# seung-lab/igneous

Measured on AMD Instinct MI355X. Metric: Mvoxels/s meshed (512^3 uint64 seg chunk), higher is better.
Workload: dtype u64; 1 GPU; 512^3 uint64 Voronoi chunk, ~50k labels, seed=303 (BASELINE configs[2]); labels=50000, simplification=0, input_residency=device (MG_FLAG_SKIP_H2D, MG_FLAG_DEVICE_ONLY), n_labels_meshed=49992, total_tris=155686827

## Files before the change

### igneous_amd/csrc/mc_table.h

```cpp
#ifndef MC_TABLE_H
#define MC_TABLE_H

#ifndef MC_TABLE_QUAL
#define MC_TABLE_QUAL static const
#endif

#define MC_MAX_TRIS 5

MC_TABLE_QUAL unsigned char MC_TRI_COUNT[256] = {
  0, 1, 1, 2, 1, 2, 2, 3, 1, 2, 2, 3, 2, 3, 3, 2,
  1, 2, 2, 3, 2, 3, 3, 4, 2, 3, 3, 4, 3, 4, 4, 3,
  1, 2, 2, 3, 2, 3, 3, 4, 2, 3, 3, 4, 3, 4, 4, 3,
  2, 3, 3, 2, 3, 4, 4, 3, 3, 4, 4, 3, 4, 5, 5, 2,
  1, 2, 2, 3, 2, 3, 3, 4, 2, 3, 3, 4, 3, 4, 4, 3,
  2, 3, 3, 4, 3, 2, 4, 3, 3, 4, 4, 5, 4, 3, 5, 2,
  2, 3, 3, 4, 3, 4, 4, 5, 3, 4, 4, 5, 4, 5, 5, 4,
  3, 4, 4, 3, 4, 3, 5, 2, 4, 5, 5, 4, 5, 4, 2, 1,
  1, 2, 2, 3, 2, 3, 3, 4, 2, 3, 3, 4, 3, 4, 4, 3,
  2, 3, 3, 4, 3, 4, 4, 5, 3, 4, 4, 5, 4, 5, 5, 4,
  2, 3, 3, 4, 3, 4, 4, 5, 3, 4, 2, 3, 4, 5, 3, 2,
  3, 4, 4, 3, 4, 5, 5, 4, 4, 5, 3, 2, 5, 2, 4, 1,
  2, 3, 3, 4, 3, 4, 4, 5, 3, 4, 4, 5, 2, 3, 3, 2,
  3, 4, 4, 5, 4, 3, 5, 4, 4, 5, 5, 2, 3, 2, 4, 1,
  3, 4, 4, 5, 4, 5, 5, 2, 4, 5, 3, 4, 3, 4, 2, 1,
// ... 496 lines not shown
  {0x5d30, 0x0af0, 0x6050, 0x6b10, 0x4750},
  {0x6891, 0x5d22, 0x0000, 0x0000, 0x0000},
  {0x5302, 0x5682, 0x5ea2, 0x0000, 0x0000},
  {0x5ea0, 0x0ae0, 0x0000, 0x0000, 0x0000},
  {0x5d30, 0x0af0, 0x6050, 0x5310, 0x0000},
  {0x5d22, 0x0000, 0x0000, 0x0000, 0x0000},
  {0x6ad2, 0x6f52, 0x6772, 0x0000, 0x0000},
  {0x2080, 0x6ad2, 0x6f52, 0x6772, 0x0000},
  {0x5a50, 0x6ad0, 0x6f50, 0x1770, 0x0000},
  {0x6ad2, 0x6f52, 0x1772, 0x10b2, 0x2092},
  {0x6761, 0x4b21, 0x5a41, 0x52c1, 0x0000},
  {0x6c20, 0x6760, 0x4b20, 0x5a40, 0x22c0},
  {0x5a50, 0x52d0, 0x0690, 0x6c30, 0x1770},
  {0x1761, 0x22d2, 0x0000, 0x0000, 0x0000},
  {0x66b1, 0x4b31, 0x5a51, 0x6ad1, 0x0000},
  {0x2080, 0x66b1, 0x4b31, 0x5a51, 0x6ad1},
  {0x5a50, 0x6ad0, 0x4750, 0x0000, 0x0000},
  {0x2091, 0x4911, 0x5a51, 0x6ad1, 0x0000},
  {0x52d2, 0x5692, 0x66b2, 0x0000, 0x0000},
  {0x66a0, 0x4b20, 0x5a40, 0x22c0, 0x0000},
  {0x5a50, 0x52d0, 0x0000, 0x0000, 0x0000},
  {0x22d2, 0x0000, 0x0000, 0x0000, 0x0000},
  {0x6f58, 0x6778, 0x0000, 0x0000, 0x0000},
  {0x6880, 0x6f40, 0x6760, 0x0000, 0x0000},
  {0x6b10, 0x6f50, 0x1770, 0x0000, 0x0000},
  {0x6f44, 0x1764, 0x0000, 0x0000, 0x0000},
  {0x6761, 0x6321, 0x5301, 0x0000, 0x0000},
  {0x6c20, 0x6760, 0x0000, 0x0000, 0x0000},
  {0x5310, 0x0690, 0x6c30, 0x1770, 0x0000},
  {0x1761, 0x0000, 0x0000, 0x0000, 0x0000},
  {0x66b1, 0x6331, 0x6b11, 0x0000, 0x0000},
  {0x6880, 0x4740, 0x5620, 0x66a0, 0x0000},
  {0x6b10, 0x4750, 0x0000, 0x0000, 0x0000},
  {0x6891, 0x0000, 0x0000, 0x0000, 0x0000},
  {0x66b4, 0x6334, 0x0000, 0x0000, 0x0000},
  {0x66a0, 0x0000, 0x0000, 0x0000, 0x0000},
  {0x5310, 0x0000, 0x0000, 0x0000, 0x0000},
  {0x0000, 0x0000, 0x0000, 0x0000, 0x0000},
};

MC_TABLE_QUAL unsigned char MC_TRI_FIRST[256][5] = {
  {0, 0, 0, 0, 0},
  {7, 0, 0, 0, 0},
  {7, 0, 0, 0, 0},
  {7, 4, 0, 0, 0},
  {7, 0, 0, 0, 0},
  {7, 4, 0, 0, 0},
  {7, 7, 0, 0, 0},
  {7, 4, 4, 0, 0},
  {7, 0, 0, 0, 0},
  {7, 7, 0, 0, 0},
  {7, 4, 0, 0, 0},
  {7, 4, 4, 0, 0},
  {7, 4, 0, 0, 0},
  {7, 4, 4, 0, 0},
  {7, 4, 4, 0, 0},
  {7, 4, 0, 0, 0},
  {7, 0, 0, 0, 0},
  {7, 4, 0, 0, 0},
  {7, 7, 0, 0, 0},
  {7, 4, 4, 0, 0},
  {7, 7, 0, 0, 0},
  {7, 4, 4, 0, 0},
  {7, 7, 7, 0, 0},
  {7, 4, 4, 4, 0},
  {7, 7, 0, 0, 0},
  {7, 4, 7, 0, 0},
  {7, 4, 7, 0, 0},
  {7, 4, 4, 4, 0},
  {7, 7, 4, 0, 0},
  {7, 4, 4, 4, 0},
  {7, 4, 4, 7, 0},
  {7, 4, 4, 0, 0},
  {7, 0, 0, 0, 0},
  {7, 7, 0, 0, 0},
  {7, 4, 0, 0, 0},
  {7, 4, 4, 0, 0},
  {7, 7, 0, 0, 0},
  {7, 4, 7, 0, 0},
  {7, 4, 7, 0, 0},
  {7, 4, 4, 4, 0},
  {7, 7, 0, 0, 0},
  {7, 7, 7, 0, 0},
  {7, 4, 4, 0, 0},
  {7, 4, 4, 4, 0},
  {7, 7, 4, 0, 0},
  {7, 4, 4, 7, 0},
  {7, 4, 4, 4, 0},
  {7, 4, 4, 0, 0},
  {7, 4, 0, 0, 0},
  {7, 4, 4, 0, 0},
  {7, 4, 4, 0, 0},
  {7, 4, 0, 0, 0},
  {7, 7, 4, 0, 0},
  {7, 4, 4, 4, 0},
  {7, 4, 4, 7, 0},
  {7, 4, 4, 0, 0},
  {7, 7, 4, 0, 0},
  {7, 4, 4, 7, 0},
  {7, 4, 4, 4, 0},
  {7, 4, 4, 0, 0},
  {7, 4, 7, 4, 0},
  {7, 4, 4, 4, 4},
  {7, 4, 4, 4, 4},
  {7, 4, 0, 0, 0},
  {7, 0, 0, 0, 0},
  {7, 7, 0, 0, 0},
  {7, 7, 0, 0, 0},
  {7, 7, 4, 0, 0},
  {7, 4, 0, 0, 0},
  {7, 4, 4, 0, 0},
  {7, 7, 4, 0, 0},
  {7, 4, 4, 4, 0},
  {7, 7, 0, 0, 0},
  {7, 7, 7, 0, 0},
  {7, 4, 7, 0, 0},
  {7, 4, 4, 7, 0},
  {7, 4, 4, 0, 0},
  {7, 4, 4, 4, 0},
  {7, 4, 4, 4, 0},
  {7, 4, 4, 0, 0},
  {7, 4, 0, 0, 0},
  {7, 4, 4, 0, 0},
  {7, 7, 4, 0, 0},
  {7, 4, 4, 4, 0},
  {7, 4, 4, 0, 0},
  {7, 4, 0, 0, 0},
  {7, 7, 4, 4, 0},
  {7, 4, 4, 0, 0},
  {7, 7, 4, 0, 0},
  {7, 4, 4, 7, 0},
  {7, 4, 7, 4, 0},
  {7, 4, 4, 4, 4},
  {7, 4, 4, 4, 0},
  {7, 4, 4, 0, 0},
  {7, 4, 4, 4, 4},
  {7, 4, 0, 0, 0},
  {7, 7, 0, 0, 0},
  {7, 7, 7, 0, 0},
  {7, 4, 7, 0, 0},
  {7, 4, 4, 7, 0},
  {7, 4, 7, 0, 0},
  {7, 4, 4, 7, 0},
  {7, 4, 7, 4, 0},
  {7, 4, 4, 4, 4},
  {7, 7, 7, 0, 0},
  {7, 7, 7, 7, 0},
  {7, 4, 4, 7, 0},
  {7, 4, 4, 4, 7},
  {7, 7, 4, 4, 0},
  {7, 4, 4, 4, 7},
  {7, 4, 4, 4, 4},
  {7, 4, 4, 4, 0},
  {7, 4, 4, 0, 0},
  {7, 4, 4, 4, 0},
  {7, 4, 4, 4, 0},
  {7, 4, 4, 0, 0},
  {7, 4, 4, 4, 0},
  {7, 4, 4, 0, 0},
  {7, 4, 4, 4, 4},
  {7, 4, 0, 0, 0},
  {7, 7, 4, 4, 0},
  {7, 4, 4, 4, 7},
  {7, 4, 4, 4, 4},
  {7, 4, 4, 4, 0},
  {7, 4, 4, 4, 4},
  {7, 4, 4, 4, 0},
  {7, 7, 0, 0, 0},
  {7, 0, 0, 0, 0},
  {7, 0, 0, 0, 0},
  {7, 7, 0, 0, 0},
  {7, 7, 0, 0, 0},
  {7, 7, 4, 0, 0},
  {7, 7, 0, 0, 0},
  {7, 4, 7, 0, 0},
  {7, 7, 7, 0, 0},
  {7, 4, 4, 7, 0},
  {7, 4, 0, 0, 0},
  {7, 7, 4, 0, 0},
  {7, 4, 4, 0, 0},
  {7, 4, 4, 4, 0},
  {7, 4, 4, 0, 0},
  {7, 4, 4, 4, 0},
  {7, 4, 4, 4, 0},
  {7, 4, 4, 0, 0},
  {7, 7, 0, 0, 0},
  {7, 4, 7, 0, 0},
  {7, 7, 7, 0, 0},
  {7, 4, 4, 7, 0},
  {7, 7, 7, 0, 0},
  {7, 4, 4, 7, 0},
  {7, 7, 7, 7, 0},
  {7, 4, 4, 4, 7},
  {7, 4, 7, 0, 0},
  {7, 4, 7, 4, 0},
  {7, 4, 4, 7, 0},
  {7, 4, 4, 4, 4},
  {7, 7, 4, 4, 0},
  {7, 4, 4, 4, 4},
  {7, 4, 4, 4, 7},
  {7, 4, 4, 4, 0},
  {7, 4, 0, 0, 0},
  {7, 7, 4, 0, 0},
  {7, 4, 4, 0, 0},
  {7, 4, 4, 4, 0},
  {7, 7, 4, 0, 0},
  {7, 4, 7, 4, 0},
  {7, 4, 4, 7, 0},
  {7, 4, 4, 4, 4},
  {7, 4, 4, 0, 0},
  {7, 7, 4, 4, 0},
  {7, 4, 0, 0, 0},
  {7, 4, 4, 0, 0},
  {7, 4, 4, 4, 0},
  {7, 4, 4, 4, 4},
  {7, 4, 4, 0, 0},
  {7, 4, 0, 0, 0},
  {7, 4, 4, 0, 0},
  {7, 4, 4, 4, 0},
  {7, 4, 4, 4, 0},
  {7, 4, 4, 0, 0},
  {7, 7, 4, 4, 0},
  {7, 4, 4, 4, 4},
  {7, 4, 4, 4, 7},
  {7, 4, 4, 4, 0},
  {7, 4, 4, 4, 0},
  {7, 4, 4, 4, 4},
  {7, 4, 4, 0, 0},
  {7, 4, 0, 0, 0},
  {7, 4, 4, 4, 4},
  {7, 7, 0, 0, 0},
  {7, 4, 4, 4, 0},
  {7, 0, 0, 0, 0},
  {7, 4, 0, 0, 0},
  {7, 7, 4, 0, 0},
  {7, 7, 4, 0, 0},
  {7, 4, 7, 4, 0},
  {7, 4, 4, 0, 0},
  {7, 4, 4, 4, 0},
  {7, 7, 4, 4, 0},
  {7, 4, 4, 4, 4},
  {7, 4, 4, 0, 0},
  {7, 7, 4, 4, 0},
  {7, 4, 4, 4, 0},
  {7, 4, 4, 4, 4},
  {7, 4, 0, 0, 0},
  {7, 4, 4, 0, 0},
  {7, 4, 4, 0, 0},
  {7, 4, 0, 0, 0},
  {7, 4, 4, 0, 0},
  {7, 4, 4, 4, 0},
  {7, 7, 4, 4, 0},
  {7, 4, 4, 4, 4},
  {7, 4, 4, 4, 0},
  {7, 4, 4, 0, 0},
  {7, 7, 4, 4, 4},
  {7, 4, 4, 4, 0},
  {7, 4, 4, 4, 0},
  {7, 4, 4, 4, 4},
  {7, 4, 4, 4, 4},
  {7, 7, 0, 0, 0},
  {7, 4, 4, 0, 0},
  {7, 4, 0, 0, 0},
  {7, 4, 4, 4, 0},
  {7, 0, 0, 0, 0},
  {7, 4, 4, 0, 0},
  {7, 7, 4, 4, 0},
  {7, 4, 4, 4, 0},
  {7, 4, 4, 4, 4},
  {7, 4, 4, 4, 0},
  {7, 4, 4, 4, 4},
  {7, 4, 4, 4, 4},
  {7, 7, 0, 0, 0},
  {7, 4, 4, 4, 0},
  {7, 7, 4, 4, 4},
  {7, 4, 4, 0, 0},
  {7, 4, 4, 4, 0},
  {7, 4, 4, 0, 0},
  {7, 4, 4, 4, 0},
  {7, 4, 0, 0, 0},
  {7, 0, 0, 0, 0},
  {7, 4, 0, 0, 0},
  {7, 4, 4, 0, 0},
  {7, 4, 4, 0, 0},
  {7, 4, 0, 0, 0},
  {7, 4, 4, 0, 0},
  {7, 4, 0, 0, 0},
  {7, 4, 4, 4, 0},
  {7, 0, 0, 0, 0},
  {7, 4, 4, 0, 0},
  {7, 4, 4, 4, 0},
  {7, 4, 0, 0, 0},
  {7, 0, 0, 0, 0},
  {7, 4, 0, 0, 0},
  {7, 0, 0, 0, 0},
  {7, 0, 0, 0, 0},
  {0, 0, 0, 0, 0},
};

MC_TABLE_QUAL unsigned char MC_EDGE_NEED[12] = {
  6, 4, 2, 0, 5, 4, 1, 0, 3, 2, 1, 0,
};

MC_TABLE_QUAL unsigned char MC_EDGE_CORNERS[12][2] = {
  {0, 1},
  {2, 3},
  {4, 5},
  {6, 7},
  {0, 2},
  {1, 3},
  {4, 6},
  {5, 7},
  {0, 4},
  {1, 5},
  {2, 6},
  {3, 7},
};

MC_TABLE_QUAL unsigned long long MC_EDGE_KEYOFF[12] = {
  0x1ULL,
  0x2001ULL,
  0x2000001ULL,
  0x2002001ULL,
  0x1000ULL,
  0x1002ULL,
  0x2001000ULL,
  0x2001002ULL,
  0x1000000ULL,
  0x1000002ULL,
  0x1002000ULL,
  0x1002002ULL,
};

#endif
```

### igneous_amd/csrc/meshgine.hip

```cpp

#include "mg_ctx.h"

#include <algorithm>
#include <atomic>
#include <vector>

#define MC_TABLE_QUAL __device__ static const
#include "mc_table.h"


#define WAVE 64

static inline uint64_t next_pow2_u64(uint64_t x) {
  if (x < 2) return 2;
  return 1ull << (64 - __builtin_clzll(x - 1));
}

__device__ __forceinline__ uint64_t mix64(uint64_t x) {
  x += 0x9E3779B97F4A7C15ull;
  x = (x ^ (x >> 30)) * 0xBF58476D1CE4E5B9ull;
  x = (x ^ (x >> 27)) * 0x94D049BB133111EBull;
  return x ^ (x >> 31);
}

__device__ __forceinline__ uint32_t wave_incl_scan(uint32_t x, int lane) {
  for (int d = 1; d < WAVE; d <<= 1) {
    uint32_t y = __shfl_up(x, d, WAVE);
    if (lane >= d) x += y;
  }
  return x;
}


struct LabelHash {
  uint64_t *keys;
  uint32_t *vals;
  uint32_t *counter;
  uint32_t *overflow;
  uint64_t nslots;
};

__device__ __forceinline__ void label_insert(LabelHash h, uint64_t label) {
  uint64_t slot = mix64(label) & (h.nslots - 1);
  for (uint64_t probe = 0; probe < h.nslots; ++probe) {
    uint64_t cur = h.keys[slot];
    if (cur == label) return;
    if (cur == 0) {
      uint64_t prev = atomicCAS((unsigned long long *)&h.keys[slot], 0ull,
                                (unsigned long long)label);
      if (prev == 0) {
        h.vals[slot] = atomicAdd(h.counter, 1u);
        return;
      }
      if (prev == label) return;
    }
    slot = (slot + 1) & (h.nslots - 1);
  }
  atomicExch(h.overflow, 1u);
}

__device__ __forceinline__ uint32_t label_lookup(LabelHash h, uint64_t label) {
  uint64_t slot = mix64(label) & (h.nslots - 1);
  for (uint64_t probe = 0; probe < h.nslots; ++probe) {
    if (h.keys[slot] == label) return h.vals[slot];
    slot = (slot + 1) & (h.nslots - 1);
  }
  atomicExch(h.overflow, 1u);
  return 0;
}


template <typename T>
__global__ void k_dust_build(const T *__restrict__ labels, uint64_t nvox,
                             LabelHash lh) {
  for (uint64_t i = (uint64_t)blockIdx.x * blockDim.x + threadIdx.x;
       i < nvox; i += (uint64_t)gridDim.x * blockDim.x) {
    T L = labels[i];
    if (L != 0) label_insert(lh, (uint64_t)L);
  }
}

template <typename T>
__global__ void k_dust_count(const T *__restrict__ labels, uint64_t nvox,
                             LabelHash lh, uint32_t *__restrict__ counts) {
  for (uint64_t i = (uint64_t)blockIdx.x * blockDim.x + threadIdx.x;
       i < nvox; i += (uint64_t)gridDim.x * blockDim.x) {
    T L = labels[i];
    if (L != 0) atomicAdd(&counts[label_lookup(lh, (uint64_t)L)], 1u);
  }
}

template <typename T>
__global__ void k_dust_zero(T *__restrict__ labels, uint64_t nvox,
                            LabelHash lh,
                            const uint32_t *__restrict__ counts,
                            uint64_t thr) {
  for (uint64_t i = (uint64_t)blockIdx.x * blockDim.x + threadIdx.x;
       i < nvox; i += (uint64_t)gridDim.x * blockDim.x) {
    T L = labels[i];
    if (L != 0 && (uint64_t)counts[label_lookup(lh, (uint64_t)L)] < thr)
      labels[i] = 0;
  }
}


struct MapTable {
  ulonglong2 *slots;
  uint64_t nslots;
};

#define MAP_ERR_DUPLICATE 1u
#define MAP_ERR_FULL      2u

__global__ void k_map_build(const uint64_t *__restrict__ keys,
                            const uint64_t *__restrict__ vals, uint64_t n,
                            MapTable t, uint32_t *__restrict__ err) {
  uint64_t i = (uint64_t)blockIdx.x * blockDim.x + threadIdx.x;
  if (i >= n) return;
  const uint64_t key = keys[i];
  uint64_t slot = mix64(key) & (t.nslots - 1);
  for (uint64_t probe = 0; probe < t.nslots; ++probe) {
    uint64_t prev = atomicCAS((unsigned long long *)&t.slots[slot].x, 0ull,
                              (unsigned long long)key);
    if (prev == 0) {
      t.slots[slot].y = vals[i];
      return;
    }
    if (prev == key) {
      atomicOr(err, MAP_ERR_DUPLICATE);
      return;
    }
    slot = (slot + 1) & (t.nslots - 1);
  }
  atomicOr(err, MAP_ERR_FULL);
}

template <typename T>
__device__ __forceinline__ T map_one(T L, const MapTable &t, bool miss_zero,
                                     T &cl, T &cr) {
  if (L == 0) return 0;
  if (L == cl) return cr;
  T r = miss_zero ? (T)0 : L;
  uint64_t slot = mix64((uint64_t)L) & (t.nslots - 1);
  for (uint64_t probe = 0; probe < t.nslots; ++probe) {
    ulonglong2 e = t.slots[slot];
    if (e.x == (uint64_t)L) { r = (T)e.y; break; }
    if (e.x == 0) break;
    slot = (slot + 1) & (t.nslots - 1);
  }
  cl = L;
  cr = r;
  return r;
}

template <typename T> struct MapVec;
template <> struct MapVec<uint64_t> { typedef ulonglong2 type; };
template <> struct MapVec<uint32_t> { typedef uint4 type; };

template <typename T>
__device__ __forceinline__ void map_volume(T *__restrict__ labels,
                                           uint64_t nvox, const MapTable &t,
                                           uint32_t miss_zero) {
  typedef typename MapVec<T>::type V;
  constexpr int NV = 16 / sizeof(T);
  const uint64_t nvec = nvox / NV;
  const uint64_t tid = (uint64_t)blockIdx.x * blockDim.x + threadIdx.x;
  const uint64_t nthr = (uint64_t)gridDim.x * blockDim.x;
  const bool mz = miss_zero != 0;
  T cl = 0, cr = 0;
  V *vp = reinterpret_cast<V *>(labels);
  for (uint64_t i = tid; i < nvec; i += nthr) {
    union { V v; T e[NV]; } in, o;
    in.v = vp[i];
    bool changed = false;
#pragma unroll
    for (int k = 0; k < NV; ++k) {
      o.e[k] = map_one<T>(in.e[k], t, mz, cl, cr);
      changed |= (o.e[k] != in.e[k]);
    }
    if (changed) vp[i] = o.v;
  }
  const uint64_t i = nvec * NV + tid;
  if (i < nvox) {
    T L = labels[i];
    T r = map_one<T>(L, t, mz, cl, cr);
    if (r != L) labels[i] = r;
  }
}

template <typename T>
__global__ void k_label_map(T *__restrict__ labels, uint64_t nvox,
                            MapTable t, uint32_t miss_zero) {
  map_volume<T>(labels, nvox, t, miss_zero);
}

#define MAP_LDS_MAX_ENTRIES 2048u
#define MAP_LDS_BLOCK 1024

template <typename T>
__global__ __launch_bounds__(MAP_LDS_BLOCK) void k_label_map_lds(
    T *__restrict__ labels, uint64_t nvox, MapTable g, uint32_t miss_zero) {
  extern __shared__ ulonglong2 s_map_tab[];
  for (uint32_t i = threadIdx.x; i < (uint32_t)g.nslots; i += blockDim.x)
    s_map_tab[i] = g.slots[i];
  __syncthreads();
  MapTable t;
  t.slots = s_map_tab;
  t.nslots = g.nslots;
  map_volume<T>(labels, nvox, t, miss_zero);
}

__global__ void k_label_values(LabelHash h, uint64_t *values, uint64_t nslots) {
  uint64_t i = (uint64_t)blockIdx.x * blockDim.x + threadIdx.x;
  if (i >= nslots) return;
  uint64_t k = h.keys[i];
  if (k != 0) values[h.vals[i]] = k;
}


template <typename T>
__device__ __forceinline__ void load_corners(const T *__restrict__ labels,
                                             int64_t sx, int64_t sxy,
                                             int64_t cx, int64_t cy, int64_t cz,
                                             T c[8]) {
  const T *p = labels + cx + cy * sx + cz * sxy;
  c[0] = p[0];            c[1] = p[1];
  c[2] = p[sx];           c[3] = p[sx + 1];
  c[4] = p[sxy];          c[5] = p[sxy + 1];
  c[6] = p[sxy + sx];     c[7] = p[sxy + sx + 1];
}

struct CellClass {
  uint64_t rows;
  uint32_t first;
  __device__ __forceinline__ uint32_t row(uint32_t i) const {
    return (uint32_t)(rows >> (i * 8u)) & 255u;
  }
};

template <typename T>
__device__ __forceinline__ CellClass classify_cell(const T c[8]) {
  uint32_t r[8];
  #pragma unroll
  for (int i = 0; i < 8; ++i) r[i] = 1u << i;
  uint32_t seen = 0;
  #pragma unroll
  for (int j = 1; j < 8; ++j) {
    #pragma unroll
    for (int i = 0; i < j; ++i) {
      const bool eq = c[i] == c[j];
      r[i] |= eq ? (1u << j) : 0u;
      r[j] |= eq ? (1u << i) : 0u;
      seen |= eq ? (1u << j) : 0u;
    }
  }
  uint32_t nz = 0;
  #pragma unroll
  for (int i = 0; i < 8; ++i) nz |= (c[i] != 0) ? (1u << i) : 0u;
  const uint32_t lo = r[0] | (r[1] << 8) | (r[2] << 16) | (r[3] << 24);
  const uint32_t hi = r[4] | (r[5] << 8) | (r[6] << 16) | (r[7] << 24);
  CellClass k;
  k.rows = ((uint64_t)hi << 32) | lo;
  k.first = r[0] == 255u ? 0u : (nz & ~seen);
  return k;
}

template <typename T>
__device__ __forceinline__ T pick_corner(const T c[8], uint32_t i) {
  const bool b0 = i & 1u, b1 = i & 2u, b2 = i & 4u;
  const T a0 = b0 ? c[1] : c[0], a1 = b0 ? c[3] : c[2];
  const T a2 = b0 ? c[5] : c[4], a3 = b0 ? c[7] : c[6];
  const T d0 = b1 ? a1 : a0, d1 = b1 ? a3 : a2;
  return b2 ? d1 : d0;
}

struct GridDims {
  int64_t sx, sy, sz;
  int64_t ncx, ncy, ncz;
  int64_t nsegx;
  int64_t nseg;
};

struct SegSched {
  int64_t beg, end, step;
};

__device__ __forceinline__ SegSched xcd_seg_sched(int64_t nseg,
                                                  int waves_per_blk,
                                                  int wave_in_blk) {
  const int64_t xcd = blockIdx.x & 7;
  const int64_t j = blockIdx.x >> 3;
  const int64_t nbx = (gridDim.x + 7) >> 3;
  const int64_t slab = (nseg + 7) >> 3;
  SegSched ss;
  ss.beg = xcd * slab + j * waves_per_blk + wave_in_blk;
  ss.end = std::min<int64_t>((xcd + 1) * slab, nseg);
  ss.step = nbx * waves_per_blk;
  return ss;
}

template <typename T>
__global__ void k_count(const T *__restrict__ labels, GridDims g,
                        uint64_t *__restrict__ segcnt, LabelHash lh) {
  __shared__ uint8_t s_cnt[256];
  for (int k = threadIdx.x; k < 256; k += blockDim.x)
    s_cnt[k] = MC_TRI_COUNT[k];
  __syncthreads();
  const int lane = threadIdx.x & (WAVE - 1);
  const int wave_in_blk = threadIdx.x / WAVE;
  const int waves_per_blk = blockDim.x / WAVE;
  const int64_t sxy = g.sx * g.sy;
  const SegSched ss = xcd_seg_sched(g.nseg, waves_per_blk, wave_in_blk);
  for (int64_t seg = ss.beg; seg < ss.end; seg += ss.step) {
    const int64_t row = seg / g.nsegx;
    const int64_t segx = seg - row * g.nsegx;
    const int64_t cy = row % g.ncy;
    const int64_t cz = row / g.ncy;
    const int64_t cx = segx * WAVE + lane;
    uint32_t cnt = 0;
    if (cx < g.ncx) {
      T c[8];
      load_corners(labels, g.sx, sxy, cx, cy, cz, c);
      const CellClass k = classify_cell(c);
      cnt = (uint32_t)__popc(k.first);
      for (uint32_t f = k.first; f; f &= f - 1) {
        const uint32_t i = (uint32_t)__builtin_ctz(f);
        cnt += (uint32_t)s_cnt[k.row(i)] << 16;
        label_insert(lh, (uint64_t)pick_corner(c, i));
      }
    }
    uint32_t incl = wave_incl_scan(cnt, lane);
    if (lane == WAVE - 1)
      segcnt[seg] = ((uint64_t)(incl >> 16) << 32) | (incl & 0xffffu);
  }
}


__device__ __forceinline__ void stage_decode_tables(
    uint16_t *s_pack, uint32_t *s_comb, int64_t sx, int64_t sxy) {
  for (int k = threadIdx.x; k < 256; k += blockDim.x) {
    #pragma unroll
    for (int t = 0; t < MC_MAX_TRIS; ++t)
      s_pack[k * MC_MAX_TRIS + t] = MC_TRI_PACK[k][t];
  }
  if (threadIdx.x < 12) {
    int e = threadIdx.x;
    uint32_t eoff = (uint32_t)(MC_EDGE_DOFF[e][0] >> 1) +
                    (uint32_t)(MC_EDGE_DOFF[e][1] >> 1) * (uint32_t)sx +
                    (uint32_t)(MC_EDGE_DOFF[e][2] >> 1) * (uint32_t)sxy;
    uint32_t axis = (MC_EDGE_DOFF[e][0] & 1)
                        ? 0u
                        : ((MC_EDGE_DOFF[e][1] & 1) ? 1u : 2u);
    s_comb[e] = eoff * 3u + axis;
  }
}

template <typename T>
__global__ __launch_bounds__(256, 8) void k_emit(
    const T *__restrict__ labels, GridDims g,
    const uint64_t *__restrict__ segoff, LabelHash lh,
    uint32_t *__restrict__ item_label, uint2 *__restrict__ item_recs) {
  const int lane = threadIdx.x & (WAVE - 1);
  const int wave_in_blk = threadIdx.x / WAVE;
  const int waves_per_blk = blockDim.x / WAVE;
  const int64_t sxy = g.sx * g.sy;
  const SegSched ss = xcd_seg_sched(g.nseg, waves_per_blk, wave_in_blk);
  for (int64_t seg = ss.beg; seg < ss.end; seg += ss.step) {
    const int64_t row = seg / g.nsegx;
    const int64_t segx = seg - row * g.nsegx;
    const int64_t cy = row % g.ncy;
    const int64_t cz = row / g.ncy;
    const int64_t cx = segx * WAVE + lane;
    T c[8];
    CellClass k;
    k.rows = 0;
    k.first = 0;
    if (cx < g.ncx) {
      load_corners(labels, g.sx, sxy, cx, cy, cz, c);
      k = classify_cell(c);
    }
    const uint32_t cnt = (uint32_t)__popc(k.first);
    uint32_t incl = wave_incl_scan(cnt, lane);
    uint32_t pos = (uint32_t)segoff[seg] + incl - cnt;
    const uint32_t cell_lin = (uint32_t)((cz * g.sy + cy) * g.sx + cx);
    const uint32_t zero = (uint32_t)(cx == 0) | ((uint32_t)(cy == 0) << 1) |
                          ((uint32_t)(cz == 0) << 2);
    for (uint32_t f = k.first; f; f &= f - 1) {
      const uint32_t i = (uint32_t)__builtin_ctz(f);
      const uint32_t lid = label_lookup(lh, (uint64_t)pick_corner(c, i));
      item_label[pos] = lid;
      item_recs[pos] = make_uint2(cell_lin, k.row(i) | (zero << 11));
      ++pos;
    }
  }
}

struct ItemTris {
  __device__ uint32_t operator()(uint2 rec) const {
    return MC_TRI_COUNT[rec.y & 255u];
  }
};
struct ItemTrisVia {
  const uint2 *recs;
  __device__ uint32_t operator()(uint32_t o) const {
    return MC_TRI_COUNT[recs[o].y & 255u];
  }
};

#define WELD_FIRST_BLK 256
__global__ void k_label_ranges(const uint32_t *__restrict__ item_lab,
                               uint32_t *__restrict__ itoff,
                               uint32_t *__restrict__ tri_off,
                               uint32_t *__restrict__ blk_item,
                               uint64_t nitems, uint64_t ntris,
                               uint32_t nlabels) {
  uint64_t i = (uint64_t)blockIdx.x * blockDim.x + threadIdx.x;
  if (i >= nitems) return;
  uint32_t a = 0;
  if (i == 0) {
    itoff[0] = 0;
    tri_off[item_lab[0]] = 0;
    tri_off[nlabels] = (uint32_t)ntris;
  } else {
    a = itoff[i];
    if (item_lab[i] != item_lab[i - 1]) tri_off[item_lab[i]] = a;
  }
  const uint32_t b = itoff[i + 1];
  const uint32_t m = (a + WELD_FIRST_BLK - 1) / WELD_FIRST_BLK;
  if (m * WELD_FIRST_BLK < b) blk_item[m] = (uint32_t)i;
}



__global__ __launch_bounds__(WELD_FIRST_BLK) void k_weld_first(
    const uint2 *__restrict__ item_recs,
    const uint32_t *__restrict__ order,
    const uint32_t *__restrict__ item_lab,
    const uint32_t *__restrict__ itoff,
    const uint32_t *__restrict__ blk_item,
    uint32_t *__restrict__ lab_sorted,
    uint32_t *__restrict__ slots_sorted,
    uint32_t *__restrict__ wminp,
    unsigned long long *__restrict__ bits,
    int64_t sx, int64_t sxy,
    uint64_t nitems, uint64_t ntris, uint64_t nwords) {
  __shared__ uint16_t s_pack[256 * MC_MAX_TRIS];
  __shared__ uint8_t s_first[256 * MC_MAX_TRIS];
  __shared__ uint32_t s_comb[12];
  __shared__ uint32_t s_need[12];
  __shared__ uint32_t s_off[WELD_FIRST_BLK + 1];
  __shared__ uint2 s_rec[WELD_FIRST_BLK];
  __shared__ uint32_t s_lab[WELD_FIRST_BLK];
  __shared__ uint8_t s_item[WELD_FIRST_BLK];
  stage_decode_tables(s_pack, s_comb, sx, sxy);
  for (int k = threadIdx.x; k < 256 * MC_MAX_TRIS; k += blockDim.x)
    s_first[k] = MC_TRI_FIRST[k / MC_MAX_TRIS][k % MC_MAX_TRIS];
  if (threadIdx.x < 12) s_need[threadIdx.x] = MC_EDGE_NEED[threadIdx.x];
  const uint64_t t = (uint64_t)blockIdx.x * WELD_FIRST_BLK + threadIdx.x;
  const uint32_t t0 = blockIdx.x * WELD_FIRST_BLK;
  const uint64_t first = blk_item[blockIdx.x];
  const uint64_t it = first + threadIdx.x;
  s_off[threadIdx.x] = itoff[std::min<uint64_t>(it, nitems)];
  if (threadIdx.x == 0)
    s_off[WELD_FIRST_BLK] =
        itoff[std::min<uint64_t>(first + WELD_FIRST_BLK, nitems)];
  __syncthreads();
  {
    const uint32_t lo = std::max(s_off[threadIdx.x], t0);
    const uint32_t hi = std::min<uint32_t>(s_off[threadIdx.x + 1],
                                           t0 + WELD_FIRST_BLK);
    if (lo < hi) {
      s_rec[threadIdx.x] = order ? item_recs[order[it]] : item_recs[it];
      s_lab[threadIdx.x] = item_lab[it];
      for (uint32_t q = lo; q < hi; ++q)
        s_item[q - t0] = (uint8_t)threadIdx.x;
    }
  }
  __syncthreads();
  const uint32_t lane = threadIdx.x & (WAVE - 1);
  bool f[3] = {false, false, false};
  if (t < ntris) {
    const uint32_t j = s_item[threadIdx.x];
    uint2 rec = s_rec[j];
    rec.y |= ((uint32_t)t - s_off[j]) << 8;
    lab_sorted[t] = s_lab[j];
    const uint32_t ti = (rec.y & 255u) * MC_MAX_TRIS + ((rec.y >> 8) & 7u);
    const uint32_t pk = s_pack[ti];
    const uint32_t fb = s_first[ti];
    const uint32_t interior = ~(rec.y >> 11) & 7u;
    const uint32_t cl3 = rec.x * 3u;
    #pragma unroll
    for (int v = 0; v < 3; ++v) {
      const uint32_t nib = (pk >> (5 * v)) & 31u;
      const uint32_t e = nib & 15u;
      const uint32_t slot = ((cl3 + s_comb[e]) << 1) | (nib >> 4);
      slots_sorted[3 * t + v] = slot;
      f[v] = ((fb >> v) & 1u) && (s_need[e] & interior) == 0;
      if (f[v]) wminp[slot] = (uint32_t)(3 * t + v);
    }
  }
  const unsigned long long bal[3] = {__ballot(f[0]), __ballot(f[1]),
                                     __ballot(f[2])};
  const uint64_t w0 = (t / WAVE) * 3;
  #pragma unroll
  for (uint32_t j = 0; j < 3; ++j) {
    const uint32_t c = 64 * j + lane;
    const uint32_t q = c / 3, r = c - 3 * q;
    const unsigned long long src = r == 0 ? bal[0] : (r == 1 ? bal[1] : bal[2]);
    const unsigned long long word = __ballot((src >> q) & 1ull);
    if (lane == j && w0 + j < nwords) bits[w0 + j] = word;
  }
}

struct PopcWord {
  __device__ uint32_t operator()(unsigned long long w) const {
    return (uint32_t)__popcll(w);
  }
};

__device__ __forceinline__ uint32_t vtx_id_of(
    const uint32_t *__restrict__ wscan,
    const unsigned long long *__restrict__ bits, uint64_t i) {
  uint64_t w = i >> 6;
  unsigned long long mask = (1ull << (i & 63)) - 1;
  return wscan[w] + (uint32_t)__popcll(bits[w] & mask);
}

__global__ void k_total_verts(const uint32_t *__restrict__ wscan,
                              const unsigned long long *__restrict__ bits,
                              uint64_t nwords, uint32_t *out) {
  *out = wscan[nwords - 1] + (uint32_t)__popcll(bits[nwords - 1]);
}

__global__ void k_vbase(const uint32_t *__restrict__ tri_off,
                        const uint32_t *__restrict__ wscan,
                        const unsigned long long *__restrict__ bits,
                        uint32_t *__restrict__ vbase,
                        uint32_t nlabels, uint64_t total_verts) {
  uint32_t l = blockIdx.x * blockDim.x + threadIdx.x;
  if (l > nlabels) return;
  if (l == nlabels) vbase[l] = (uint32_t)total_verts;
  else vbase[l] = vtx_id_of(wscan, bits, 3ull * tri_off[l]);
}

__global__ void k_weld_verts_faces(const uint32_t *__restrict__ slots,
                                   const uint32_t *__restrict__ wminp,
                                   const uint32_t *__restrict__ lab_sorted,
                                   const uint32_t *__restrict__ wscan,
                                   const unsigned long long *__restrict__ bits,
                                   const uint32_t *__restrict__ vbase,
                                   float *__restrict__ verts,
                                   uint32_t *__restrict__ faces,
                                   uint32_t usx, uint32_t usxy,
                                   float rx, float ry, float rz, float shift,
                                   uint64_t ntris) {
  uint64_t t = (uint64_t)blockIdx.x * blockDim.x + threadIdx.x;
  if (t >= ntris) return;
  const uint32_t e[3] = {slots[3 * t], slots[3 * t + 1], slots[3 * t + 2]};
  const uint32_t base = vbase[lab_sorted[t]];
  const uint64_t w0 = (3 * t) >> 6;
  const uint32_t b0 = (uint32_t)((3 * t) & 63);
  const bool straddle = b0 > 61;
  const unsigned long long word0 = bits[w0];
  const uint32_t scan0 = wscan[w0];
  const unsigned long long word1 = straddle ? bits[w0 + 1] : 0ull;
  const uint32_t scan1 = straddle ? wscan[w0 + 1] : 0u;
  #pragma unroll
  for (int v = 0; v < 3; ++v) {
    uint32_t b = b0 + v;
    const bool second = b > 63;
    const unsigned long long word = second ? word1 : word0;
    b &= 63;
    uint32_t vid;
    if ((word >> b) & 1ull) {
      vid = (second ? scan1 : scan0) +
            (uint32_t)__popcll(word & ((1ull << b) - 1));
      uint32_t eslot = e[v] >> 1;
      uint32_t axis = eslot % 3u;
      uint32_t lin = eslot / 3u;
      uint32_t vz = lin / usxy;
      uint32_t rem = lin - vz * usxy;
      uint32_t vy = rem / usx;
      uint32_t vx = rem - vy * usx;
      float dx = (float)(2 * vx + (axis == 0));
      float dy = (float)(2 * vy + (axis == 1));
      float dz = (float)(2 * vz + (axis == 2));
      verts[3ull * vid + 0] = (0.5f * dx + shift) * rx;
      verts[3ull * vid + 1] = (0.5f * dy + shift) * ry;
      verts[3ull * vid + 2] = (0.5f * dz + shift) * rz;
    } else {
      vid = vtx_id_of(wscan, bits, wminp[e[v]]);
    }
    faces[3 * t + v] = vid - base;
  }
}

__global__ void k_iota(uint32_t *p, uint64_t n) {
  uint64_t i = (uint64_t)blockIdx.x * blockDim.x + threadIdx.x;
  if (i < n) p[i] = (uint32_t)i;
}

__global__ void k_last_sum(const uint32_t *scan, const uint32_t *input,
                           uint64_t n, uint32_t *out) {
  *out = scan[n - 1] + input[n - 1];
}

__global__ void k_any_active(const uint8_t *active, uint32_t nlabels,
                             uint32_t *any) {
  uint32_t l = blockIdx.x * blockDim.x + threadIdx.x;
  if (l < nlabels && active[l]) atomicExch(any, 1u);
}

#include "simplify.hip"


static LabelHash label_hash_view(mg_ctx *c) {
  LabelHash lh;
  lh.keys = c->lh_keys.get();
  lh.vals = c->lh_vals.get();
  lh.counter = &c->scalars->lh_counter;
  lh.overflow = &c->scalars->lh_overflow;
  lh.nslots = c->lh_slots;
  return lh;
}

static int label_hash_reset(mg_ctx *c, int rc) {
  if (ensure(c, c->lh_keys, c->lh_slots)) return rc;
  if (ensure(c, c->lh_vals, c->lh_slots)) return rc;
  HIP_TRY(c, hipMemsetAsync(c->lh_keys.get(), 0, c->lh_slots * 8, c->stream),
          rc);
  HIP_TRY(c, hipMemsetAsync(c->scalars.get(), 0, sizeof(CtxScalars),
                            c->stream), rc);
  return 0;
}

static int label_hash_grow(mg_ctx *c, const char *where, int rc) {
  if (c->lh_slots >= (1ull << 27)) {
    SET_ERR(c, "label hash overflow%s at %llu slots", where,
            (unsigned long long)c->lh_slots);
    return rc;
  }
  c->lh_slots <<= 2;
  return 0;
}

static int hash_volume_labels(mg_ctx *c, int dtype, uint64_t nvox,
                              const char *where, int rc, uint32_t *p_n) {
  hipStream_t s = c->stream;
  for (;;) {
    if (int e = label_hash_reset(c, rc)) return e;
    const LabelHash lh = label_hash_view(c);
    by_dtype(dtype, [&](auto t) {
      using T = decltype(t);
      hipLaunchKernelGGL(k_dust_build<T>, dim3(4096), dim3(256), 0, s,
                         c->labels.as<const T>(), nvox, lh);
    });
    uint32_t misc[2] = {0, 0};
    HIP_TRY(c, hipMemcpyAsync(misc, &c->scalars->lh_counter, 8,
                              hipMemcpyDeviceToHost, s), rc);
    HIP_TRY(c, hipStreamSynchronize(s), rc);
    if (!misc[1]) {
      *p_n = misc[0];
      return 0;
    }
    if (int e = label_hash_grow(c, where, rc)) return e;
  }
}

#include "fill_holes.hip"

extern "C" {

const char *mg_version(void) { return "meshgine 0.1.0 (gfx950)"; }

int mg_device_count(void) {
  int n = 0;
  if (hipGetDeviceCount(&n) != hipSuccess) return 0;
  return n;
}

mg_ctx *mg_init(int device_id) {
  int n = 0;
  if (hipGetDeviceCount(&n) != hipSuccess || device_id >= n || n == 0) {
    return nullptr;
  }
  if (hipSetDevice(device_id) != hipSuccess) return nullptr;
  mg_ctx *c = new mg_ctx();
  c->device = device_id;
  bool ok =
      hipStreamCreateWithFlags(&c->stream, hipStreamNonBlocking) ==
          hipSuccess &&
      hipStreamCreateWithFlags(&c->stream2, hipStreamNonBlocking) ==
          hipSuccess;
  for (auto &e : c->ev) ok = ok && hipEventCreate(&e) == hipSuccess;
  ok = ok && ensure(c, c->scalars, 1) == 0 &&
       hipMemsetAsync(c->scalars.get(), 0, sizeof(CtxScalars), c->stream) ==
           hipSuccess;
  if (!ok) {
    delete c;
    return nullptr;
  }
  return c;
}

void mg_destroy(mg_ctx *c) { delete c; }

const char *mg_last_error(mg_ctx *c) {
  return c ? c->err.c_str() : g_err.c_str();
}

int mg_get_stats(mg_ctx *c, mg_stats *out) {
  if (!c || !out) return 1;
  *out = c->stats;
  return 0;
}

void mg_meshset_free(mg_meshset *ms) {
  free(ms);
}

}

static int new_meshset(mg_ctx *c, uint32_t n, mg_meshset **out) {
  *out = alloc_meshset(n, 0);
  if (!*out) {
    SET_ERR(c, "mesh_chunk: out of host memory");
    return 24;
  }
  return 0;
}

static double ev_ms(mg_ctx *c, int a, int b) {
  float ms = 0.f;
  if (hipEventElapsedTime(&ms, c->ev[a], c->ev[b]) != hipSuccess) return 0.0;
  return (double)ms;
}


#define MG_MAP_MAX_ENTRIES (1ull << 24)

struct ChunkCall {
  int sx, sy, sz, dtype;
  size_t esize;
  uint64_t nvox;
  GridDims g;
  float rx, ry, rz;
  int voxel_centered;
  uint32_t nlabels;
  uint64_t NI;
  uint64_t T;
  uint64_t V;
  const uint32_t *item_lab;
  const uint2 *rec_src;
  const uint32_t *order_sorted;
  uint32_t *slots;
  uint32_t *lab_sorted;
};

static void set_hole_stash(mg_ctx *c, const ChunkCall &k) {
  c->holes_valid = true;
  c->holes_sx = k.sx; c->holes_sy = k.sy; c->holes_sz = k.sz;
  c->holes_dtype = k.dtype;
}

static int upload_labels(mg_ctx *c, const ChunkCall &k,
                         const void *labels_host, uint32_t flags) {
  const size_t bytes = k.nvox * k.esize;
  if ((flags & (MG_FLAG_SKIP_H2D | MG_FLAG_COUNTED)) && c->labels.cap >= bytes)
    return 0;
  if (ensure_bytes(c, c->labels, bytes)) return 11;
  HIP_TRY(c, hipMemcpyAsync(c->labels.ptr, labels_host, bytes,
                            hipMemcpyHostToDevice, c->stream), 11);
  return 0;
}

static int run_dust(mg_ctx *c, const ChunkCall &k, uint64_t dust_threshold) {
  hipStream_t s = c->stream;
  uint32_t ndl = 0;
  if (int e = hash_volume_labels(c, k.dtype, k.nvox, " (dust)", 16, &ndl))
    return e;
  if (ndl == 0) return 0;
  const LabelHash lh = label_hash_view(c);
  if (ensure(c, c->order, ndl)) return 16;
  HIP_TRY(c, hipMemsetAsync(c->order.get(), 0, (uint64_t)ndl * 4, s), 16);
  by_dtype(k.dtype, [&](auto t) {
    using T = decltype(t);
    const dim3 nb(4096), blk(256);
    hipLaunchKernelGGL(k_dust_count<T>, nb, blk, 0, s,
                       c->labels.as<const T>(), k.nvox, lh, c->order.get());
    hipLaunchKernelGGL(k_dust_zero<T>, nb, blk, 0, s, c->labels.as<T>(),
                       k.nvox, lh, c->order.get(), dust_threshold);
  });
  HIP_TRY(c, hipGetLastError(), 16);
  return 0;
}

static int run_label_map(mg_ctx *c, const ChunkCall &k,
                         const mg_label_map *map) {
  hipStream_t s = c->stream;
  const uint64_t n = map->n, nvox = k.nvox;
  MapTable mt;
  mt.nslots = next_pow2_u64(std::max<uint64_t>(2 * n, 64));
  if (ensure(c, c->map_tab, mt.nslots)) return 41;
  mt.slots = c->map_tab.get();
  uint32_t *d_err = &c->scalars->map_err;
  HIP_TRY(c, hipEventRecord(c->ev[EV_MAP_START], s), 41);
  HIP_TRY(c, hipMemsetAsync(mt.slots, 0, mt.nslots * 16, s), 41);
  HIP_TRY(c, hipMemsetAsync(d_err, 0, 4, s), 41);
  if (n > 0) {
    if (ensure(c, c->map_keys, n)) return 41;
    if (ensure(c, c->map_vals, n)) return 41;
    HIP_TRY(c, hipMemcpyAsync(c->map_keys.get(), map->keys, n * 8,
                              hipMemcpyHostToDevice, s), 41);
    HIP_TRY(c, hipMemcpyAsync(c->map_vals.get(), map->vals, n * 8,
                              hipMemcpyHostToDevice, s), 41);
    const int bblk = 256;
    hipLaunchKernelGGL(k_map_build, dim3((uint32_t)((n + bblk - 1) / bblk)),
                       dim3(bblk), 0, s, c->map_keys.get(),
                       c->map_vals.get(), n, mt, d_err);
  }
  const uint64_t nvec = nvox / (16 / k.esize);
  const uint32_t miss_zero = map->miss == MG_MAP_MISS_ZERO;
  static const bool use_lds = []() {
    const char *e = getenv("MG_MAP_LDS");
    return !(e && e[0] == '0');
  }();
  const bool lds = use_lds && n <= MAP_LDS_MAX_ENTRIES;
  const int mblk = lds ? MAP_LDS_BLOCK : 256;
  const uint32_t mnb = (uint32_t)std::min<uint64_t>(
      std::max<uint64_t>((nvec + mblk - 1) / mblk, 1), lds ? 512 : 4096);
  by_dtype(k.dtype, [&](auto t) {
    using T = decltype(t);
    if (lds)
      hipLaunchKernelGGL(k_label_map_lds<T>, dim3(mnb), dim3(mblk),
                         mt.nslots * 16, s, c->labels.as<T>(), nvox, mt,
                         miss_zero);
    else
      hipLaunchKernelGGL(k_label_map<T>, dim3(mnb), dim3(mblk), 0, s,
                         c->labels.as<T>(), nvox, mt, miss_zero);
  });
  HIP_TRY(c, hipGetLastError(), 41);
  HIP_TRY(c, hipEventRecord(c->ev[EV_MAP_END], s), 41);
  uint32_t map_err = 0;
  HIP_TRY(c, hipMemcpyAsync(&map_err, d_err, 4, hipMemcpyDeviceToHost, s),
          41);
  HIP_TRY(c, hipStreamSynchronize(s), 41);
  if (map_err & MAP_ERR_DUPLICATE) {
    SET_ERR(c, "label map: duplicate key among %llu entries",
            (unsigned long long)n);
    return 42;
  }
  if (map_err) {
    SET_ERR(c, "label map: table build failed (flag %u)", map_err);
    return 42;
  }
  c->stats.ms_labelmap = ev_ms(c, EV_MAP_START, EV_MAP_END);
  return 0;
}

static inline uint32_t seg_blocks(const GridDims &g, int blk) {
  const int waves_per_blk = blk / WAVE;
  int64_t nb = std::min<int64_t>(
      (g.nseg + waves_per_blk - 1) / waves_per_blk, 8192);
  return (uint32_t)((nb + 7) & ~7ll);
}

static int count_pass(mg_ctx *c, ChunkCall &k, bool *p_overflow) {
  hipStream_t s = c->stream;
  const LabelHash lh = label_hash_view(c);
  uint64_t *d_segcnt = c->segcnt.get();
  uint64_t *d_segoff = c->segoff.get();
  const int64_t nseg = k.g.nseg;
  HIP_TRY(c, hipEventRecord(c->ev[EV_H2D_END], s), 30);
  by_dtype(k.dtype, [&](auto t) {
    using T = decltype(t);
    hipLaunchKernelGGL(k_count<T>, dim3(seg_blocks(k.g, 256)), dim3(256), 0,
                       s, c->labels.as<const T>(), k.g, d_segcnt, lh);
  });
  HIP_TRY(c, hipGetLastError(), 30);
  HIP_TRY(c, hipEventRecord(c->ev[EV_COUNT_END], s), 30);

  uint32_t misc[2] = {0, 0};
  HIP_TRY(c, hipMemcpyAsync(misc, &c->scalars->lh_counter, 8,
                            hipMemcpyDeviceToHost, s), 30);
  if (int e = scan_u64(c, d_segcnt, d_segoff, (size_t)nseg, s,
                       "seg scan size query failed", "seg scan failed", 30))
    return e;
  uint64_t last_off = 0, last_cnt = 0;
  HIP_TRY(c, hipMemcpyAsync(&last_off, d_segoff + (nseg - 1), 8,
                            hipMemcpyDeviceToHost, s), 30);
  HIP_TRY(c, hipMemcpyAsync(&last_cnt, d_segcnt + (nseg - 1), 8,
                            hipMemcpyDeviceToHost, s), 30);
  HIP_TRY(c, hipEventRecord(c->ev[EV_SCAN_END], s), 30);
  HIP_TRY(c, hipStreamSynchronize(s), 30);
  *p_overflow = misc[1] != 0;
  k.nlabels = misc[0];
  const uint64_t total = last_off + last_cnt;
  k.NI = total & 0xffffffffull;
  k.T = total >> 32;
  return 0;
}

static int run_count_emit(mg_ctx *c, ChunkCall &k) {
  hipStream_t s = c->stream;
  if (ensure(c, c->segcnt, k.g.nseg)) return 12;
  if (ensure(c, c->segoff, k.g.nseg)) return 12;
  for (;;) {
    if (int e = label_hash_reset(c, 12)) return e;
    bool overflow = false;
    if (int e = count_pass(c, k, &overflow)) return e;
    if (!overflow) break;
    if (int e = label_hash_grow(c, "", 13)) return e;
  }
  c->stats.total_tris = k.T;
  c->stats.n_labels = k.nlabels;
  if (k.T == 0 || k.nlabels == 0) return 0;
  if (k.T > (1ull << 31) / 3 * 2) {
    SET_ERR(c, "chunk produces %llu triangles (> corner-index limit); "
            "split the task shape", (unsigned long long)k.T);
    return 15;
  }
  if (k.nlabels >= (1u << 27)) {
    SET_ERR(c, "%u labels exceed the 2^27 per-chunk label limit", k.nlabels);
    return 15;
  }
  const LabelHash lh = label_hash_view(c);
  if (ensure(c, c->label_values, k.nlabels)) return 17;
  hipLaunchKernelGGL(k_label_values,
                     dim3((uint32_t)((c->lh_slots + 255) / 256)), dim3(256),
                     0, s, lh, c->label_values.get(), c->lh_slots);
  if (ensure(c, c->tri_label, k.NI)) return 18;
  if (ensure(c, c->tri_keys, k.NI)) return 18;
  by_dtype(k.dtype, [&](auto t) {
    using T = decltype(t);
    hipLaunchKernelGGL(k_emit<T>, dim3(seg_blocks(k.g, 256)), dim3(256), 0, s,
                       c->labels.as<const T>(), k.g, c->segoff.get(), lh,
                       c->tri_label.get(), c->tri_keys.get());
  });
  HIP_TRY(c, hipGetLastError(), 18);
  HIP_TRY(c, hipEventRecord(c->ev[EV_EMIT_END], s), 18);
  return 0;
}

struct TriSortView {
  uint64_t *recs, *recs_alt;
  uint32_t *slots;
};

static TriSortView tri_sort_view(mg_ctx *c, uint64_t NI) {
  return {reinterpret_cast<uint64_t *>(c->tri_keys.get()),
          reinterpret_cast<uint64_t *>(c->keys_sorted.get()),
          c->keys_sorted.get() + 2 * NI};
}

static int run_partition(mg_ctx *c, ChunkCall &k) {
  hipStream_t s = c->stream;
  const uint64_t T = k.T, NI = k.NI;
  const char *sre = getenv("MG_SORT_RECS");
  const bool sort_recs = !(sre && sre[0] == '0');
  if (ensure(c, c->keys_sorted, 2 * NI + 3 * T)) return 19;
  if (ensure(c, c->tri_label_alt, NI)) return 19;
  const TriSortView tv = tri_sort_view(c, NI);
  k.slots = tv.slots;
  const dim3 nb((uint32_t)((NI + 255) / 256)), blk(256);
  unsigned end_bit = 1;
  while ((1u << end_bit) < k.nlabels) ++end_bit;
  rocprim::double_buffer<uint32_t> d_keys(c->tri_label.get(),
                                          c->tri_label_alt.get());
  if (sort_recs) {
    rocprim::double_buffer<uint64_t> d_vals(tv.recs, tv.recs_alt);
    if (int e = sort_pairs(c, d_keys, d_vals, NI, 0u, end_bit, s,
                           "radix_sort size query failed",
                           "radix_sort failed", 19))
      return e;
    k.rec_src = reinterpret_cast<const uint2 *>(d_vals.current());
    k.order_sorted = nullptr;
  } else {
    if (ensure(c, c->order, NI)) return 19;
    if (ensure(c, c->order_alt, NI)) return 19;
    hipLaunchKernelGGL(k_iota, nb, blk, 0, s, c->order.get(), NI);
    rocprim::double_buffer<uint32_t> d_vals(c->order.get(),
                                            c->order_alt.get());
    if (int e = sort_pairs(c, d_keys, d_vals, NI, 0u, end_bit, s,
                           "radix_sort size query failed",
                           "radix_sort failed", 19))
      return e;
    k.rec_src = c->tri_keys.get();
    k.order_sorted = d_vals.current();
  }
  k.item_lab = d_keys.current();
  if (ensure(c, c->itoff, NI + 1)) return 19;
  uint32_t *itoff = c->itoff.get();
  if (int e = k.order_sorted
          ? scan_incl_u32(c, rocprim::make_transform_iterator(
                                 k.order_sorted, ItemTrisVia{k.rec_src}),
                          itoff + 1, NI, s, "item scan size query failed",
                          "item scan failed", 19)
          : scan_incl_u32(c, rocprim::make_transform_iterator(
                                 k.rec_src, ItemTris{}),
                          itoff + 1, NI, s, "item scan size query failed",
                          "item scan failed", 19))
    return e;
  if (ensure(c, c->tri_off, (uint64_t)k.nlabels + 1)) return 19;
  if (ensure(c, c->blk_item, (T + WELD_FIRST_BLK - 1) / WELD_FIRST_BLK))
    return 19;
  hipLaunchKernelGGL(k_label_ranges, nb, blk, 0, s, k.item_lab, itoff,
                     c->tri_off.get(), c->blk_item.get(), NI, T, k.nlabels);
  HIP_TRY(c, hipGetLastError(), 19);
  HIP_TRY(c, hipEventRecord(c->ev[EV_PARTITION_END], s), 19);
  return 0;
}

struct WeldScanView {
  unsigned long long *bits;
  uint32_t *wscan;
};

static WeldScanView weld_scan_view(mg_ctx *c, uint64_t nwords) {
  return {reinterpret_cast<unsigned long long *>(c->vtx_scan.get()),
          c->vtx_scan.get() + 2 * nwords};
}

static int run_weld(mg_ctx *c, ChunkCall &k) {
  hipStream_t s = c->stream;
  const uint64_t T = k.T, NC = 3 * T;
  const uint64_t wslots = 6 * k.nvox;
  if (wslots >= (1ull << 32)) {
    SET_ERR(c, "chunk too large for the 32-bit weld table (%d x %d x %d); "
            "split the task shape (the reference's own mesher bound is "
            "1023x1023x511, igneous_cli/cli.py:1049-1052)", k.sx, k.sy, k.sz);
    return 20;
  }
  if (ensure(c, c->wh_keys, wslots)) return 20;
  if (ensure(c, c->vtx_scan, NC)) return 20;
  if (ensure(c, c->lab_sorted, T)) return 20;
  k.lab_sorted = c->lab_sorted.get();
  uint32_t *wminp = c->wh_keys.get();
  const dim3 nbt((uint32_t)((T + 255) / 256)), blk(256);
  const uint64_t nwords = (NC + 63) / 64;
  auto [bits, wscan] = weld_scan_view(c, nwords);
  hipLaunchKernelGGL(k_weld_first,
                     dim3((uint32_t)((T + WELD_FIRST_BLK - 1) / WELD_FIRST_BLK)),
                     dim3(WELD_FIRST_BLK), 0, s, k.rec_src, k.order_sorted,
                     k.item_lab, c->itoff.get(), c->blk_item.get(),
                     k.lab_sorted, k.slots, wminp, bits, k.g.sx,
                     k.g.sx * k.g.sy, k.NI, T, nwords);
  if (int e = scan_u32(c, rocprim::make_transform_iterator(bits, PopcWord{}),
                       wscan, nwords, s, "weld scan size query failed",
                       "weld scan failed", 20))
    return e;
  uint32_t *d_tv = &c->scalars->weld_verts;
  hipLaunchKernelGGL(k_total_verts, dim3(1), dim3(1), 0, s, wscan, bits,
                     nwords, d_tv);
  uint32_t tv = 0;
  HIP_TRY(c, hipMemcpyAsync(&tv, d_tv, 4, hipMemcpyDeviceToHost, s), 21);
  HIP_TRY(c, hipStreamSynchronize(s), 21);
  k.V = tv;
  c->stats.total_verts = tv;

  if (ensure(c, c->verts, 3 * k.V)) return 22;
  if (ensure(c, c->faces, NC)) return 22;
  if (ensure(c, c->vbase, (uint64_t)k.nlabels + 1)) return 22;
  hipLaunchKernelGGL(k_vbase, dim3((k.nlabels + 1 + 255) / 256), dim3(256),
                     0, s, c->tri_off.get(), wscan, bits, c->vbase.get(),
                     k.nlabels, k.V);
  hipLaunchKernelGGL(k_weld_verts_faces, nbt, blk, 0, s, k.slots, wminp,
                     k.lab_sorted, wscan, bits, c->vbase.get(),
                     c->verts.get(), c->faces.get(), (uint32_t)k.g.sx,
                     (uint32_t)(k.g.sx * k.g.sy), k.rx, k.ry, k.rz,
                     k.voxel_centered ? 0.0f : 0.5f, T);
  HIP_TRY(c, hipGetLastError(), 22);
  HIP_TRY(c, hipEventRecord(c->ev[EV_WELD_END], s), 22);
  return 0;
}

static int extract_meshset(mg_ctx *c, const ChunkCall &k, uint32_t flags,
                           mg_meshset **out) {
  hipStream_t s = c->stream;
  if (flags & MG_FLAG_DEVICE_ONLY) {
    HIP_TRY(c, hipStreamSynchronize(s), 23);
    return new_meshset(c, 0, out);
  }
  const uint32_t nlabels = k.nlabels;
  const uint64_t V = k.V, NC = 3 * k.T;
  if (ensure(c, c->h_verts, 3 * V + 3)) return 24;
  if (ensure(c, c->h_faces, NC + 1)) return 24;
  float *h_verts = c->h_verts.get();
  uint32_t *h_faces = c->h_faces.get();
  std::vector<uint32_t> h_tri_off(nlabels + 1), h_vbase(nlabels + 1);
  std::vector<uint64_t> h_label_values(nlabels);
  if (V > 0)
    HIP_TRY(c, hipMemcpyAsync(h_verts, c->verts.get(), V * 12,
                              hipMemcpyDeviceToHost, s), 24);
  if (NC > 0)
    HIP_TRY(c, hipMemcpyAsync(h_faces, c->faces.get(), NC * 4,
                              hipMemcpyDeviceToHost, s), 24);
  HIP_TRY(c, hipMemcpyAsync(h_tri_off.data(), c->tri_off.get(),
                            (nlabels + 1) * 4, hipMemcpyDeviceToHost, s), 24);
  HIP_TRY(c, hipMemcpyAsync(h_vbase.data(), c->vbase.get(), (nlabels + 1) * 4,
                            hipMemcpyDeviceToHost, s), 24);
  HIP_TRY(c, hipMemcpyAsync(h_label_values.data(), c->label_values.get(),
                            nlabels * 8, hipMemcpyDeviceToHost, s), 24);
  HIP_TRY(c, hipStreamSynchronize(s), 24);

  mg_meshset *ms = nullptr;
  if (int e = new_meshset(c, nlabels, &ms)) return e;
  ms->verts_base = h_verts;
  ms->faces_base = h_faces;
  ms->total_verts = V;
  ms->total_tris = k.T;
  std::vector<uint32_t> idx(nlabels);
  for (uint32_t i = 0; i < nlabels; ++i) idx[i] = i;
  std::sort(idx.begin(), idx.end(), [&](uint32_t a, uint32_t b) {
    return h_label_values[a] < h_label_values[b];
  });
  for (uint32_t m = 0; m < nlabels; ++m) {
    uint32_t l = idx[m];
    set_mesh(ms, m, h_label_values[l], h_vbase[l], h_vbase[l + 1] - h_vbase[l],
             h_tri_off[l], h_tri_off[l + 1] - h_tri_off[l]);
  }
  *out = ms;
  return 0;
}

#include "encode.hip"

struct ChunkRequest {
  const void *labels;
  int sx, sy, sz, dtype;
  float rx, ry, rz;
  uint32_t reduction_factor;
  float max_error;
  int voxel_centered;
  uint64_t dust_threshold;
  uint32_t flags;
  const mg_label_map *map;
  uint32_t fill_level;
  const mg_encode_params *ep;
  mg_meshset **out;
  mg_blobset **bout;
  EncParams enc;
};

static int empty_result(mg_ctx *c, const ChunkRequest &r) {
  return r.bout ? new_blobset(c, 0, r.bout) : new_meshset(c, 0, r.out);
}

static void write_stage_times(mg_ctx *c, const ChunkRequest &r, bool meshed) {
  mg_stats &st = c->stats;
  st.ms_h2d = ev_ms(c, EV_START, EV_H2D_END);
  if (r.fill_level) st.ms_fill = ev_ms(c, EV_FILL_START, EV_FILL_END);
  if (!meshed) return;
  st.ms_count = ev_ms(c, EV_H2D_END, EV_COUNT_END);
  st.ms_scan = ev_ms(c, EV_COUNT_END, EV_SCAN_END);
  st.ms_emit = ev_ms(c, EV_SCAN_END, EV_EMIT_END);
  st.ms_partition = ev_ms(c, EV_EMIT_END, EV_PARTITION_END);
  st.ms_weld = ev_ms(c, EV_PARTITION_END, EV_WELD_END);
  st.ms_simplify = ev_ms(c, EV_WELD_END, EV_SIMPLIFY_END);
  st.ms_d2h = ev_ms(c, r.bout ? EV_ENCODE_END : EV_SIMPLIFY_END, EV_END);
  if (r.bout) st.ms_encode = ev_ms(c, EV_SIMPLIFY_END, EV_ENCODE_END);
  st.ms_total = ev_ms(c, EV_START, EV_END);
}

static int mesh_chunk_impl(mg_ctx *c, const ChunkRequest &r) {
  ChunkCall k = {};
  k.sx = r.sx; k.sy = r.sy; k.sz = r.sz; k.dtype = r.dtype;
  k.esize = (r.dtype == MG_U64) ? 8 : 4;
  k.nvox = (uint64_t)r.sx * r.sy * r.sz;
  k.rx = r.rx; k.ry = r.ry; k.rz = r.rz;
  k.voxel_centered = r.voxel_centered;
  GridDims &g = k.g;
  g.sx = r.sx; g.sy = r.sy; g.sz = r.sz;
  g.ncx = r.sx > 1 ? r.sx - 1 : 0;
  g.ncy = r.sy > 1 ? r.sy - 1 : 0;
  g.ncz = r.sz > 1 ? r.sz - 1 : 0;
  g.nsegx = (g.ncx + WAVE - 1) / WAVE;
  g.nseg = g.nsegx * g.ncy * g.ncz;

  memset(&c->stats, 0, sizeof(c->stats));
  c->stats.bytes_read_algorithmic = k.nvox * k.esize;
  hipStream_t s = c->stream;

  if (g.nseg == 0) {
    if (int e = empty_result(c, r)) return e;
    if (r.fill_level) set_hole_stash(c, k);
    return 0;
  }

  HIP_TRY(c, hipEventRecord(c->ev[EV_START], s), 10);
  if (int e = upload_labels(c, k, r.labels, r.flags)) return e;
  HIP_TRY(c, hipEventRecord(c->ev[EV_H2D_END], s), 11);
  if (r.dust_threshold > 0)
    if (int e = run_dust(c, k, r.dust_threshold)) return e;
  if (r.map)
    if (int e = run_label_map(c, k, r.map)) return e;
  if (r.fill_level) {
    HIP_TRY(c, hipEventRecord(c->ev[EV_FILL_START], s), 56);
    if (int e = run_fill_holes(c, r.dtype, r.sx, r.sy, r.sz, r.fill_level,
                               nullptr))
      return e;
    HIP_TRY(c, hipEventRecord(c->ev[EV_FILL_END], s), 56);
    set_hole_stash(c, k);
  }

  if (int e = run_count_emit(c, k)) return e;
  if (k.T == 0 || k.nlabels == 0) {
    if (int e = empty_result(c, r)) return e;
    HIP_TRY(c, hipStreamSynchronize(s), 14);
    write_stage_times(c, r, false);
    return 0;
  }
  if (int e = run_partition(c, k)) return e;
  if (int e = run_weld(c, k)) return e;
  if (r.reduction_factor > 1 && k.T > 0)
    if (int e = run_simplify(c, k.nlabels, k.lab_sorted, r.reduction_factor,
                             r.max_error, &k.T, &k.V))
      return e;
  HIP_TRY(c, hipEventRecord(c->ev[EV_SIMPLIFY_END], s), 22);
  if (int e = r.bout ? run_encode(c, k, r.flags, r.enc, r.bout)
                     : extract_meshset(c, k, r.flags, r.out))
    return e;
  HIP_TRY(c, hipEventRecord(c->ev[EV_END], s), 25);
  HIP_TRY(c, hipStreamSynchronize(s), 25);
  write_stage_times(c, r, true);
  return 0;
}


static int check_volume_args(mg_ctx *c, int sx, int sy, int sz, int dtype) {
  if (sx < 1 || sy < 1 || sz < 1 || sx > 2047 || sy > 2047 || sz > 2047) {
    SET_ERR(c, "dims out of range (1..2047): %d %d %d", sx, sy, sz);
    return 2;
  }
  if (dtype != MG_U32 && dtype != MG_U64) {
    SET_ERR(c, "bad dtype %d", dtype);
    return 3;
  }
  return 0;
}

static int check_label_map(mg_ctx *c, const mg_label_map *map, int dtype,
                           uint32_t flags) {
  if (map->miss != MG_MAP_MISS_KEEP && map->miss != MG_MAP_MISS_ZERO) {
    SET_ERR(c, "label map: bad miss policy %u", map->miss);
    return 5;
  }
  if (flags & MG_FLAG_SKIP_H2D) {
    SET_ERR(c, "label map cannot be combined with MG_FLAG_SKIP_H2D "
            "(the resident volume is already mapped)");
    return 5;
  }
  if (map->n > MG_MAP_MAX_ENTRIES) {
    SET_ERR(c, "label map: %llu entries exceed the %llu-entry cap",
            (unsigned long long)map->n,
            (unsigned long long)MG_MAP_MAX_ENTRIES);
    return 5;
  }
  if (map->n > 0 && (!map->keys || !map->vals)) {
    SET_ERR(c, "label map: null keys/vals with n=%llu",
            (unsigned long long)map->n);
    return 5;
  }
  for (uint64_t i = 0; i < map->n; ++i) {
    if (map->keys[i] == 0) {
      SET_ERR(c, "label map: key 0 at entry %llu (label 0 is never "
              "looked up)", (unsigned long long)i);
      return 5;
    }
    if (dtype == MG_U32 && map->vals[i] > 0xFFFFFFFFull) {
      SET_ERR(c, "label map: value %llu at entry %llu does not fit "
              "MG_U32", (unsigned long long)map->vals[i],
              (unsigned long long)i);
      return 5;
    }
  }
  return 0;
}

#include "chunk_mesh.hip"
#include "merge_verts.hip"
#include "octree_level.hip"
#include "count_voxels.hip"

static int check_counted(mg_ctx *c, const ChunkRequest &r, bool counted) {
  if (r.flags & MG_FLAG_SKIP_H2D) {
    SET_ERR(c, "MG_FLAG_COUNTED cannot be combined with MG_FLAG_SKIP_H2D");
    return 9;
  }
  if (!counted) {
    SET_ERR(c, "MG_FLAG_COUNTED: no counted volume on this ctx (it is left "
            "by mg_count_voxels for the call right after it)");
    return 9;
  }
  if (r.sx != c->counted_sx || r.sy != c->counted_sy ||
      r.sz != c->counted_sz || r.dtype != c->counted_dtype) {
    SET_ERR(c, "MG_FLAG_COUNTED: the counted volume is %d x %d x %d dtype %d, "
            "the call asks for %d x %d x %d dtype %d", c->counted_sx,
            c->counted_sy, c->counted_sz, c->counted_dtype, r.sx, r.sy, r.sz,
            r.dtype);
    return 9;
  }
  return 0;
}

static int mesh_chunk_checked(mg_ctx *c, ChunkRequest r) {
  if (!c) { SET_ERR(c, "null ctx"); return 1; }
  std::lock_guard<std::mutex> g(c->lock);
  c->err.clear();
  if (r.fill_level > 2) {
    SET_ERR(c, "fill_level %u: only levels 0-2 are implemented (level 3 "
            "needs a multilabel dilation, 4+ a merge threshold)",
            r.fill_level);
    return 6;
  }
  if (r.fill_level && (r.flags & MG_FLAG_SKIP_H2D)) {
    SET_ERR(c, "fill_holes cannot be combined with MG_FLAG_SKIP_H2D (the "
            "resident volume is already filled)");
    return 6;
  }
  if (!r.labels || (!r.out && !r.bout)) {
    SET_ERR(c, "null argument");
    return 1;
  }
  if (r.bout)
    if (int e = check_encode_params(c, r.ep, &r.enc)) return e;
  const bool counted = c->counted_valid;
  c->holes_valid = false;
  c->counted_valid = false;
  if (int e = check_volume_args(c, r.sx, r.sy, r.sz, r.dtype)) return e;
  if (r.map)
    if (int e = check_label_map(c, r.map, r.dtype, r.flags)) return e;
  if (r.flags & MG_FLAG_COUNTED)
    if (int e = check_counted(c, r, counted)) return e;
  HIP_TRY(c, hipSetDevice(c->device), 4);
  return mesh_chunk_impl(c, r);
}

extern "C" {

int mg_mesh_chunk_filled(mg_ctx *c, const void *labels, int sx, int sy,
                         int sz, int dtype, float rx, float ry, float rz,
                         uint32_t reduction_factor, float max_error,
                         int voxel_centered, uint64_t dust_threshold,
                         uint32_t flags, const mg_label_map *map,
                         uint32_t fill_level, mg_meshset **out) {
  return mesh_chunk_checked(
      c, {labels, sx, sy, sz, dtype, rx, ry, rz, reduction_factor, max_error,
          voxel_centered, dust_threshold, flags, map, fill_level, nullptr,
          out, nullptr});
}

int mg_mesh_chunk_encoded(mg_ctx *c, const void *labels, int sx, int sy,
                          int sz, int dtype, float rx, float ry, float rz,
                          uint32_t reduction_factor, float max_error,
                          int voxel_centered, uint64_t dust_threshold,
                          uint32_t flags, const mg_label_map *map,
                          const mg_encode_params *params, mg_blobset **out) {
  return mesh_chunk_checked(
      c, {labels, sx, sy, sz, dtype, rx, ry, rz, reduction_factor, max_error,
          voxel_centered, dust_threshold, flags, map, 0u, params, nullptr,
          out});
}

void mg_blobset_free(mg_blobset *bs) { free(bs); }

int mg_mesh_chunk_mapped(mg_ctx *c, const void *labels, int sx, int sy,
                         int sz, int dtype, float rx, float ry, float rz,
                         uint32_t reduction_factor, float max_error,
                         int voxel_centered, uint64_t dust_threshold,
                         uint32_t flags, const mg_label_map *map,
                         mg_meshset **out) {
  return mesh_chunk_checked(
      c, {labels, sx, sy, sz, dtype, rx, ry, rz, reduction_factor, max_error,
          voxel_centered, dust_threshold, flags, map, 0u, nullptr, out,
          nullptr});
}

int mg_mesh_chunk(mg_ctx *c, const void *labels, int sx, int sy, int sz,
                  int dtype, float rx, float ry, float rz,
                  uint32_t reduction_factor, float max_error,
                  int voxel_centered, uint64_t dust_threshold,
                  uint32_t flags, mg_meshset **out) {
  return mesh_chunk_checked(
      c, {labels, sx, sy, sz, dtype, rx, ry, rz, reduction_factor, max_error,
          voxel_centered, dust_threshold, flags, nullptr, 0u, nullptr, out,
          nullptr});
}

int mg_mesh_holes(mg_ctx *c, float rx, float ry, float rz,
                  uint32_t reduction_factor, float max_error,
                  int voxel_centered, uint32_t flags, mg_meshset **out) {
  if (!c) { SET_ERR(c, "null ctx"); return 1; }
  std::lock_guard<std::mutex> g(c->lock);
  c->err.clear();
  if (!out) { SET_ERR(c, "null argument"); return 1; }
  if (!c->holes_valid) {
    SET_ERR(c, "mg_mesh_holes: no hole volume on this ctx (it is left by "
            "mg_mesh_chunk_filled with fill_level > 0 and consumed by one "
            "mg_mesh_holes call)");
    return 7;
  }
  c->holes_valid = false;
  c->counted_valid = false;
  HIP_TRY(c, hipSetDevice(c->device), 4);
  std::swap(c->labels, c->holes);
  return mesh_chunk_impl(
      c, {nullptr, c->holes_sx, c->holes_sy, c->holes_sz, c->holes_dtype, rx,
          ry, rz, reduction_factor, max_error, voxel_centered, 0,
          (flags & MG_FLAG_DEVICE_ONLY) | MG_FLAG_SKIP_H2D, nullptr, 0u,
          nullptr, out, nullptr});
}

int mg_fill_holes(mg_ctx *c, const void *labels, int sx, int sy, int sz,
                  int dtype, uint32_t level, void *filled_out,
                  void *holes_out, uint32_t *rounds_out) {
  if (!c) { SET_ERR(c, "null ctx"); return 1; }
  std::lock_guard<std::mutex> g(c->lock);
  c->err.clear();
  if (!labels || !filled_out || !holes_out) {
    SET_ERR(c, "null argument");
    return 1;
  }
  if (int e = check_volume_args(c, sx, sy, sz, dtype)) return e;
  if (level < 1 || level > 2) {
    SET_ERR(c, "fill level %u: only levels 1-2 are implemented (level 3 "
            "needs a multilabel dilation, 4+ a merge threshold)", level);
    return 6;
  }
  HIP_TRY(c, hipSetDevice(c->device), 4);
  const size_t bytes = (size_t)sx * sy * sz * (dtype == MG_U64 ? 8 : 4);
  c->holes_valid = false;
  c->counted_valid = false;
  if (ensure_bytes(c, c->labels, bytes)) return 11;
  HIP_TRY(c, hipMemcpyAsync(c->labels.ptr, labels, bytes,
                            hipMemcpyHostToDevice, c->stream), 11);
  uint32_t rounds = 0;
  int rc = run_fill_holes(c, dtype, sx, sy, sz, level, &rounds);
  if (rc) return rc;
  HIP_TRY(c, hipMemcpyAsync(filled_out, c->labels.ptr, bytes,
                            hipMemcpyDeviceToHost, c->stream), 55);
  HIP_TRY(c, hipMemcpyAsync(holes_out, c->holes.ptr, bytes,
                            hipMemcpyDeviceToHost, c->stream), 55);
  HIP_TRY(c, hipStreamSynchronize(c->stream), 55);
  if (rounds_out) *rounds_out = rounds;
  return 0;
}

int mg_simplify_mesh(mg_ctx *c,
                     const float *verts, uint32_t nverts,
                     const uint32_t *faces, uint32_t ntris,
                     uint32_t reduction_factor, float max_error,
                     const float **out_verts, uint32_t *out_nverts,
                     const uint32_t **out_faces, uint32_t *out_ntris) {
  if (!c) { SET_ERR(c, "null ctx"); return 1; }
  std::lock_guard<std::mutex> g(c->lock);
  c->err.clear();
  if (!verts || !faces || !out_verts || !out_faces) {
    SET_ERR(c, "null argument");
    return 1;
  }
  c->counted_valid = false;
  if (ntris > (1u << 31) / 3) {
    SET_ERR(c, "mesh too large (%u tris)", ntris);
    return 2;
  }
  HIP_TRY(c, hipSetDevice(c->device), 4);
  hipStream_t s = c->stream;
  uint64_t T = ntris, V = nverts;

  if (reduction_factor > 1 && T > 0 && V > 0) {
    if (ensure(c, c->verts, 3 * V + 3)) return 10;
    if (ensure(c, c->faces, 3 * T + 1)) return 10;
    if (ensure(c, c->tri_off, 2)) return 10;
    if (ensure(c, c->vbase, 2)) return 10;
    if (ensure(c, c->tri_label, T + 1)) return 10;
    if (ensure(c, c->vtx_scan, std::max<uint64_t>(V + 1, 3 * T))) return 10;
    HIP_TRY(c, hipMemcpyAsync(c->verts.get(), verts, V * 12,
                              hipMemcpyHostToDevice, s), 11);
    HIP_TRY(c, hipMemcpyAsync(c->faces.get(), faces, 3 * T * 4,
                              hipMemcpyHostToDevice, s), 11);
    uint32_t off_h[2] = {0, (uint32_t)T};
    uint32_t vb_h[2] = {0, (uint32_t)V};
    HIP_TRY(c, hipMemcpyAsync(c->tri_off.get(), off_h, 8,
                              hipMemcpyHostToDevice, s), 11);
    HIP_TRY(c, hipMemcpyAsync(c->vbase.get(), vb_h, 8,
                              hipMemcpyHostToDevice, s), 11);
    HIP_TRY(c, hipMemsetAsync(c->tri_label.get(), 0, T * 4, s), 11);
    int rc = run_simplify(c, 1, c->tri_label.get(), reduction_factor,
                          max_error, &T, &V);
    if (rc) return rc;
    if (ensure(c, c->h_verts, 3 * V + 3)) return 12;
    if (ensure(c, c->h_faces, 3 * T + 1)) return 12;
    if (V > 0)
      HIP_TRY(c, hipMemcpyAsync(c->h_verts.get(), c->verts.get(), V * 12,
                                hipMemcpyDeviceToHost, s), 12);
    if (T > 0)
      HIP_TRY(c, hipMemcpyAsync(c->h_faces.get(), c->faces.get(), 3 * T * 4,
                                hipMemcpyDeviceToHost, s), 12);
    HIP_TRY(c, hipStreamSynchronize(s), 12);
  } else {
    if (ensure(c, c->h_verts, 3 * V + 3)) return 12;
    if (ensure(c, c->h_faces, 3 * T + 1)) return 12;
    memcpy(c->h_verts.get(), verts, V * 12);
    memcpy(c->h_faces.get(), faces, 3 * T * 4);
  }
  *out_verts = c->h_verts.get();
  *out_nverts = (uint32_t)V;
  *out_faces = c->h_faces.get();
  *out_ntris = (uint32_t)T;
  return 0;
}

int mg_chunk_mesh(mg_ctx *c,
                  const float *verts, uint32_t nverts,
                  const uint32_t *faces, uint32_t ntris,
                  const double scale[3], const double offset[3],
                  mg_meshset **out, const uint32_t **out_order) {
  if (!c) { SET_ERR(c, "null ctx"); return 1; }
  std::lock_guard<std::mutex> g(c->lock);
  c->err.clear();
  if (!out || !out_order || !scale || !offset ||
      (ntris > 0 && (!verts || !faces))) {
    SET_ERR(c, "null argument");
    return 1;
  }
  *out = nullptr;
// ... 114 lines not shown
```

### igneous_amd/csrc/mg_ctx.h

```cpp
#pragma once

#include <cmath>
#include <cstddef>
#include <cstdint>
#include <cstdio>
#include <cstdlib>
#include <cstring>
#include <mutex>
#include <string>
#include <utility>

#include <hip/hip_runtime.h>
#include <rocprim/rocprim.hpp>

#include "../../include/meshgine.h"

template <hipError_t (*FREE)(void *)>
struct OwnedBuf {
  void *ptr = nullptr;
  size_t cap = 0;
  OwnedBuf() = default;
  OwnedBuf(const OwnedBuf &) = delete;
  OwnedBuf &operator=(const OwnedBuf &) = delete;
  OwnedBuf(OwnedBuf &&o) noexcept
      : ptr(std::exchange(o.ptr, nullptr)), cap(std::exchange(o.cap, 0)) {}
  OwnedBuf &operator=(OwnedBuf &&o) noexcept {
    if (this != &o) {
      release();
      ptr = std::exchange(o.ptr, nullptr);
      cap = std::exchange(o.cap, 0);
    }
    return *this;
  }
  ~OwnedBuf() { release(); }
  void release() {
    if (ptr) (void)FREE(ptr);
    ptr = nullptr;
    cap = 0;
  }
};
using DevBuf = OwnedBuf<hipFree>;
using HostBuf = OwnedBuf<hipHostFree>;

template <typename T, typename Owner>
struct TypedArr : Owner {
  T *get() const { return static_cast<T *>(this->ptr); }
  T *operator->() const { return get(); }
};
template <typename T> using DevArr = TypedArr<T, DevBuf>;
template <typename T> using HostArr = TypedArr<T, HostBuf>;

struct LabelVolume : DevBuf {
  template <typename T> T *as() const { return static_cast<T *>(ptr); }
};

struct CtxScalars {
  uint32_t lh_counter;
  uint32_t lh_overflow;
  uint32_t map_err;
  uint32_t weld_verts;
  uint32_t simp_kept;
  uint32_t simp_new_verts;
  uint32_t simp_final_tris;
  uint32_t cv_cursor;
  unsigned long long simp_prof[6];
};
static_assert(offsetof(CtxScalars, lh_overflow) ==
                  offsetof(CtxScalars, lh_counter) + 4, "");

struct SimpPlane;
struct CmMisc;
struct MvMisc;

struct DeviceBuffers {
  DevArr<CtxScalars> scalars;
  LabelVolume labels, holes;
  DevBuf scan_tmp, sort_tmp;
  DevArr<uint64_t> lh_keys, label_values,
      segcnt, segoff;
  DevArr<uint32_t> lh_vals,
      tri_label, tri_label_alt, order, order_alt, tri_off,
      itoff,
      blk_item,
      lab_sorted,
      keys_sorted,
      vtx_scan,
      wh_keys, faces, vbase;
  DevArr<uint2> tri_keys;
  DevArr<float> verts;
  DevArr<SimpPlane> simp_fq;
  DevArr<uint8_t> simp_valid;
  DevArr<float> simp_Q, simp_verts_alt;
  DevArr<unsigned long long> simp_pick;
  DevArr<uint32_t> simp_pk, simp_pk_alt, simp_pv, simp_pv_alt,
      simp_remap, simp_flab, simp_flab_alt, simp_faces_alt, simp_vbase_alt,
      simp_meta,
      simp_ref, simp_keep, simp_keep_scan, simp_park, simp_first,
      simp_troff_final, simp_deg, simp_adj, simp_rh, simp_accept;
  DevArr<ulonglong2> map_tab;
  DevArr<uint64_t> map_keys, map_vals;
  DevArr<uint32_t> fill_vol, fill_parent, fill_cmin, fill_cmax, fill_misc;
  DevArr<CmMisc> cm_misc;
  DevArr<float> cm_verts, cm_pos, cm_out_v;
  DevArr<uint32_t> cm_faces, cm_ncells, cm_pair_off,
      cm_fkey, cm_fkey_alt, cm_fval, cm_fval_alt,
      cm_npts, cm_npts_s, cm_fhead, cm_coff, cm_ford,
      cm_cfrag, cm_ccell,
      cm_cells,
      cm_wkey, cm_wkey_alt, cm_wval, cm_wval_alt, cm_whead, cm_wrun,
      cm_head_pos, cm_rep, cm_keep, cm_used, cm_vid, cm_fslot, cm_out_f;
  DevArr<MvMisc> mv_misc;
  DevArr<float> mv_verts, mv_out_v;
  DevArr<long long> mv_cell;
  DevArr<uint32_t> mv_faces, mv_key, mv_key_alt, mv_val, mv_val_alt,
      mv_parent, mv_keep, mv_used, mv_vid, mv_fslot, mv_out_f,
      mv_tab;
  DevArr<uint64_t> enc_size, enc_off, enc_ilen;
  DevArr<uint32_t> enc_box;
  DevArr<float> enc_bbox;
  DevArr<uint8_t> enc_blob;
  DevArr<uint32_t> ol_order, ol_pref;
  DevArr<int32_t> ol_node;
  DevArr<uint64_t> ol_zsize, ol_zoff;
};

enum {
  EV_START = 0,
  EV_H2D_END,
  EV_COUNT_END,
  EV_SCAN_END,
  EV_EMIT_END,
  EV_PARTITION_END,
  EV_WELD_END,
  EV_END,
  EV_SIMPLIFY_END,
  EV_SIMP_FORK,
  EV_SIMP_JOIN,
  EV_MAP_START,
  EV_MAP_END,
  EV_FILL_START,
  EV_FILL_END,
  EV_ENCODE_END,
  EV_COUNT_
};

struct mg_ctx : DeviceBuffers {
  int device = 0;
  hipStream_t stream = nullptr;
  hipStream_t stream2 = nullptr;
  std::mutex lock;
  std::string err;
  mg_stats stats = {};
  bool holes_valid = false;
  int holes_sx = 0, holes_sy = 0, holes_sz = 0, holes_dtype = 0;
  bool counted_valid = false;
  int counted_sx = 0, counted_sy = 0, counted_sz = 0, counted_dtype = 0;
  uint64_t lh_slots = 1ull << 20;
  HostArr<float> h_verts;
  HostArr<uint32_t> h_faces;
  HostArr<uint8_t> h_blob;
  hipEvent_t ev[EV_COUNT_] = {};

  ~mg_ctx() {
    (void)hipSetDevice(device);
    static_cast<DeviceBuffers &>(*this) = DeviceBuffers();
    h_verts.release();
    h_faces.release();
    h_blob.release();
    for (auto &e : ev) if (e) (void)hipEventDestroy(e);
    if (stream2) (void)hipStreamDestroy(stream2);
    if (stream) (void)hipStreamDestroy(stream);
  }
};

static thread_local std::string g_err;

#define SET_ERR(ctx, ...)                                     \
  do {                                                        \
    char _buf[512];                                           \
    snprintf(_buf, sizeof(_buf), __VA_ARGS__);                \
    if (ctx) (ctx)->err = _buf; else g_err = _buf;            \
  } while (0)

#define HIP_TRY(ctx, call, retcode)                           \
  do {                                                        \
    hipError_t _e = (call);                                   \
    if (_e != hipSuccess) {                                   \
      SET_ERR(ctx, "%s failed: %s (%s:%d)", #call,            \
              hipGetErrorString(_e), __FILE__, __LINE__);     \
      return retcode;                                         \
    }                                                         \
  } while (0)

static int ensure_bytes(mg_ctx *c, HostBuf &b, size_t bytes) {
  if (b.cap >= bytes) return 0;
  b.release();
  size_t want = bytes + bytes / 4;
  if (hipHostMalloc(&b.ptr, want) != hipSuccess &&
      hipHostMalloc(&b.ptr, want = bytes) != hipSuccess) {
    SET_ERR(c, "hipHostMalloc(%zu) failed", bytes);
    return 1;
  }
  b.cap = want;
  return 0;
}

static int ensure_bytes(mg_ctx *c, DevBuf &b, size_t bytes) {
  if (b.cap >= bytes) return 0;
  b.release();
  size_t want = bytes + bytes / 4;
  hipError_t e = hipMalloc(&b.ptr, want);
  if (e != hipSuccess) e = hipMalloc(&b.ptr, want = bytes);
  if (e != hipSuccess) {
    SET_ERR(c, "hipMalloc(%zu) failed: %s", bytes, hipGetErrorString(e));
    return 1;
  }
  b.cap = want;
  return 0;
}

template <typename T, typename Owner>
static int ensure(mg_ctx *c, TypedArr<T, Owner> &b, size_t n) {
  return ensure_bytes(c, static_cast<Owner &>(b), n * sizeof(T));
}

template <typename F>
static auto by_dtype(int dtype, F &&f) {
  if (dtype == MG_U64) return f(uint64_t{});
  return f(uint32_t{});
}

template <typename F>
static int rocprim_two_call(mg_ctx *c, DevBuf &tmp, const char *err_size,
                            const char *err_run, int rc, F call) {
  size_t bytes = 0;
  if (call(nullptr, bytes) != hipSuccess) {
    SET_ERR(c, "%s", err_size);
    return rc;
  }
  if (ensure_bytes(c, tmp, bytes)) return rc;
  if (call(tmp.ptr, bytes) != hipSuccess) {
    SET_ERR(c, "%s", err_run);
    return rc;
  }
  return 0;
}

template <typename In>
static int scan_u32(mg_ctx *c, In in, uint32_t *out, size_t n, hipStream_t s,
                    const char *err_size, const char *err_run, int rc) {
  return rocprim_two_call(
      c, c->scan_tmp, err_size, err_run, rc, [&](void *tmp, size_t &bytes) {
        return rocprim::exclusive_scan(tmp, bytes, in, out, 0u, n,
                                       rocprim::plus<uint32_t>(), s);
      });
}

static int scan_u64(mg_ctx *c, const uint64_t *in, uint64_t *out, size_t n,
                    hipStream_t s, const char *err_size, const char *err_run,
                    int rc) {
  return rocprim_two_call(
      c, c->scan_tmp, err_size, err_run, rc, [&](void *tmp, size_t &bytes) {
        return rocprim::exclusive_scan(tmp, bytes, in, out, uint64_t{0}, n,
                                       rocprim::plus<uint64_t>(), s);
      });
}

template <typename In>
static int scan_incl_u32(mg_ctx *c, In in, uint32_t *out, size_t n,
                         hipStream_t s, const char *err_size,
                         const char *err_run, int rc) {
  return rocprim_two_call(
      c, c->scan_tmp, err_size, err_run, rc, [&](void *tmp, size_t &bytes) {
        return rocprim::inclusive_scan(tmp, bytes, in, out, n,
                                       rocprim::plus<uint32_t>(), s);
      });
}

template <typename V>
static int sort_pairs(mg_ctx *c, rocprim::double_buffer<uint32_t> &keys,
                      rocprim::double_buffer<V> &vals, size_t n,
                      unsigned begin_bit, unsigned end_bit, hipStream_t s,
                      const char *err_size, const char *err_run, int rc) {
  return rocprim_two_call(
      c, c->sort_tmp, err_size, err_run, rc, [&](void *tmp, size_t &bytes) {
        return rocprim::radix_sort_pairs(tmp, bytes, keys, vals, n,
                                         begin_bit, end_bit, s);
      });
}

static mg_meshset *alloc_meshset(uint32_t n, uint32_t extra_u32_per_mesh) {
  const size_t meta_off = sizeof(mg_meshset) + sizeof(mg_mesh) * n;
  mg_meshset *ms = (mg_meshset *)calloc(
      1, meta_off + (size_t)n * (24 + 4 * extra_u32_per_mesh) +
             2 * sizeof(void *));
  if (!ms) return nullptr;
  ms->nmeshes = n;
  ms->meshes = (mg_mesh *)((char *)ms + sizeof(mg_meshset));
  ms->labels_arr = (uint64_t *)((char *)ms + meta_off);
  ms->voff_arr = (uint32_t *)(ms->labels_arr + n);
  ms->nv_arr = ms->voff_arr + n;
  ms->foff_arr = ms->nv_arr + n;
  ms->nf_arr = ms->foff_arr + n;
  return ms;
}

static void set_mesh(mg_meshset *ms, uint32_t m, uint64_t label,
                     uint32_t voff, uint32_t nv, uint32_t foff, uint32_t nf) {
  ms->meshes[m] = {label, nv, nf, ms->verts_base + 3ull * voff,
                   ms->faces_base + 3ull * foff};
  ms->labels_arr[m] = label;
  ms->voff_arr[m] = voff;
  ms->nv_arr[m] = nv;
  ms->foff_arr[m] = foff;
  ms->nf_arr[m] = nf;
}
```

### igneous_amd/engine.py

```python
from __future__ import annotations

import ctypes
import os
import threading
from typing import NamedTuple, Optional

import numpy as np

_HERE = os.path.dirname(os.path.abspath(__file__))
SO_PATH = os.path.join(_HERE, "csrc", "libmeshgine.so")

MG_U32, MG_U64 = 0, 1
MG_FLAG_DEVICE_ONLY = 1
MG_FLAG_SKIP_H2D = 2
MG_FLAG_COUNTED = 4
MG_ERR_NOT_COUNTED = 9
MG_MAP_MISS_KEEP, MG_MAP_MISS_ZERO = 0, 1
LABEL_MAP_MAX_ENTRIES = 1 << 24
LABEL_MAP_LDS_MAX = 2048

_EXPORTED_SYMBOLS = [
    "mg_init", "mg_destroy", "mg_mesh_chunk", "mg_mesh_chunk_mapped",
    "mg_mesh_chunk_filled", "mg_mesh_holes", "mg_fill_holes",
    "mg_simplify_mesh", "mg_chunk_mesh", "mg_meshset_free",
    "mg_get_stats", "mg_last_error", "mg_device_count", "mg_version",
    "mg_mesh_chunk_encoded", "mg_blobset_free",
    "mg_count_voxels", "mg_label_counts_free",
    "mg_merge_close_vertices", "mg_retriangulate_mesh",
    "mg_encode_octree_level", "mg_fragset_free",
]
MG_ENC_PRECOMPUTED, MG_ENC_DRACO = 0, 1


class _MgMesh(ctypes.Structure):
    _fields_ = [
        ("label", ctypes.c_uint64),
        ("nverts", ctypes.c_uint32),
        ("ntris", ctypes.c_uint32),
        ("verts", ctypes.POINTER(ctypes.c_float)),
        ("faces", ctypes.POINTER(ctypes.c_uint32)),
    ]


class _MgMeshSet(ctypes.Structure):
    _fields_ = [
        ("nmeshes", ctypes.c_uint32),
        ("meshes", ctypes.POINTER(_MgMesh)),
        ("verts_base", ctypes.POINTER(ctypes.c_float)),
        ("faces_base", ctypes.POINTER(ctypes.c_uint32)),
        ("total_verts", ctypes.c_uint64),
        ("total_tris", ctypes.c_uint64),
        ("labels_arr", ctypes.POINTER(ctypes.c_uint64)),
        ("voff_arr", ctypes.POINTER(ctypes.c_uint32)),
        ("nv_arr", ctypes.POINTER(ctypes.c_uint32)),
        ("foff_arr", ctypes.POINTER(ctypes.c_uint32)),
        ("nf_arr", ctypes.POINTER(ctypes.c_uint32)),
    ]


class _MgLabelMap(ctypes.Structure):
    _fields_ = [
        ("keys", ctypes.c_void_p),
        ("vals", ctypes.c_void_p),
        ("n", ctypes.c_uint64),
        ("miss", ctypes.c_uint32),
    ]


class MgStats(ctypes.Structure):
    _fields_ = [
        ("ms_h2d", ctypes.c_double),
        ("ms_count", ctypes.c_double),
        ("ms_scan", ctypes.c_double),
        ("ms_emit", ctypes.c_double),
        ("ms_partition", ctypes.c_double),
        ("ms_weld", ctypes.c_double),
        ("ms_simplify", ctypes.c_double),
        ("ms_d2h", ctypes.c_double),
        ("ms_total", ctypes.c_double),
        ("total_tris", ctypes.c_uint64),
        ("total_verts", ctypes.c_uint64),
        ("n_labels", ctypes.c_uint64),
        ("bytes_read_algorithmic", ctypes.c_uint64),
        ("ms_labelmap", ctypes.c_double),
    ]

    def as_dict(self) -> dict:
        out = {}
        for klass in reversed(type(self).__mro__):
            for name, _t in klass.__dict__.get("_fields_", ()):
                out[name] = getattr(self, name)
        return out


class MgStatsFill(MgStats):
    _fields_ = [
        ("ms_fill", ctypes.c_double),
    ]


class MgStatsEncode(MgStatsFill):
    _fields_ = [
        ("ms_encode", ctypes.c_double),
    ]


class _MgEncodeParams(ctypes.Structure):
    _fields_ = [
        ("format", ctypes.c_uint32),
        ("shift", ctypes.c_float * 3),
        ("q_origin", ctypes.c_double * 3),
        ("q_range", ctypes.c_double),
        ("q_bits", ctypes.c_uint32),
    ]


class _MgBlobSet(ctypes.Structure):
    _fields_ = [
        ("n", ctypes.c_uint32),
        ("labels", ctypes.POINTER(ctypes.c_uint64)),
        ("offset", ctypes.POINTER(ctypes.c_uint64)),
        ("size", ctypes.POINTER(ctypes.c_uint64)),
        ("nverts", ctypes.POINTER(ctypes.c_uint32)),
        ("ntris", ctypes.POINTER(ctypes.c_uint32)),
        ("bbox", ctypes.POINTER(ctypes.c_float)),
        ("blob", ctypes.POINTER(ctypes.c_uint8)),
        ("blob_bytes", ctypes.c_uint64),
    ]


_ORDER_CELLS_FN = ctypes.CFUNCTYPE(
    ctypes.c_int, ctypes.POINTER(ctypes.c_int32), ctypes.c_uint32,
    ctypes.POINTER(ctypes.c_uint32), ctypes.c_void_p)


class _MgOctreeLevel(ctypes.Structure):
    _fields_ = [
        ("scale", ctypes.c_double * 3),
        ("offset", ctypes.c_double * 3),
        ("retriangulate", ctypes.c_uint32),
        ("upper_scale", ctypes.c_double * 3),
        ("radius", ctypes.c_double),
        ("chunked", ctypes.c_uint32),
        ("q_origin", ctypes.c_double * 3),
        ("q_voffset", ctypes.c_double * 3),
        ("q_cell", ctypes.c_double * 3),
        ("q_bits", ctypes.c_uint32),
        ("order_cells", _ORDER_CELLS_FN),
        ("order_arg", ctypes.c_void_p),
    ]


class _MgFragSet(ctypes.Structure):
    _fields_ = [
        ("n", ctypes.c_uint32),
        ("nodes", ctypes.POINTER(ctypes.c_int32)),
        ("offset", ctypes.POINTER(ctypes.c_uint64)),
        ("size", ctypes.POINTER(ctypes.c_uint64)),
        ("nverts", ctypes.POINTER(ctypes.c_uint32)),
        ("ntris", ctypes.POINTER(ctypes.c_uint32)),
        ("blob", ctypes.POINTER(ctypes.c_uint8)),
        ("blob_bytes", ctypes.c_uint64),
    ]


class EncodedLevel(NamedTuple):
    nodes: tuple
    sizes: list
    blob: bytes


@_ORDER_CELLS_FN
def _order_cells(nodes, n, order, _arg):
    try:
        import functools
        from .tasks.multires import cmp_zorder
        keys = [tuple(nodes[3 * i:3 * i + 3]) for i in range(n)]
        ranked = sorted(range(n), key=functools.cmp_to_key(
            lambda a, b: cmp_zorder(keys[a], keys[b])))
        for r, i in enumerate(ranked):
            order[r] = i
        return 0
    except Exception:
        return 1


class _MgLabelCounts(ctypes.Structure):
    _fields_ = [
        ("n", ctypes.c_uint64),
        ("labels", ctypes.POINTER(ctypes.c_uint64)),
        ("counts", ctypes.POINTER(ctypes.c_uint64)),
    ]


class EncodedChunk:

    def __init__(self, labels, offsets, sizes, nverts, ntris, bboxes, blob):
        self.labels = np.asarray(labels, dtype=np.uint64)
        self.offsets = np.asarray(offsets, dtype=np.uint64)
        self.sizes = np.asarray(sizes, dtype=np.uint64)
        self.nverts = np.asarray(nverts, dtype=np.uint32)
        self.ntris = np.asarray(ntris, dtype=np.uint32)
        self.bboxes = np.asarray(bboxes, dtype=np.float32).reshape(-1, 6)
        self.blob = np.asarray(blob, dtype=np.uint8)
        n = self.labels.shape[0]
        for name in ("offsets", "sizes", "nverts", "ntris", "bboxes"):
            if getattr(self, name).shape[0] != n:
                raise ValueError(f"EncodedChunk: {name} does not have one "
                                 f"entry per label")
        if n and np.any(self.labels[1:] <= self.labels[:-1]):
            raise ValueError("EncodedChunk: labels must be ascending")
        if n and int((self.offsets + self.sizes).max()) > self.blob.shape[0]:
            raise ValueError("EncodedChunk: an entry ends past the blob")

    def __len__(self) -> int:
        return int(self.labels.shape[0])

    def _index(self, label) -> int:
        label = int(label)
        if 0 <= label < (1 << 64):
            i = int(np.searchsorted(self.labels, np.uint64(label)))
            if i < len(self) and int(self.labels[i]) == label:
                return i
        raise KeyError(label)

    def __contains__(self, label) -> bool:
        try:
            self._index(label)
        except KeyError:
            return False
        return True

    def _bytes(self, i: int) -> bytes:
        o = int(self.offsets[i])
        return self.blob[o:o + int(self.sizes[i])].tobytes()

    def __getitem__(self, label) -> bytes:
        return self._bytes(self._index(label))

    def bbox(self, label) -> list:
        return self.bboxes[self._index(label)].tolist()

    def items(self):
        boxes = self.bboxes.tolist()
        for i, label in enumerate(self.labels.tolist()):
            yield label, self._bytes(i), boxes[i]


def _draco_numbers(draco):
    if draco is None:
        raise ValueError("encoding='draco' needs the draco settings "
                         "(quantization_bits / _range / _origin)")
    if draco.get("quantization_origin") is None \
            or draco.get("quantization_range") is None:
        raise ValueError("draco: quantization_origin and quantization_range "
                         "must be given (MeshTask's draco_encoding_settings "
                         "always sets them)")
    origin = np.asarray(draco["quantization_origin"], dtype=np.float64)
    if origin.shape != (3,):
        raise ValueError("draco: quantization_origin must have 3 components")
    rng = float(np.max(draco["quantization_range"]))
    if rng <= 0:
        rng = 1.0
    bits = int(draco.get("quantization_bits", 14))
    return [float(x) for x in origin], rng, bits


_CHUNK_ARGTYPES = [
    ctypes.c_void_p, ctypes.c_void_p,
    ctypes.c_int, ctypes.c_int, ctypes.c_int, ctypes.c_int,
    ctypes.c_float, ctypes.c_float, ctypes.c_float,
    ctypes.c_uint32, ctypes.c_float, ctypes.c_int,
    ctypes.c_uint64, ctypes.c_uint32,
]
_P_MAP = ctypes.POINTER(_MgLabelMap)
_PP_MESHSET = ctypes.POINTER(ctypes.POINTER(_MgMeshSet))
_CHUNK_TAIL_ARGTYPES = {
    "mg_mesh_chunk": [_PP_MESHSET],
    "mg_mesh_chunk_mapped": [_P_MAP, _PP_MESHSET],
    "mg_mesh_chunk_filled": [_P_MAP, ctypes.c_uint32, _PP_MESHSET],
    "mg_mesh_chunk_encoded": [_P_MAP, ctypes.POINTER(_MgEncodeParams),
                              ctypes.POINTER(ctypes.POINTER(_MgBlobSet))],
}

_lib = None
_lib_lock = threading.Lock()


def load_library() -> ctypes.CDLL:
    global _lib
    with _lib_lock:
        if _lib is not None:
            return _lib
        if not os.path.exists(SO_PATH):
            raise RuntimeError(
                f"meshgine HIP engine not built: {SO_PATH} missing. "
                f"Run __graft_entry__.build() (hipcc --offload-arch=gfx950). "
                f"There is no CPU fallback.")
        lib = ctypes.CDLL(SO_PATH)
        for sym in _EXPORTED_SYMBOLS:
            if not hasattr(lib, sym):
                raise RuntimeError(f"{SO_PATH} missing symbol {sym}")
        lib.mg_init.restype = ctypes.c_void_p
        lib.mg_init.argtypes = [ctypes.c_int]
        lib.mg_destroy.argtypes = [ctypes.c_void_p]
        for name, tail in _CHUNK_TAIL_ARGTYPES.items():
            fn = getattr(lib, name)
            fn.restype = ctypes.c_int
            fn.argtypes = _CHUNK_ARGTYPES + tail
        lib.mg_blobset_free.argtypes = [ctypes.POINTER(_MgBlobSet)]
        lib.mg_mesh_holes.restype = ctypes.c_int
        lib.mg_mesh_holes.argtypes = [
            ctypes.c_void_p,
            ctypes.c_float, ctypes.c_float, ctypes.c_float,
            ctypes.c_uint32, ctypes.c_float, ctypes.c_int, ctypes.c_uint32,
            ctypes.POINTER(ctypes.POINTER(_MgMeshSet)),
        ]
        lib.mg_fill_holes.restype = ctypes.c_int
        lib.mg_fill_holes.argtypes = [
            ctypes.c_void_p, ctypes.c_void_p,
            ctypes.c_int, ctypes.c_int, ctypes.c_int, ctypes.c_int,
            ctypes.c_uint32, ctypes.c_void_p, ctypes.c_void_p,
            ctypes.POINTER(ctypes.c_uint32),
        ]
        lib.mg_meshset_free.argtypes = [ctypes.POINTER(_MgMeshSet)]
        lib.mg_count_voxels.restype = ctypes.c_int
        lib.mg_count_voxels.argtypes = [
            ctypes.c_void_p, ctypes.c_void_p,
            ctypes.c_int, ctypes.c_int, ctypes.c_int, ctypes.c_int,
            ctypes.c_uint32,
            ctypes.POINTER(ctypes.POINTER(_MgLabelCounts)),
        ]
        lib.mg_label_counts_free.argtypes = [ctypes.POINTER(_MgLabelCounts)]
        lib.mg_get_stats.restype = ctypes.c_int
        lib.mg_get_stats.argtypes = [ctypes.c_void_p,
                                     ctypes.POINTER(MgStatsEncode)]
        lib.mg_last_error.restype = ctypes.c_char_p
        lib.mg_last_error.argtypes = [ctypes.c_void_p]
        lib.mg_device_count.restype = ctypes.c_int
        lib.mg_version.restype = ctypes.c_char_p
        lib.mg_simplify_mesh.restype = ctypes.c_int
        lib.mg_simplify_mesh.argtypes = [
            ctypes.c_void_p,
            ctypes.c_void_p, ctypes.c_uint32,
            ctypes.c_void_p, ctypes.c_uint32,
            ctypes.c_uint32, ctypes.c_float,
            ctypes.POINTER(ctypes.POINTER(ctypes.c_float)),
            ctypes.POINTER(ctypes.c_uint32),
            ctypes.POINTER(ctypes.POINTER(ctypes.c_uint32)),
            ctypes.POINTER(ctypes.c_uint32),
        ]
        lib.mg_chunk_mesh.restype = ctypes.c_int
        lib.mg_chunk_mesh.argtypes = [
            ctypes.c_void_p,
            ctypes.c_void_p, ctypes.c_uint32,
            ctypes.c_void_p, ctypes.c_uint32,
            ctypes.POINTER(ctypes.c_double), ctypes.POINTER(ctypes.c_double),
            ctypes.POINTER(ctypes.POINTER(_MgMeshSet)),
            ctypes.POINTER(ctypes.POINTER(ctypes.c_uint32)),
        ]
        mesh_out = [
            ctypes.POINTER(ctypes.POINTER(ctypes.c_float)),
            ctypes.POINTER(ctypes.c_uint32),
            ctypes.POINTER(ctypes.POINTER(ctypes.c_uint32)),
            ctypes.POINTER(ctypes.c_uint32),
        ]
        lib.mg_merge_close_vertices.restype = ctypes.c_int
        lib.mg_merge_close_vertices.argtypes = [
            ctypes.c_void_p,
            ctypes.c_void_p, ctypes.c_uint32,
            ctypes.c_void_p, ctypes.c_uint32,
            ctypes.c_double,
        ] + mesh_out
        lib.mg_retriangulate_mesh.restype = ctypes.c_int
        lib.mg_retriangulate_mesh.argtypes = [
            ctypes.c_void_p,
            ctypes.c_void_p, ctypes.c_uint32,
            ctypes.c_void_p, ctypes.c_uint32,
            ctypes.POINTER(ctypes.c_double), ctypes.POINTER(ctypes.c_double),
            ctypes.c_double,
        ] + mesh_out
        lib.mg_encode_octree_level.restype = ctypes.c_int
        lib.mg_encode_octree_level.argtypes = [
            ctypes.c_void_p,
            ctypes.c_void_p, ctypes.c_uint32,
            ctypes.c_void_p, ctypes.c_uint32,
            ctypes.POINTER(_MgOctreeLevel),
            ctypes.POINTER(ctypes.POINTER(_MgFragSet)),
        ]
        lib.mg_fragset_free.argtypes = [ctypes.POINTER(_MgFragSet)]
        _lib = lib
        return lib


def _mg_dtype(arr: np.ndarray) -> int:
    if arr.dtype == np.uint32:
        return MG_U32
    if arr.dtype == np.uint64:
        return MG_U64
    raise ValueError(f"unsupported label dtype {arr.dtype}")


def _np_array(ptr, n: int, width=None, copy: bool = False) -> np.ndarray:
    shape = (n,) if width is None else (n, width)
    if not n:
        return np.zeros(shape, dtype=ptr._type_)
    arr = np.ctypeslib.as_array(ptr, shape=shape)
    return arr.copy() if copy else arr


def _engine(device_id: Optional[int]) -> "Engine":
    if device_id is None:
        device_id = int(os.environ.get("MESHGINE_DEVICE",
                                       os.environ.get("LOCAL_RANK", "0")))
    return Engine.get(device_id)


def _check_dust_global(dust_global, dust_threshold, skip_h2d) -> None:
    if dust_global is None:
        return
    if dust_threshold:
        raise ValueError(
            "dust_global (the global threshold) cannot be combined with "
            "dust_threshold (the chunk-local one)")
    if skip_h2d:
        raise ValueError(
            "dust_global cannot be combined with skip_h2d: it counts and "
            "meshes the volume it is given")
    threshold, lookup = dust_global
    if int(threshold) < 0 or not callable(lookup):
        raise ValueError("dust_global: expected (threshold >= 0, lookup)")


def _fill_level_unsupported(what: str) -> NotImplementedError:
    return NotImplementedError(
        f"{what}: the engine implements levels "
        f"1-2; level 3 needs a multilabel dilation and levels >= 4 "
        f"a merge threshold")


PER_THREAD_CTX = False


class Engine:

    _per_device: dict = {}
    _cls_lock = threading.Lock()

    def __init__(self, device_id: int = 0):
        lib = load_library()
        self.lib = lib
        self.device_id = int(device_id)
        self._lock = threading.Lock()
        self.last_fill_stats = None
        self.ctx = lib.mg_init(self.device_id)
        if not self.ctx:
            raise RuntimeError(
                f"mg_init({device_id}) failed — no usable HIP device. "
                f"The meshgine product path requires an MI355X GPU.")

    @classmethod
    def get(cls, device_id: int = 0) -> "Engine":
        key = (device_id, threading.get_ident()) if PER_THREAD_CTX \
            else device_id
        with cls._cls_lock:
            eng = cls._per_device.get(key)
            if eng is None:
                eng = cls(device_id)
                cls._per_device[key] = eng
            return eng

    def _check(self, rc: int, fn: str) -> None:
        if rc != 0:
            err = self.lib.mg_last_error(self.ctx)
            raise RuntimeError(
                f"{fn} failed rc={rc}: "
                f"{err.decode() if err else 'unknown'}")

    def mesh_chunk(self, labels: np.ndarray, resolution=(1.0, 1.0, 1.0),
                   reduction_factor: int = 0, max_error: float = 40.0,
                   voxel_centered: bool = True,
                   device_only: bool = False,
                   skip_h2d: bool = False,
                   dust_threshold: int = 0,
                   copy: bool = True,
                   label_map=None,
                   fill_holes: int = 0,
                   dust_global=None):
        fill_holes = int(fill_holes)
        if fill_holes < 0 or fill_holes > 2:
            raise _fill_level_unsupported(f"fill_holes={fill_holes}")
        if fill_holes and skip_h2d:
            raise ValueError(
                "fill_holes cannot be combined with skip_h2d: the "
                "resident volume has already been filled")
        if fill_holes:
            copy = True
        _check_dust_global(dust_global, dust_threshold, skip_h2d)
        labels = np.asfortranarray(labels)
        with self._lock:
            if dust_global is not None:
                label_map = self._fold_global_dust(
                    labels, dust_global, label_map)
            args, cmap, _keep = self._chunk_args(
                labels, resolution, reduction_factor, max_error,
                voxel_centered, dust_threshold, device_only, skip_h2d,
                label_map, counted=dust_global is not None)
            if fill_holes:
                fn, tail = "mg_mesh_chunk_filled", (cmap, fill_holes)
            elif cmap is not None:
                fn, tail = "mg_mesh_chunk_mapped", (cmap,)
            else:
                fn, tail = "mg_mesh_chunk", ()
            out = ctypes.POINTER(_MgMeshSet)()
            rc = getattr(self.lib, fn)(*args, *tail, ctypes.byref(out))
            self._check(rc, fn)
            result = self._collect(out, copy)
            if not fill_holes:
                return result
            self.last_fill_stats = self.stats()
            out = ctypes.POINTER(_MgMeshSet)()
            rc = self.lib.mg_mesh_holes(
                self.ctx, *args[6:12],
                MG_FLAG_DEVICE_ONLY if device_only else 0, ctypes.byref(out))
            self._check(rc, "mg_mesh_holes")
            return result, self._collect(out, True)

    def _count_locked(self, labels, skip_h2d: bool = False):
        dtype = _mg_dtype(labels)
        if labels.ndim != 3:
            raise ValueError("count_voxels expects a 3-D volume")
        sx, sy, sz = labels.shape
        out = ctypes.POINTER(_MgLabelCounts)()
        rc = self.lib.mg_count_voxels(
            self.ctx, labels.ctypes.data_as(ctypes.c_void_p),
            sx, sy, sz, dtype, MG_FLAG_SKIP_H2D if skip_h2d else 0,
            ctypes.byref(out))
        self._check(rc, "mg_count_voxels")
        try:
            n = int(out.contents.n)
            return (_np_array(out.contents.labels, n, copy=True),
                    _np_array(out.contents.counts, n, copy=True))
        finally:
            self.lib.mg_label_counts_free(out)

    def count_voxels(self, labels: np.ndarray, skip_h2d: bool = False):
        labels = np.asfortranarray(labels)
        with self._lock:
            return self._count_locked(labels, skip_h2d)

    def _fold_global_dust(self, labels, dust_global, label_map):
        from .remap import fold_dust
        threshold, lookup = dust_global
        values, _ = self._count_locked(labels)
        values = values[values != 0]
        totals = np.asarray(lookup(values), dtype=np.uint64)
        if totals.shape != values.shape:
            raise ValueError("dust_global: lookup must return one count "
                             "per label")
        return fold_dust(label_map, values[totals < np.uint64(threshold)],
                         labels.dtype)

    def _chunk_args(self, labels, resolution, reduction_factor, max_error,
                    voxel_centered, dust_threshold, device_only, skip_h2d,
                    label_map, counted: bool = False):
        labels = np.asfortranarray(labels)
        dtype = _mg_dtype(labels)
        sx, sy, sz = labels.shape
        flags = (MG_FLAG_DEVICE_ONLY if device_only else 0) | \
                (MG_FLAG_SKIP_H2D if skip_h2d else 0) | \
                (MG_FLAG_COUNTED if counted else 0)
        args = (
            self.ctx, labels.ctypes.data_as(ctypes.c_void_p),
            sx, sy, sz, dtype,
            float(resolution[0]), float(resolution[1]), float(resolution[2]),
            int(reduction_factor), float(max_error),
            int(bool(voxel_centered)), int(dust_threshold), flags)
        if label_map is None:
            return args, None, (labels,)
        if skip_h2d:
            raise ValueError(
                "label_map cannot be combined with skip_h2d: the "
                "resident volume has already been mapped")
        keys, vals, miss = label_map
        if miss not in ('keep', 'zero'):
            raise ValueError(f"label_map miss policy {miss!r}: "
                             f"expected 'keep' or 'zero'")
        keys = np.ascontiguousarray(keys, dtype=np.uint64)
        vals = np.ascontiguousarray(vals, dtype=np.uint64)
        if keys.ndim != 1 or keys.shape != vals.shape:
            raise ValueError("label_map keys/vals must be 1-D arrays "
                             "of equal length")
        cmap = _MgLabelMap(
            keys.ctypes.data, vals.ctypes.data, keys.shape[0],
            MG_MAP_MISS_ZERO if miss == 'zero' else MG_MAP_MISS_KEEP)
        return args, ctypes.byref(cmap), (labels, keys, vals, cmap)

    def mesh_chunk_encoded(self, labels: np.ndarray,
                           resolution=(1.0, 1.0, 1.0),
                           reduction_factor: int = 0,
                           max_error: float = 40.0,
                           voxel_centered: bool = True,
                           dust_threshold: int = 0,
                           label_map=None,
                           shift=(0.0, 0.0, 0.0),
                           encoding: str = 'precomputed',
                           draco=None,
                           device_only: bool = False,
                           copy: bool = True,
                           skip_h2d: bool = False,
                           dust_global=None) -> EncodedChunk:
        if encoding not in ('precomputed', 'draco'):
            raise ValueError(f"encoding {encoding!r}: expected "
                             f"'precomputed' or 'draco'")
        params = _MgEncodeParams()
        params.format = (MG_ENC_DRACO if encoding == 'draco'
                         else MG_ENC_PRECOMPUTED)
        shift = np.asarray(shift, dtype=np.float32).reshape(3)
        params.shift[:] = [float(x) for x in shift]
        if encoding == 'draco':
            origin, rng, bits = _draco_numbers(draco)
            params.q_origin[:] = origin
            params.q_range = rng
            if not 0 <= bits < (1 << 32):
                raise ValueError(f"draco: quantization_bits {bits}")
            params.q_bits = bits
        _check_dust_global(dust_global, dust_threshold, skip_h2d)
        labels = np.asfortranarray(labels)
        with self._lock:
            if dust_global is not None:
                label_map = self._fold_global_dust(
                    labels, dust_global, label_map)
            args, cmap, _keep = self._chunk_args(
                labels, resolution, reduction_factor, max_error,
                voxel_centered, dust_threshold, device_only, skip_h2d,
                label_map, counted=dust_global is not None)
            out = ctypes.POINTER(_MgBlobSet)()
            rc = self.lib.mg_mesh_chunk_encoded(
                *args, cmap, ctypes.byref(params), ctypes.byref(out))
            self._check(rc, "mg_mesh_chunk_encoded")
            try:
                bs = out.contents
                n = int(bs.n)
                return EncodedChunk(
                    *(_np_array(p, n, copy=True) for p in (
                        bs.labels, bs.offset, bs.size, bs.nverts, bs.ntris)),
                    _np_array(bs.bbox, n, 6, copy=True),
                    _np_array(bs.blob, int(bs.blob_bytes), copy=copy))
            finally:
                self.lib.mg_blobset_free(out)

    def _collect(self, out, copy: bool) -> dict:
        result = {}
        try:
            ms = out.contents
            n = int(ms.nmeshes)
            if n:
                tv, tt = int(ms.total_verts), int(ms.total_tris)
                if copy:
                    all_v = np.empty((tv, 3), dtype=np.float32)
                    all_f = np.empty((tt, 3), dtype=np.uint32)
                    if tv:
                        ctypes.memmove(all_v.ctypes.data, ms.verts_base,
                                       tv * 12)
                    if tt:
                        ctypes.memmove(all_f.ctypes.data, ms.faces_base,
                                       tt * 12)
                else:
                    all_v = np.ctypeslib.as_array(
                        ms.verts_base, shape=(max(tv, 1), 3))[:tv]
                    all_f = np.ctypeslib.as_array(
                        ms.faces_base, shape=(max(tt, 1), 3))[:tt]
                tables = (_np_array(p, n).tolist() for p in (
                    ms.labels_arr, ms.voff_arr, ms.nv_arr, ms.foff_arr,
                    ms.nf_arr))
                result = {
                    lab: (all_v[vo:vo + kv], all_f[fo:fo + kf])
                    for lab, vo, kv, fo, kf in zip(*tables)
                }
        finally:
            self.lib.mg_meshset_free(out)
        return result

    def fill_holes(self, labels: np.ndarray, level: int = 1):
        level = int(level)
        if level not in (1, 2):
            raise _fill_level_unsupported(f"fill_holes level {level}")
        labels = np.asfortranarray(labels)
        dtype = _mg_dtype(labels)
        if labels.ndim != 3:
            raise ValueError("fill_holes expects a 3-D volume")
        sx, sy, sz = labels.shape
        filled = np.empty(labels.shape, dtype=labels.dtype, order="F")
        holes = np.empty(labels.shape, dtype=labels.dtype, order="F")
        rounds = ctypes.c_uint32()
        with self._lock:
            rc = self.lib.mg_fill_holes(
                self.ctx, labels.ctypes.data_as(ctypes.c_void_p),
                sx, sy, sz, dtype, level,
                filled.ctypes.data_as(ctypes.c_void_p),
                holes.ctypes.data_as(ctypes.c_void_p), ctypes.byref(rounds))
            self._check(rc, "mg_fill_holes")
        return filled, holes, int(rounds.value)

    def simplify_mesh(self, verts: np.ndarray, faces: np.ndarray,
                      reduction_factor: int,
                      max_error: float = 1e30):
        v = np.ascontiguousarray(verts, dtype=np.float32)
        f = np.ascontiguousarray(faces, dtype=np.uint32)
        ov = ctypes.POINTER(ctypes.c_float)()
        of = ctypes.POINTER(ctypes.c_uint32)()
        onv = ctypes.c_uint32()
        ont = ctypes.c_uint32()
        with self._lock:
            rc = self.lib.mg_simplify_mesh(
                self.ctx,
                v.ctypes.data_as(ctypes.c_void_p), v.shape[0],
                f.ctypes.data_as(ctypes.c_void_p), f.shape[0],
                int(reduction_factor), float(max_error),
                ctypes.byref(ov), ctypes.byref(onv),
                ctypes.byref(of), ctypes.byref(ont))
            self._check(rc, "mg_simplify_mesh")
            out_v = _np_array(ov, onv.value, 3, copy=True)
            out_f = _np_array(of, ont.value, 3, copy=True)
        return out_v, out_f

    def chunk_mesh(self, verts: np.ndarray, faces: np.ndarray,
                   scale, offset) -> dict:
        v = np.ascontiguousarray(verts, dtype=np.float32).reshape(-1, 3)
        f = np.ascontiguousarray(faces, dtype=np.uint32).reshape(-1, 3)
        sc = (ctypes.c_double * 3)(*[float(x) for x in scale])
        off = (ctypes.c_double * 3)(*[float(x) for x in offset])
        out = ctypes.POINTER(_MgMeshSet)()
        order = ctypes.POINTER(ctypes.c_uint32)()
        with self._lock:
            rc = self.lib.mg_chunk_mesh(
                self.ctx,
                v.ctypes.data_as(ctypes.c_void_p), v.shape[0],
                f.ctypes.data_as(ctypes.c_void_p), f.shape[0],
                sc, off, ctypes.byref(out), ctypes.byref(order))
            self._check(rc, "mg_chunk_mesh")
            n = int(out.contents.nmeshes)
            idx = _np_array(order, n).tolist()
            by_label = self._collect(out, True)
        labels = list(by_label)
        mask = (1 << 21) - 1
        bias = 1 << 20
        result = {}
        for i in idx:
            lab = labels[i]
            key = (((lab >> 42) & mask) - bias, ((lab >> 21) & mask) - bias,
                   (lab & mask) - bias)
            result[key] = by_label[lab]
        return result

    def _weld_call(self, fn: str, verts, faces, radius, *grid):
        radius = float(radius)
        if not np.isfinite(radius) or radius <= 0:
            raise ValueError(f"radius {radius}: must be finite and > 0")
        v = np.ascontiguousarray(verts, dtype=np.float32).reshape(-1, 3)
        f = np.ascontiguousarray(faces, dtype=np.uint32).reshape(-1, 3)
        grid = [(ctypes.c_double * 3)(*[float(x) for x in g]) for g in grid]
        ov = ctypes.POINTER(ctypes.c_float)()
        of = ctypes.POINTER(ctypes.c_uint32)()
        onv = ctypes.c_uint32()
        ont = ctypes.c_uint32()
        with self._lock:
            rc = getattr(self.lib, fn)(
                self.ctx,
                v.ctypes.data_as(ctypes.c_void_p), v.shape[0],
                f.ctypes.data_as(ctypes.c_void_p), f.shape[0],
                *grid, radius,
                ctypes.byref(ov), ctypes.byref(onv),
                ctypes.byref(of), ctypes.byref(ont))
            self._check(rc, fn)
            if not ov:
                return v.copy(), f.copy()
            return (_np_array(ov, onv.value, 3, copy=True),
                    _np_array(of, ont.value, 3, copy=True))

    def merge_close_vertices(self, verts: np.ndarray, faces: np.ndarray,
                             radius: float = 1e-5):
        return self._weld_call("mg_merge_close_vertices", verts, faces,
                               radius)

    def retriangulate_mesh(self, verts: np.ndarray, faces: np.ndarray,
                           scale, offset, radius: float = 1e-5):
        return self._weld_call("mg_retriangulate_mesh", verts, faces, radius,
                               scale, offset)

    def encode_octree_level(self, verts: np.ndarray, faces: np.ndarray, *,
                            scale, offset, upper_scale=None,
                            radius: float = 1e-5, chunked: bool = True,
                            q_origin, q_voffset, q_cell,
                            q_bits: int) -> EncodedLevel:
        v = np.ascontiguousarray(verts, dtype=np.float32).reshape(-1, 3)
        f = np.ascontiguousarray(faces, dtype=np.uint32).reshape(-1, 3)
        vec = ctypes.c_double * 3
        lv = _MgOctreeLevel()
        lv.scale = vec(*[float(x) for x in scale])
        lv.offset = vec(*[float(x) for x in offset])
        lv.retriangulate = 0 if upper_scale is None else 1
        lv.upper_scale = vec(*[float(x) for x in (
            scale if upper_scale is None else upper_scale)])
        lv.radius = float(radius)
        lv.chunked = 1 if chunked else 0
        lv.q_origin = vec(*[float(x) for x in q_origin])
        lv.q_voffset = vec(*[float(x) for x in q_voffset])
        lv.q_cell = vec(*[float(x) for x in q_cell])
        q_bits = int(q_bits)
        lv.q_bits = q_bits if 0 <= q_bits < 2 ** 32 else 0
        lv.order_cells = _order_cells
        out = ctypes.POINTER(_MgFragSet)()
        with self._lock:
            rc = self.lib.mg_encode_octree_level(
                self.ctx,
                v.ctypes.data_as(ctypes.c_void_p), v.shape[0],
                f.ctypes.data_as(ctypes.c_void_p), f.shape[0],
                ctypes.byref(lv), ctypes.byref(out))
            self._check(rc, "mg_encode_octree_level")
            try:
                fs = out.contents
                n = int(fs.n)
                nodes = _np_array(fs.nodes, 3 * n).reshape(n, 3).tolist()
                sizes = _np_array(fs.size, n).tolist()
                nbytes = int(fs.blob_bytes)
                blob = ctypes.string_at(fs.blob, nbytes) if nbytes else b""
            finally:
                self.lib.mg_fragset_free(out)
        return EncodedLevel(tuple(tuple(p) for p in nodes), sizes, blob)

    def stats(self) -> dict:
        s = MgStatsEncode()
        rc = self.lib.mg_get_stats(self.ctx, ctypes.byref(s))
        if rc != 0:
            raise RuntimeError("mg_get_stats failed")
        return s.as_dict()


def mesh_chunk(labels: np.ndarray, resolution=(1.0, 1.0, 1.0),
               reduction_factor: int = 0, max_error: float = 40.0,
               voxel_centered: bool = True, device_id: Optional[int] = None,
               dust_threshold: int = 0,
               copy: bool = True, label_map=None, fill_holes: int = 0,
               dust_global=None):
    return _engine(device_id).mesh_chunk(
        labels, resolution, reduction_factor, max_error, voxel_centered,
        dust_threshold=dust_threshold, copy=copy, label_map=label_map,
        fill_holes=fill_holes, dust_global=dust_global)


mesh_chunk.handles_dust = True
mesh_chunk.handles_label_map = True
mesh_chunk.handles_fill_holes = True
mesh_chunk.handles_dust_global = True


def mesh_chunk_encoded(labels: np.ndarray, resolution=(1.0, 1.0, 1.0),
                       reduction_factor: int = 0, max_error: float = 40.0,
                       voxel_centered: bool = True,
                       device_id: Optional[int] = None,
                       dust_threshold: int = 0, label_map=None,
                       shift=(0.0, 0.0, 0.0), encoding: str = 'precomputed',
                       draco=None, copy: bool = True,
                       dust_global=None) -> EncodedChunk:
    return _engine(device_id).mesh_chunk_encoded(
        labels, resolution, reduction_factor, max_error, voxel_centered,
        dust_threshold=dust_threshold, label_map=label_map, shift=shift,
        encoding=encoding, draco=draco, copy=copy, dust_global=dust_global)


mesh_chunk.encode_chunk = mesh_chunk_encoded
mesh_chunk_encoded.formats = ('draco',)


def count_voxels(labels: np.ndarray, device_id: Optional[int] = None):
    return _engine(device_id).count_voxels(labels)


mesh_chunk.count_voxels = count_voxels


def fill_holes(labels: np.ndarray, level: int = 1,
               device_id: Optional[int] = None):
    return _engine(device_id).fill_holes(labels, level)


def chunk_mesh(mesh, scale, offset, device_id: Optional[int] = None):
    from .meshes import Mesh
    cells = _engine(device_id).chunk_mesh(
        mesh.vertices, mesh.faces, scale, offset)
    return {key: Mesh(v, f, id=mesh.id) for key, (v, f) in cells.items()}


def merge_close_vertices(mesh, radius: float = 1e-5,
                         device_id: Optional[int] = None):
    from .meshes import Mesh
    v, f = _engine(device_id).merge_close_vertices(
        mesh.vertices, mesh.faces, radius)
    return Mesh(v, f, id=mesh.id)


def retriangulate_mesh(mesh, scale, offset, radius: float = 1e-5,
                       device_id: Optional[int] = None):
    from .meshes import Mesh
    v, f = _engine(device_id).retriangulate_mesh(
        mesh.vertices, mesh.faces, scale, offset, radius)
    return Mesh(v, f, id=mesh.id)


def encode_octree_level(mesh, *, scale, offset, upper_scale=None,
                        radius: float = 1e-5, chunked: bool = True,
                        q_origin, q_voffset, q_cell, q_bits: int,
                        device_id: Optional[int] = None) -> EncodedLevel:
    return _engine(device_id).encode_octree_level(
        mesh.vertices, mesh.faces, scale=scale, offset=offset,
        upper_scale=upper_scale, radius=radius, chunked=chunked,
        q_origin=q_origin, q_voffset=q_voffset, q_cell=q_cell,
        q_bits=q_bits)


def simplify_mesh(mesh, target_count: int, max_error: float = 1e30,
                  device_id: Optional[int] = None):
    from .meshes import Mesh
    nt = int(mesh.faces.shape[0])
    target = max(int(target_count), 1)
    if nt <= target:
        return Mesh(mesh.vertices.copy(), mesh.faces.copy(), id=mesh.id)
    rf = max(nt // target, 2)
    v, f = _engine(device_id).simplify_mesh(
        mesh.vertices, mesh.faces, rf, max_error)
    return Mesh(v, f, id=mesh.id)
```

### include/meshgine.h

```cpp
#ifndef MESHGINE_H
#define MESHGINE_H

#include <stdint.h>

#ifdef __cplusplus
extern "C" {
#endif

typedef struct mg_ctx mg_ctx;

#define MG_U32 0
#define MG_U64 1

#define MG_FLAG_NONE        0u
#define MG_FLAG_DEVICE_ONLY 1u
#define MG_FLAG_SKIP_H2D    2u
#define MG_FLAG_COUNTED     4u

typedef struct {
  uint64_t  label;
  uint32_t  nverts;
  uint32_t  ntris;
  float    *verts;
  uint32_t *faces;
} mg_mesh;

typedef struct {
  uint32_t  nmeshes;
  mg_mesh  *meshes;
  float    *verts_base;
  uint32_t *faces_base;
  uint64_t  total_verts;
  uint64_t  total_tris;
  uint64_t *labels_arr;
  uint32_t *voff_arr;
  uint32_t *nv_arr;
  uint32_t *foff_arr;
  uint32_t *nf_arr;
} mg_meshset;

typedef struct {
  double ms_h2d;
  double ms_count;
  double ms_scan;
  double ms_emit;
  double ms_partition;
  double ms_weld;
  double ms_simplify;
  double ms_d2h;
  double ms_total;
  uint64_t total_tris;
  uint64_t total_verts;
  uint64_t n_labels;
  uint64_t bytes_read_algorithmic;
  double ms_labelmap;
  double ms_fill;
  double ms_encode;
} mg_stats;

#define MG_ENC_PRECOMPUTED 0u
#define MG_ENC_DRACO       1u
typedef struct {
  uint32_t format;
  float    shift[3];
  double   q_origin[3];
  double   q_range;
  uint32_t q_bits;
} mg_encode_params;

typedef struct {
  uint32_t  n;
  uint64_t *labels;
  uint64_t *offset;
  uint64_t *size;
  uint32_t *nverts;
  uint32_t *ntris;
  float    *bbox;
  uint8_t  *blob;
  uint64_t  blob_bytes;
} mg_blobset;

#define MG_MAP_MISS_KEEP 0u
#define MG_MAP_MISS_ZERO 1u
typedef struct {
  const uint64_t *keys;
  const uint64_t *vals;
  uint64_t        n;
  uint32_t        miss;
} mg_label_map;

mg_ctx  *mg_init(int device_id);
void     mg_destroy(mg_ctx *ctx);

int mg_mesh_chunk(mg_ctx *ctx, const void *labels,
                  int sx, int sy, int sz, int dtype,
                  float rx, float ry, float rz,
                  uint32_t reduction_factor, float max_error,
                  int voxel_centered, uint64_t dust_threshold,
                  uint32_t flags,
                  mg_meshset **out);

int mg_mesh_chunk_mapped(mg_ctx *ctx, const void *labels,
                         int sx, int sy, int sz, int dtype,
                         float rx, float ry, float rz,
                         uint32_t reduction_factor, float max_error,
                         int voxel_centered, uint64_t dust_threshold,
                         uint32_t flags,
                         const mg_label_map *map,
                         mg_meshset **out);

int mg_mesh_chunk_filled(mg_ctx *ctx, const void *labels,
                         int sx, int sy, int sz, int dtype,
                         float rx, float ry, float rz,
                         uint32_t reduction_factor, float max_error,
                         int voxel_centered, uint64_t dust_threshold,
                         uint32_t flags,
                         const mg_label_map *map,
                         uint32_t fill_level,
                         mg_meshset **out);

int mg_mesh_chunk_encoded(mg_ctx *ctx, const void *labels,
                          int sx, int sy, int sz, int dtype,
                          float rx, float ry, float rz,
                          uint32_t reduction_factor, float max_error,
                          int voxel_centered, uint64_t dust_threshold,
                          uint32_t flags,
                          const mg_label_map *map,
                          const mg_encode_params *params,
                          mg_blobset **out);

void mg_blobset_free(mg_blobset *bs);

int mg_mesh_holes(mg_ctx *ctx, float rx, float ry, float rz,
                  uint32_t reduction_factor, float max_error,
                  int voxel_centered, uint32_t flags,
                  mg_meshset **out);

int mg_fill_holes(mg_ctx *ctx, const void *labels,
                  int sx, int sy, int sz, int dtype, uint32_t level,
                  void *filled_out, void *holes_out, uint32_t *rounds_out);

void mg_meshset_free(mg_meshset *ms);

typedef struct {
  uint64_t  n;
  uint64_t *labels;
  uint64_t *counts;
} mg_label_counts;

int mg_count_voxels(mg_ctx *ctx, const void *labels,
                    int sx, int sy, int sz, int dtype, uint32_t flags,
                    mg_label_counts **out);

void mg_label_counts_free(mg_label_counts *lc);

int mg_simplify_mesh(mg_ctx *ctx,
                     const float *verts, uint32_t nverts,
                     const uint32_t *faces, uint32_t ntris,
                     uint32_t reduction_factor, float max_error,
                     const float **out_verts, uint32_t *out_nverts,
                     const uint32_t **out_faces, uint32_t *out_ntris);

int mg_chunk_mesh(mg_ctx *ctx,
                  const float *verts, uint32_t nverts,
                  const uint32_t *faces, uint32_t ntris,
                  const double scale[3], const double offset[3],
                  mg_meshset **out, const uint32_t **out_order);

int mg_merge_close_vertices(mg_ctx *ctx,
                            const float *verts, uint32_t nverts,
                            const uint32_t *faces, uint32_t ntris,
                            double radius,
                            const float **out_verts, uint32_t *out_nverts,
                            const uint32_t **out_faces, uint32_t *out_ntris);

int mg_retriangulate_mesh(mg_ctx *ctx,
                          const float *verts, uint32_t nverts,
                          const uint32_t *faces, uint32_t ntris,
                          const double scale[3], const double offset[3],
                          double radius,
                          const float **out_verts, uint32_t *out_nverts,
                          const uint32_t **out_faces, uint32_t *out_ntris);

typedef struct mg_octree_level {
  double   scale[3];
  double   offset[3];
  uint32_t retriangulate;
  double   upper_scale[3];
  double   radius;
  uint32_t chunked;
  double   q_origin[3];
  double   q_voffset[3];
  double   q_cell[3];
  uint32_t q_bits;
  int (*order_cells)(const int32_t *nodes, uint32_t n, uint32_t *order,
                     void *arg);
  void    *order_arg;
} mg_octree_level;

typedef struct mg_fragset {
  uint32_t  n;
  int32_t  *nodes;
  uint64_t *offset;
  uint64_t *size;
  uint32_t *nverts;
  uint32_t *ntris;
  const uint8_t *blob;
  uint64_t  blob_bytes;
} mg_fragset;

int mg_encode_octree_level(mg_ctx *ctx,
                           const float *verts, uint32_t nverts,
                           const uint32_t *faces, uint32_t ntris,
                           const mg_octree_level *lv, mg_fragset **out);

void mg_fragset_free(mg_fragset *fs);

int mg_get_stats(mg_ctx *ctx, mg_stats *out);

const char *mg_last_error(mg_ctx *ctx);

int mg_device_count(void);
const char *mg_version(void);

#ifdef __cplusplus
}
#endif

#endif
```

Before: 12260 Mvox/s.

## Weld vertices per label in LDS with capacity bands, table fallback for large labels

```diff
diff --git a/igneous_amd/csrc/mc_table.h b/igneous_amd/csrc/mc_table.h
--- a/igneous_amd/csrc/mc_table.h
+++ b/igneous_amd/csrc/mc_table.h
@@ -822,6 +822,265 @@
   6, 4, 2, 0, 5, 4, 1, 0, 3, 2, 1, 0,
 };
 
+MC_TABLE_QUAL unsigned short MC_ITEM_FIRST[256][8] = {
+  {0x0000, 0x0000, 0x0000, 0x0000, 0x0000, 0x0000, 0x0000, 0x0000},
+  {0x0007, 0x0001, 0x0002, 0x0000, 0x0004, 0x0000, 0x0000, 0x0000},
+  {0x0007, 0x0007, 0x0004, 0x0004, 0x0002, 0x0002, 0x0000, 0x0000},
+  {0x0027, 0x0024, 0x0021, 0x0020, 0x0006, 0x0004, 0x0000, 0x0000},
+  {0x0007, 0x0001, 0x0007, 0x0001, 0x0002, 0x0000, 0x0002, 0x0000},
+  {0x0027, 0x0003, 0x0006, 0x0002, 0x0024, 0x0000, 0x0004, 0x0000},
+  {0x003f, 0x000f, 0x003c, 0x000c, 0x0012, 0x0002, 0x0010, 0x0000},
+  {0x0127, 0x0121, 0x0103, 0x0101, 0x0026, 0x0020, 0x0002, 0x0000},
+  {0x0007, 0x0007, 0x0007, 0x0007, 0x0004, 0x0004, 0x0004, 0x0004},
+  {0x003f, 0x0039, 0x003a, 0x0038, 0x0024, 0x0020, 0x0020, 0x0020},
+  {0x0027, 0x0027, 0x0024, 0x0024, 0x0006, 0x0006, 0x0004, 0x0004},
+  {0x0127, 0x0121, 0x0103, 0x0101, 0x0124, 0x0120, 0x0100, 0x0100},
+  {0x0027, 0x0006, 0x0027, 0x0006, 0x0024, 0x0004, 0x0024, 0x0004},
+  {0x0127, 0x0007, 0x0026, 0x0006, 0x0124, 0x0004, 0x0024, 0x0004},
+  {0x0127, 0x0007, 0x0124, 0x0004, 0x0026, 0x0006, 0x0024, 0x0004},
+  {0x0027, 0x0006, 0x0024, 0x0004, 0x0027, 0x0006, 0x0024, 0x0004},
+  {0x0007, 0x0001, 0x0004, 0x0000, 0x0007, 0x0001, 0x0004, 0x0000},
+  {0x0027, 0x0021, 0x0006, 0x0000, 0x0024, 0x0020, 0x0004, 0x0000},
+  {0x003f, 0x000f, 0x0024, 0x0004, 0x003a, 0x000a, 0x0020, 0x0000},
+  {0x0127, 0x0007, 0x0124, 0x0004, 0x0103, 0x0003, 0x0100, 0x0000},
+  {0x003f, 0x0009, 0x0027, 0x0001, 0x003a, 0x0008, 0x0022, 0x0000},
+  {0x0127, 0x0103, 0x0026, 0x0002, 0x0124, 0x0100, 0x0024, 0x0000},
+  {0x01ff, 0x004f, 0x013c, 0x000c, 0x01d2, 0x0042, 0x0110, 0x0000},
+  {0x0927, 0x0921, 0x0807, 0x0801, 0x0126, 0x0120, 0x0006, 0x0000},
+  {0x003f, 0x000f, 0x0027, 0x0007, 0x003c, 0x000c, 0x0024, 0x0004},
+  {0x01e7, 0x01e1, 0x01c6, 0x01c0, 0x0124, 0x0120, 0x0104, 0x0100},
+  {0x01e7, 0x0067, 0x0124, 0x0024, 0x01c6, 0x0046, 0x0104, 0x0004},
+  {0x0927, 0x0921, 0x0807, 0x0801, 0x0924, 0x0920, 0x0804, 0x0800},
+  {0x013f, 0x0031, 0x013c, 0x0030, 0x0127, 0x0021, 0x0124, 0x0020},
+  {0x0927, 0x0807, 0x0126, 0x0006, 0x0924, 0x0804, 0x0124, 0x0004},
+  {0x0f27, 0x0207, 0x0924, 0x0004, 0x0e26, 0x0206, 0x0824, 0x0004},
+  {0x0127, 0x0007, 0x0124, 0x0004, 0x0127, 0x0007, 0x0124, 0x0004},
+  {0x0007, 0x0007, 0x0002, 0x0002, 0x0007, 0x0007, 0x0002, 0x0002},
+  {0x003f, 0x0039, 0x0012, 0x0010, 0x003c, 0x0038, 0x0010, 0x0010},
+  {0x0027, 0x0027, 0x0024, 0x0024, 0x0006, 0x0006, 0x0004, 0x0004},
+  {0x0127, 0x0007, 0x0026, 0x0006, 0x0103, 0x0003, 0x0002, 0x0002},
+  {0x003f, 0x0039, 0x0017, 0x0011, 0x003a, 0x0038, 0x0012, 0x0010},
+  {0x01e7, 0x01c3, 0x0086, 0x0082, 0x01e4, 0x01c0, 0x0084, 0x0080},
+  {0x01e7, 0x0067, 0x01e4, 0x0064, 0x0086, 0x0006, 0x0084, 0x0004},
+  {0x0927, 0x0921, 0x0903, 0x0901, 0x0126, 0x0120, 0x0102, 0x0100},
+  {0x003f, 0x003f, 0x0017, 0x0017, 0x003c, 0x003c, 0x0014, 0x0014},
+  {0x01ff, 0x01f9, 0x00ba, 0x00b8, 0x01e4, 0x01e0, 0x00a0, 0x00a0},
+  {0x0127, 0x0127, 0x0124, 0x0124, 0x0026, 0x0026, 0x0024, 0x0024},
+  {0x0927, 0x0921, 0x0903, 0x0901, 0x0924, 0x0920, 0x0900, 0x0900},
+  {0x013f, 0x0037, 0x013a, 0x0032, 0x0127, 0x0027, 0x0122, 0x0022},
+  {0x0f27, 0x0e07, 0x0426, 0x0406, 0x0f24, 0x0e04, 0x0424, 0x0404},
+  {0x0927, 0x0027, 0x0924, 0x0024, 0x0126, 0x0026, 0x0124, 0x0024},
+  {0x0127, 0x0007, 0x0026, 0x0006, 0x0127, 0x0007, 0x0026, 0x0006},
+  {0x0027, 0x0006, 0x0003, 0x0002, 0x0027, 0x0006, 0x0003, 0x0002},
+  {0x0127, 0x0121, 0x0026, 0x0020, 0x0124, 0x0120, 0x0024, 0x0020},
+  {0x0127, 0x0121, 0x0124, 0x0120, 0x0026, 0x0020, 0x0024, 0x0020},
+  {0x0027, 0x0024, 0x0027, 0x0024, 0x0006, 0x0004, 0x0006, 0x0004},
+  {0x013f, 0x0031, 0x001f, 0x0011, 0x013a, 0x0030, 0x001a, 0x0010},
+  {0x0927, 0x0903, 0x0126, 0x0102, 0x0924, 0x0900, 0x0124, 0x0100},
+  {0x0f27, 0x0321, 0x0f24, 0x0320, 0x0426, 0x0020, 0x0424, 0x0020},
+  {0x0127, 0x0121, 0x0127, 0x0121, 0x0026, 0x0020, 0x0026, 0x0020},
+  {0x013f, 0x0037, 0x001f, 0x0017, 0x013c, 0x0034, 0x001c, 0x0014},
+  {0x0f27, 0x0f21, 0x0e26, 0x0e20, 0x0924, 0x0920, 0x0824, 0x0820},
+  {0x0927, 0x0921, 0x0924, 0x0920, 0x0126, 0x0120, 0x0124, 0x0120},
+  {0x0127, 0x0121, 0x0127, 0x0121, 0x0124, 0x0120, 0x0124, 0x0120},
+  {0x09e7, 0x0186, 0x00e7, 0x0086, 0x09e4, 0x0184, 0x00e4, 0x0084},
+  {0x4927, 0x4807, 0x0926, 0x0806, 0x4924, 0x4804, 0x0924, 0x0804},
+  {0x4927, 0x0121, 0x4924, 0x0120, 0x0926, 0x0120, 0x0924, 0x0120},
+  {0x0027, 0x0006, 0x0027, 0x0006, 0x0027, 0x0006, 0x0027, 0x0006},
+  {0x0007, 0x0001, 0x0007, 0x0001, 0x0007, 0x0001, 0x0007, 0x0001},
+  {0x003f, 0x0009, 0x003a, 0x0008, 0x003c, 0x0008, 0x0038, 0x0008},
+  {0x003f, 0x000f, 0x003c, 0x000c, 0x003a, 0x000a, 0x0038, 0x0008},
+  {0x013f, 0x0121, 0x010f, 0x0101, 0x0037, 0x0021, 0x0007, 0x0001},
+  {0x0027, 0x0003, 0x0027, 0x0003, 0x0006, 0x0002, 0x0006, 0x0002},
+  {0x0127, 0x0007, 0x0026, 0x0006, 0x0124, 0x0004, 0x0024, 0x0004},
+  {0x013f, 0x001f, 0x013c, 0x001c, 0x0032, 0x0012, 0x0030, 0x0010},
+  {0x0927, 0x0903, 0x0807, 0x0803, 0x0126, 0x0102, 0x0006, 0x0002},
+  {0x003f, 0x000f, 0x003f, 0x000f, 0x003c, 0x000c, 0x003c, 0x000c},
+  {0x01ff, 0x0079, 0x01fa, 0x0078, 0x01e4, 0x0060, 0x01e0, 0x0060},
+  {0x01e7, 0x0067, 0x01e4, 0x0064, 0x01c6, 0x0046, 0x01c4, 0x0044},
+  {0x0f27, 0x0321, 0x0f03, 0x0301, 0x0f24, 0x0320, 0x0f00, 0x0300},
+  {0x0127, 0x0121, 0x0127, 0x0121, 0x0103, 0x0101, 0x0103, 0x0101},
+  {0x0927, 0x0027, 0x0126, 0x0026, 0x0924, 0x0024, 0x0124, 0x0024},
+  {0x0927, 0x0027, 0x0924, 0x0024, 0x0126, 0x0026, 0x0124, 0x0024},
+  {0x0127, 0x0121, 0x0103, 0x0101, 0x0127, 0x0121, 0x0103, 0x0101},
+  {0x0027, 0x0021, 0x0024, 0x0020, 0x0027, 0x0021, 0x0024, 0x0020},
+  {0x0127, 0x0121, 0x0026, 0x0020, 0x0124, 0x0120, 0x0024, 0x0020},
+  {0x013f, 0x010f, 0x0124, 0x0104, 0x013a, 0x010a, 0x0120, 0x0100},
+  {0x0927, 0x0807, 0x0924, 0x0804, 0x0903, 0x0803, 0x0900, 0x0800},
+  {0x0127, 0x0007, 0x0103, 0x0003, 0x0026, 0x0006, 0x0002, 0x0002},
+  {0x0027, 0x0027, 0x0006, 0x0006, 0x0024, 0x0024, 0x0004, 0x0004},
+  {0x093f, 0x003f, 0x081c, 0x001c, 0x0132, 0x0032, 0x0010, 0x0010},
+  {0x0127, 0x0127, 0x0103, 0x0103, 0x0026, 0x0026, 0x0002, 0x0002},
+  {0x013f, 0x010f, 0x0127, 0x0107, 0x013c, 0x010c, 0x0124, 0x0104},
+  {0x0f27, 0x0f21, 0x0e26, 0x0e20, 0x0924, 0x0920, 0x0824, 0x0820},
+  {0x09e7, 0x0867, 0x0924, 0x0824, 0x09c6, 0x0846, 0x0904, 0x0804},
+  {0x4927, 0x4921, 0x4027, 0x4021, 0x4924, 0x4920, 0x4024, 0x4020},
+  {0x0927, 0x0921, 0x0924, 0x0920, 0x0903, 0x0901, 0x0900, 0x0900},
+  {0x0127, 0x0127, 0x0026, 0x0026, 0x0124, 0x0124, 0x0024, 0x0024},
+  {0x4927, 0x0127, 0x4024, 0x0024, 0x0926, 0x0126, 0x0024, 0x0024},
+  {0x0027, 0x0027, 0x0024, 0x0024, 0x0027, 0x0027, 0x0024, 0x0024},
+  {0x003f, 0x000f, 0x003a, 0x000a, 0x003f, 0x000f, 0x003a, 0x000a},
+  {0x01ff, 0x0079, 0x01d2, 0x0050, 0x01fc, 0x0078, 0x01d0, 0x0050},
+  {0x01e7, 0x0067, 0x01e4, 0x0064, 0x01c6, 0x0046, 0x01c4, 0x0044},
+  {0x0f27, 0x0207, 0x0e26, 0x0206, 0x0f03, 0x0203, 0x0e02, 0x0202},
+  {0x01e7, 0x01c3, 0x00a7, 0x0083, 0x01c6, 0x01c2, 0x0086, 0x0082},
+  {0x0f27, 0x0e07, 0x0426, 0x0406, 0x0f24, 0x0e04, 0x0424, 0x0404},
+  {0x09e7, 0x00e7, 0x09e4, 0x00e4, 0x0186, 0x0086, 0x0184, 0x0084},
+  {0x4927, 0x4903, 0x4807, 0x4803, 0x0926, 0x0902, 0x0806, 0x0802},
+  {0x01ff, 0x007f, 0x01d7, 0x0057, 0x01fc, 0x007c, 0x01d4, 0x0054},
+  {0x0fff, 0x03f9, 0x0eba, 0x02b8, 0x0fe4, 0x03e0, 0x0ea0, 0x02a0},
+  {0x0f27, 0x0327, 0x0f24, 0x0324, 0x0e26, 0x0226, 0x0e24, 0x0224},
+  {0x7927, 0x1921, 0x7903, 0x1901, 0x7924, 0x1920, 0x7900, 0x1900},
+  {0x093f, 0x090f, 0x093a, 0x090a, 0x081f, 0x080f, 0x081a, 0x080a},
+  {0x7927, 0x7027, 0x2126, 0x2026, 0x7924, 0x7024, 0x2124, 0x2024},
+  {0x4927, 0x0127, 0x4924, 0x0124, 0x0926, 0x0126, 0x0924, 0x0124},
+  {0x0927, 0x0027, 0x0126, 0x0026, 0x0927, 0x0027, 0x0126, 0x0026},
+  {0x0127, 0x0007, 0x0103, 0x0003, 0x0127, 0x0007, 0x0103, 0x0003},
+  {0x0927, 0x0921, 0x0126, 0x0120, 0x0924, 0x0920, 0x0124, 0x0120},
+  {0x0927, 0x0921, 0x0924, 0x0920, 0x0126, 0x0120, 0x0124, 0x0120},
+  {0x0127, 0x0007, 0x0127, 0x0007, 0x0103, 0x0003, 0x0103, 0x0003},
+  {0x0927, 0x0027, 0x0807, 0x0007, 0x0126, 0x0026, 0x0006, 0x0006},
+  {0x0127, 0x0127, 0x0026, 0x0026, 0x0124, 0x0124, 0x0024, 0x0024},
+  {0x4927, 0x4921, 0x4924, 0x4920, 0x0902, 0x0900, 0x0900, 0x0900},
+  {0x0027, 0x0027, 0x0027, 0x0027, 0x0006, 0x0006, 0x0006, 0x0006},
+  {0x093f, 0x003f, 0x081f, 0x001f, 0x093c, 0x003c, 0x081c, 0x001c},
+  {0x7927, 0x7921, 0x7126, 0x7120, 0x4924, 0x4920, 0x4124, 0x4120},
+  {0x4927, 0x4921, 0x4924, 0x4920, 0x0926, 0x0920, 0x0924, 0x0920},
+  {0x0927, 0x0921, 0x0927, 0x0921, 0x0924, 0x0920, 0x0924, 0x0920},
+  {0x4927, 0x4807, 0x4903, 0x4803, 0x4027, 0x4007, 0x4003, 0x4003},
+  {0x0927, 0x0927, 0x0126, 0x0126, 0x0924, 0x0924, 0x0124, 0x0124},
+  {0x003f, 0x0039, 0x003c, 0x0038, 0x003a, 0x0038, 0x0038, 0x0038},
+  {0x0007, 0x0007, 0x0007, 0x0007, 0x0007, 0x0007, 0x0007, 0x0007},
+  {0x0007, 0x0007, 0x0007, 0x0007, 0x0007, 0x0007, 0x0007, 0x0007},
+  {0x003f, 0x0039, 0x003a, 0x0038, 0x003c, 0x0038, 0x0038, 0x0038},
+  {0x003f, 0x003f, 0x003c, 0x003c, 0x003a, 0x003a, 0x0038, 0x0038},
+  {0x013f, 0x0127, 0x010f, 0x0107, 0x0037, 0x0027, 0x0007, 0x0007},
+  {0x003f, 0x0039, 0x003f, 0x0039, 0x003a, 0x0038, 0x003a, 0x0038},
+  {0x01e7, 0x01c3, 0x01c6, 0x01c2, 0x01e4, 0x01c0, 0x01c4, 0x01c0},
+  {0x01ff, 0x01cf, 0x01fc, 0x01cc, 0x01d2, 0x01c2, 0x01d0, 0x01c0},
+  {0x0f27, 0x0f21, 0x0f03, 0x0f01, 0x0e26, 0x0e20, 0x0e02, 0x0e00},
+  {0x0027, 0x0027, 0x0027, 0x0027, 0x0024, 0x0024, 0x0024, 0x0024},
+  {0x013f, 0x0139, 0x013a, 0x0138, 0x0124, 0x0120, 0x0120, 0x0120},
+  {0x0127, 0x0127, 0x0124, 0x0124, 0x0026, 0x0026, 0x0024, 0x0024},
+  {0x0927, 0x0921, 0x0903, 0x0901, 0x0924, 0x0920, 0x0900, 0x0900},
+  {0x0127, 0x0121, 0x0127, 0x0121, 0x0103, 0x0101, 0x0103, 0x0101},
+  {0x0927, 0x0027, 0x0126, 0x0026, 0x0924, 0x0024, 0x0124, 0x0024},
+  {0x0927, 0x0027, 0x0924, 0x0024, 0x0126, 0x0026, 0x0124, 0x0024},
+  {0x0127, 0x0121, 0x0103, 0x0101, 0x0127, 0x0121, 0x0103, 0x0101},
+  {0x003f, 0x0039, 0x003c, 0x0038, 0x003f, 0x0039, 0x003c, 0x0038},
+  {0x01e7, 0x01e1, 0x01c6, 0x01c0, 0x01e4, 0x01e0, 0x01c4, 0x01c0},
+  {0x01ff, 0x01cf, 0x01e4, 0x01c4, 0x01fa, 0x01ca, 0x01e0, 0x01c0},
+  {0x0f27, 0x0e07, 0x0f24, 0x0e04, 0x0f03, 0x0e03, 0x0f00, 0x0e00},
+  {0x01ff, 0x01c9, 0x01e7, 0x01c1, 0x01fa, 0x01c8, 0x01e2, 0x01c0},
+  {0x0f27, 0x0f03, 0x0e26, 0x0e02, 0x0f24, 0x0f00, 0x0e24, 0x0e00},
+  {0x0fff, 0x0e4f, 0x0f3c, 0x0e0c, 0x0fd2, 0x0e42, 0x0f10, 0x0e00},
+  {0x7927, 0x7921, 0x7807, 0x7801, 0x7126, 0x7120, 0x7006, 0x7000},
+  {0x01e7, 0x0067, 0x0127, 0x0027, 0x01e4, 0x0064, 0x0124, 0x0024},
+  {0x09e7, 0x09e1, 0x09c6, 0x09c0, 0x0924, 0x0920, 0x0904, 0x0900},
+  {0x0f27, 0x0327, 0x0924, 0x0124, 0x0e26, 0x0226, 0x0824, 0x0024},
+  {0x4927, 0x4921, 0x4807, 0x4801, 0x4924, 0x4920, 0x4804, 0x4800},
+  {0x093f, 0x0909, 0x093c, 0x0908, 0x081f, 0x0809, 0x081c, 0x0808},
+  {0x4927, 0x4027, 0x0926, 0x0026, 0x4924, 0x4024, 0x0924, 0x0024},
+  {0x7927, 0x1027, 0x4924, 0x0024, 0x7126, 0x1026, 0x4124, 0x0024},
+  {0x0927, 0x0027, 0x0924, 0x0024, 0x0927, 0x0027, 0x0924, 0x0024},
+  {0x0027, 0x0027, 0x0006, 0x0006, 0x0027, 0x0027, 0x0006, 0x0006},
+  {0x013f, 0x0139, 0x0032, 0x0030, 0x013c, 0x0138, 0x0030, 0x0030},
+  {0x0127, 0x0127, 0x0124, 0x0124, 0x0026, 0x0026, 0x0024, 0x0024},
+  {0x0927, 0x0027, 0x0126, 0x0026, 0x0807, 0x0007, 0x0006, 0x0006},
+  {0x013f, 0x0139, 0x0037, 0x0031, 0x013a, 0x0138, 0x0032, 0x0030},
+  {0x09e7, 0x09c3, 0x0186, 0x0182, 0x09e4, 0x09c0, 0x0184, 0x0180},
+  {0x0f27, 0x0327, 0x0f24, 0x0324, 0x0426, 0x0026, 0x0424, 0x0024},
+  {0x4927, 0x4921, 0x4903, 0x4901, 0x0926, 0x0920, 0x0902, 0x0900},
+  {0x0127, 0x0127, 0x0103, 0x0103, 0x0124, 0x0124, 0x0100, 0x0100},
+  {0x093f, 0x0939, 0x081a, 0x0818, 0x0924, 0x0920, 0x0800, 0x0800},
+  {0x0027, 0x0027, 0x0024, 0x0024, 0x0006, 0x0006, 0x0004, 0x0004},
+  {0x0127, 0x0121, 0x0103, 0x0101, 0x0124, 0x0120, 0x0100, 0x0100},
+  {0x0927, 0x0903, 0x0126, 0x0102, 0x0807, 0x0803, 0x0006, 0x0002},
+  {0x4927, 0x0127, 0x0902, 0x0102, 0x4924, 0x0124, 0x0900, 0x0100},
+  {0x0127, 0x0007, 0x0124, 0x0004, 0x0026, 0x0006, 0x0024, 0x0004},
+  {0x0027, 0x0003, 0x0006, 0x0002, 0x0027, 0x0003, 0x0006, 0x0002},
+  {0x0127, 0x0007, 0x0103, 0x0003, 0x0127, 0x0007, 0x0103, 0x0003},
+  {0x0927, 0x0921, 0x0126, 0x0120, 0x0924, 0x0920, 0x0124, 0x0120},
+  {0x0927, 0x0921, 0x0924, 0x0920, 0x0126, 0x0120, 0x0124, 0x0120},
+  {0x0127, 0x0007, 0x0127, 0x0007, 0x0103, 0x0003, 0x0103, 0x0003},
+  {0x093f, 0x0039, 0x081f, 0x0019, 0x093a, 0x0038, 0x081a, 0x0018},
+  {0x4927, 0x4903, 0x0926, 0x0902, 0x4924, 0x4900, 0x0924, 0x0900},
+  {0x7927, 0x1921, 0x7924, 0x1920, 0x2126, 0x0120, 0x2124, 0x0120},
+  {0x0927, 0x0921, 0x0927, 0x0921, 0x0126, 0x0120, 0x0126, 0x0120},
+  {0x0927, 0x0807, 0x0903, 0x0803, 0x0924, 0x0804, 0x0900, 0x0800},
+  {0x4927, 0x4921, 0x0926, 0x0920, 0x4024, 0x4020, 0x0024, 0x0020},
+  {0x0127, 0x0121, 0x0124, 0x0120, 0x0026, 0x0020, 0x0024, 0x0020},
+  {0x0027, 0x0021, 0x0027, 0x0021, 0x0024, 0x0020, 0x0024, 0x0020},
+  {0x4927, 0x0121, 0x4027, 0x0021, 0x4903, 0x0101, 0x4003, 0x0001},
+  {0x003f, 0x000f, 0x003a, 0x000a, 0x003c, 0x000c, 0x0038, 0x0008},
+  {0x0927, 0x0021, 0x0924, 0x0020, 0x0126, 0x0020, 0x0124, 0x0020},
+  {0x0007, 0x0001, 0x0007, 0x0001, 0x0007, 0x0001, 0x0007, 0x0001},
+  {0x0027, 0x0024, 0x0027, 0x0024, 0x0027, 0x0024, 0x0027, 0x0024},
+  {0x013f, 0x0121, 0x013a, 0x0120, 0x013c, 0x0120, 0x0138, 0x0120},
+  {0x013f, 0x0127, 0x013c, 0x0124, 0x013a, 0x0122, 0x0138, 0x0120},
+  {0x09e7, 0x0924, 0x09e1, 0x0920, 0x09c6, 0x0904, 0x09c0, 0x0900},
+  {0x0127, 0x0007, 0x0127, 0x0007, 0x0026, 0x0006, 0x0026, 0x0006},
+  {0x0927, 0x0027, 0x0126, 0x0026, 0x0924, 0x0024, 0x0124, 0x0024},
+  {0x093f, 0x003f, 0x093c, 0x003c, 0x0132, 0x0032, 0x0130, 0x0030},
+  {0x4927, 0x4807, 0x4027, 0x4007, 0x0926, 0x0806, 0x0026, 0x0006},
+  {0x0127, 0x0007, 0x0127, 0x0007, 0x0124, 0x0004, 0x0124, 0x0004},
+  {0x093f, 0x0039, 0x093a, 0x0038, 0x0924, 0x0020, 0x0920, 0x0020},
+  {0x0927, 0x0807, 0x0924, 0x0804, 0x0126, 0x0006, 0x0124, 0x0004},
+  {0x4927, 0x0121, 0x4903, 0x0101, 0x4924, 0x0120, 0x4900, 0x0100},
+  {0x0027, 0x0006, 0x0027, 0x0006, 0x0024, 0x0004, 0x0024, 0x0004},
+  {0x0127, 0x0007, 0x0026, 0x0006, 0x0124, 0x0004, 0x0024, 0x0004},
+  {0x0127, 0x0007, 0x0124, 0x0004, 0x0026, 0x0006, 0x0024, 0x0004},
+  {0x0027, 0x0024, 0x0021, 0x0020, 0x0027, 0x0024, 0x0021, 0x0020},
+  {0x0127, 0x0121, 0x0124, 0x0120, 0x0127, 0x0121, 0x0124, 0x0120},
+  {0x0927, 0x0921, 0x0126, 0x0120, 0x0924, 0x0920, 0x0124, 0x0120},
+  {0x093f, 0x090f, 0x0924, 0x0904, 0x093a, 0x090a, 0x0920, 0x0900},
+  {0x4927, 0x4807, 0x4924, 0x4804, 0x4903, 0x4803, 0x4900, 0x4800},
+  {0x0927, 0x0027, 0x0807, 0x0007, 0x0126, 0x0026, 0x0006, 0x0006},
+  {0x0127, 0x0127, 0x0026, 0x0026, 0x0124, 0x0124, 0x0024, 0x0024},
+  {0x493f, 0x013f, 0x403c, 0x003c, 0x0932, 0x0132, 0x0030, 0x0030},
+  {0x0927, 0x0927, 0x0807, 0x0807, 0x0126, 0x0126, 0x0006, 0x0006},
+  {0x0927, 0x0027, 0x0807, 0x0007, 0x0924, 0x0024, 0x0804, 0x0004},
+  {0x4927, 0x4921, 0x0926, 0x0920, 0x4804, 0x4800, 0x0804, 0x0800},
+  {0x4927, 0x4027, 0x4804, 0x4004, 0x0926, 0x0026, 0x0804, 0x0004},
+  {0x003f, 0x0039, 0x0027, 0x0021, 0x003c, 0x0038, 0x0024, 0x0020},
+  {0x0127, 0x0121, 0x0124, 0x0120, 0x0103, 0x0101, 0x0100, 0x0100},
+  {0x0027, 0x0027, 0x0006, 0x0006, 0x0024, 0x0024, 0x0004, 0x0004},
+  {0x0927, 0x0027, 0x0804, 0x0004, 0x0126, 0x0026, 0x0004, 0x0004},
+  {0x0007, 0x0007, 0x0004, 0x0004, 0x0007, 0x0007, 0x0004, 0x0004},
+  {0x0127, 0x0121, 0x0026, 0x0020, 0x0127, 0x0121, 0x0026, 0x0020},
+  {0x093f, 0x0909, 0x0132, 0x0100, 0x093c, 0x0908, 0x0130, 0x0100},
+  {0x0927, 0x0903, 0x0924, 0x0900, 0x0126, 0x0102, 0x0124, 0x0100},
+  {0x4927, 0x0121, 0x0926, 0x0120, 0x4027, 0x0021, 0x0026, 0x0020},
+  {0x0927, 0x0027, 0x0903, 0x0003, 0x0126, 0x0026, 0x0102, 0x0002},
+  {0x4927, 0x0127, 0x0806, 0x0006, 0x4924, 0x0124, 0x0804, 0x0004},
+  {0x4927, 0x4903, 0x4924, 0x4900, 0x0806, 0x0802, 0x0804, 0x0800},
+  {0x003f, 0x000f, 0x0017, 0x0007, 0x003a, 0x000a, 0x0012, 0x0002},
+  {0x0927, 0x0027, 0x0903, 0x0003, 0x0924, 0x0024, 0x0900, 0x0000},
+  {0x493f, 0x0139, 0x481a, 0x0018, 0x4924, 0x0120, 0x4800, 0x0000},
+  {0x0127, 0x0103, 0x0124, 0x0100, 0x0026, 0x0002, 0x0024, 0x0000},
+  {0x0927, 0x0021, 0x0903, 0x0001, 0x0924, 0x0020, 0x0900, 0x0000},
+  {0x0127, 0x0121, 0x0026, 0x0020, 0x0103, 0x0101, 0x0002, 0x0000},
+  {0x0927, 0x0027, 0x0102, 0x0002, 0x0924, 0x0024, 0x0100, 0x0000},
+  {0x0027, 0x0003, 0x0024, 0x0000, 0x0006, 0x0002, 0x0004, 0x0000},
+  {0x0007, 0x0001, 0x0002, 0x0000, 0x0007, 0x0001, 0x0002, 0x0000},
+  {0x0027, 0x0024, 0x0006, 0x0004, 0x0027, 0x0024, 0x0006, 0x0004},
+  {0x0127, 0x0121, 0x0026, 0x0020, 0x0124, 0x0120, 0x0024, 0x0020},
+  {0x0127, 0x0121, 0x0124, 0x0120, 0x0026, 0x0020, 0x0024, 0x0020},
+  {0x0027, 0x0024, 0x0027, 0x0024, 0x0006, 0x0004, 0x0006, 0x0004},
+  {0x0127, 0x0007, 0x0103, 0x0003, 0x0026, 0x0006, 0x0002, 0x0002},
+  {0x0027, 0x0027, 0x0006, 0x0006, 0x0024, 0x0024, 0x0004, 0x0004},
+  {0x0927, 0x0921, 0x0924, 0x0920, 0x0102, 0x0100, 0x0100, 0x0100},
+  {0x0007, 0x0007, 0x0007, 0x0007, 0x0002, 0x0002, 0x0002, 0x0002},
+  {0x0127, 0x0007, 0x0103, 0x0003, 0x0124, 0x0004, 0x0100, 0x0000},
+  {0x0927, 0x0921, 0x0126, 0x0120, 0x0804, 0x0800, 0x0004, 0x0000},
+  {0x0027, 0x0021, 0x0024, 0x0020, 0x0006, 0x0000, 0x0004, 0x0000},
+  {0x0007, 0x0001, 0x0007, 0x0001, 0x0004, 0x0000, 0x0004, 0x0000},
+  {0x0027, 0x0006, 0x0003, 0x0002, 0x0024, 0x0004, 0x0000, 0x0000},
+  {0x0007, 0x0007, 0x0002, 0x0002, 0x0004, 0x0004, 0x0000, 0x0000},
+  {0x0007, 0x0001, 0x0004, 0x0000, 0x0002, 0x0000, 0x0000, 0x0000},
+  {0x0000, 0x0000, 0x0000, 0x0000, 0x0000, 0x0000, 0x0000, 0x0000},
+};
+
 MC_TABLE_QUAL unsigned char MC_EDGE_CORNERS[12][2] = {
   {0, 1},
   {2, 3},
diff --git a/igneous_amd/csrc/meshgine.hip b/igneous_amd/csrc/meshgine.hip
--- a/igneous_amd/csrc/meshgine.hip
+++ b/igneous_amd/csrc/meshgine.hip
@@ -3,6 +3,7 @@
 
 #include <algorithm>
 #include <atomic>
+#include <type_traits>
 #include <vector>
 
 #define MC_TABLE_QUAL __device__ static const
@@ -395,204 +396,320 @@
   }
 }
 
-struct ItemTris {
-  __device__ uint32_t operator()(uint2 rec) const {
-    return MC_TRI_COUNT[rec.y & 255u];
+__device__ __forceinline__ uint32_t item_first_bits(uint2 rec) {
+  return MC_ITEM_FIRST[rec.y & 255u][~(rec.y >> 11) & 7u];
+}
+struct ItemCounts {
+  __device__ uint64_t operator()(uint2 rec) const {
+    return ((uint64_t)__popc(item_first_bits(rec)) << 32) |
+           MC_TRI_COUNT[rec.y & 255u];
   }
 };
-struct ItemTrisVia {
+struct ItemCountsVia {
   const uint2 *recs;
-  __device__ uint32_t operator()(uint32_t o) const {
-    return MC_TRI_COUNT[recs[o].y & 255u];
+  __device__ uint64_t operator()(uint32_t o) const {
+    return ItemCounts{}(recs[o]);
   }
 };
 
-#define WELD_FIRST_BLK 256
+#define WELD_BLK 256
 __global__ void k_label_ranges(const uint32_t *__restrict__ item_lab,
-                               uint32_t *__restrict__ itoff,
+                               uint64_t *__restrict__ itscan,
                                uint32_t *__restrict__ tri_off,
+                               uint32_t *__restrict__ lab_item,
+                               uint32_t *__restrict__ vbase,
                                uint32_t *__restrict__ blk_item,
-                               uint64_t nitems, uint64_t ntris,
-                               uint32_t nlabels) {
+                               uint64_t nitems, uint32_t nlabels) {
   uint64_t i = (uint64_t)blockIdx.x * blockDim.x + threadIdx.x;
   if (i >= nitems) return;
-  uint32_t a = 0;
+  uint64_t sa = 0;
   if (i == 0) {
-    itoff[0] = 0;
-    tri_off[item_lab[0]] = 0;
-    tri_off[nlabels] = (uint32_t)ntris;
+    itscan[0] = 0;
+    const uint64_t tot = itscan[nitems];
+    tri_off[nlabels] = (uint32_t)tot;
+    vbase[nlabels] = (uint32_t)(tot >> 32);
+    lab_item[nlabels] = (uint32_t)nitems;
   } else {
-    a = itoff[i];
-    if (item_lab[i] != item_lab[i - 1]) tri_off[item_lab[i]] = a;
-  }
-  const uint32_t b = itoff[i + 1];
-  const uint32_t m = (a + WELD_FIRST_BLK - 1) / WELD_FIRST_BLK;
-  if (m * WELD_FIRST_BLK < b) blk_item[m] = (uint32_t)i;
-}
-
-
-
-__global__ __launch_bounds__(WELD_FIRST_BLK) void k_weld_first(
+    sa = itscan[i];
+  }
+  const uint32_t a = (uint32_t)sa;
+  if (i == 0 || item_lab[i] != item_lab[i - 1]) {
+    const uint32_t l = item_lab[i];
+    tri_off[l] = a;
+    lab_item[l] = (uint32_t)i;
+    vbase[l] = (uint32_t)(sa >> 32);
+  }
+  const uint32_t b = (uint32_t)itscan[i + 1];
+  const uint32_t m = (a + WELD_BLK - 1) / WELD_BLK;
+  if (m * WELD_BLK < b) blk_item[m] = (uint32_t)i;
+}
+
+
+struct WeldGeom {
+  uint32_t usx, usxy;
+  float rx, ry, rz, shift;
+};
+
+__device__ __forceinline__ void write_slot_vertex(float *__restrict__ verts,
+                                                  uint64_t vid, uint32_t slot,
+                                                  const WeldGeom &g) {
+  const uint32_t eslot = slot >> 1;
+  const uint32_t axis = eslot % 3u;
+  const uint32_t lin = eslot / 3u;
+  const uint32_t vz = lin / g.usxy;
+  const uint32_t rem = lin - vz * g.usxy;
+  const uint32_t vy = rem / g.usx;
+  const uint32_t vx = rem - vy * g.usx;
+  const float dx = (float)(2 * vx + (axis == 0));
+  const float dy = (float)(2 * vy + (axis == 1));
+  const float dz = (float)(2 * vz + (axis == 2));
+  verts[3 * vid + 0] = (0.5f * dx + g.shift) * g.rx;
+  verts[3 * vid + 1] = (0.5f * dy + g.shift) * g.ry;
+  verts[3 * vid + 2] = (0.5f * dz + g.shift) * g.rz;
+}
+
+struct WeldTile {
+  uint32_t off[WELD_BLK + 1];
+  uint32_t voff[WELD_BLK];
+  uint2 rec[WELD_BLK];
+  uint8_t item[WELD_BLK];
+  uint32_t next;
+};
+
+struct WeldItem {
+  uint64_t sc, sc_end;
+  uint2 rec;
+};
+
+__device__ __forceinline__ WeldItem load_weld_item(
+    const uint2 *__restrict__ item_recs, const uint32_t *__restrict__ order,
+    const uint64_t *__restrict__ itscan, uint64_t first, uint64_t i_end) {
+  const uint64_t it = first + threadIdx.x;
+  WeldItem w;
+  w.sc = itscan[std::min<uint64_t>(it, i_end)];
+  w.sc_end = 0;
+  if (threadIdx.x == 0)
+    w.sc_end = itscan[std::min<uint64_t>(first + WELD_BLK, i_end)];
+  w.rec = make_uint2(0, 0);
+  if (it < i_end) w.rec = order ? item_recs[order[it]] : item_recs[it];
+  return w;
+}
+
+template <bool NEXT>
+__device__ __forceinline__ void stage_weld_tile(WeldTile &w,
+                                                const WeldItem &li,
+                                                uint32_t t0, uint32_t t1) {
+  w.off[threadIdx.x] = (uint32_t)li.sc;
+  w.voff[threadIdx.x] = (uint32_t)(li.sc >> 32);
+  w.rec[threadIdx.x] = li.rec;
+  if (threadIdx.x == 0) w.off[WELD_BLK] = (uint32_t)li.sc_end;
+  __syncthreads();
+  const uint32_t a = w.off[threadIdx.x], b = w.off[threadIdx.x + 1];
+  const uint32_t lo = std::max(a, t0), hi = std::min(b, t1);
+  for (uint32_t q = lo; q < hi; ++q) w.item[q - t0] = (uint8_t)threadIdx.x;
+  if (NEXT && a <= t1) {
+    if (b > t1) w.next = threadIdx.x;
+    else if (threadIdx.x == WELD_BLK - 1) w.next = WELD_BLK;
+  }
+  __syncthreads();
+}
+
+struct TriCorners {
+  uint32_t slot[3];
+  uint32_t first;
+  uint32_t id[3];
+};
+
+__device__ __forceinline__ TriCorners decode_tri(
+    const WeldTile &w, const uint16_t *s_pack, const uint16_t *s_ifirst,
+    const uint32_t *s_comb, uint32_t j, uint32_t t) {
+  const uint2 rec = w.rec[j];
+  const uint32_t tin = t - w.off[j];
+  const uint32_t mask = rec.y & 255u;
+  const uint32_t pk = s_pack[mask * MC_MAX_TRIS + tin];
+  const uint32_t ib = s_ifirst[mask * 8u + (~(rec.y >> 11) & 7u)];
+  const uint32_t cl3 = rec.x * 3u;
+  TriCorners c;
+  c.first = (ib >> (3u * tin)) & 7u;
+  #pragma unroll
+  for (int v = 0; v < 3; ++v) {
+    const uint32_t nib = (pk >> (5 * v)) & 31u;
+    c.slot[v] = ((cl3 + s_comb[nib & 15u]) << 1) | (nib >> 4);
+    c.id[v] = w.voff[j] + (uint32_t)__popc(ib & ((1u << (3u * tin + v)) - 1u));
+  }
+  return c;
+}
+
+__device__ __forceinline__ void stage_item_first(uint16_t *s_ifirst) {
+  for (int k = threadIdx.x; k < 256 * 8; k += blockDim.x)
+    s_ifirst[k] = MC_ITEM_FIRST[k >> 3][k & 7];
+}
+
+#define WELD_LDS_CAP 8192u
+#define WELD_EMPTY 0xffffffffu
+
+template <uint32_t CAP>
+__global__ __launch_bounds__(WELD_BLK) void k_weld_label(
     const uint2 *__restrict__ item_recs,
     const uint32_t *__restrict__ order,
+    const uint64_t *__restrict__ itscan,
+    const uint32_t *__restrict__ lab_item,
+    const uint32_t *__restrict__ tri_off,
+    const uint32_t *__restrict__ vbase,
+    uint32_t *__restrict__ lab_sorted,
+    float *__restrict__ verts, uint32_t *__restrict__ faces,
+    WeldGeom g, uint32_t lo_cap, uint32_t *__restrict__ err) {
+  constexpr uint32_t TAB = 2 * CAP;
+  static_assert((TAB & (TAB - 1)) == 0 && CAP <= 65536, "");
+  constexpr uint32_t SHIFT = 32 - __builtin_ctz(TAB);
+  __shared__ uint32_t s_key[TAB];
+  __shared__ uint16_t s_val[TAB];
+  __shared__ uint16_t s_pack[256 * MC_MAX_TRIS];
+  __shared__ uint16_t s_ifirst[256 * 8];
+  __shared__ uint32_t s_comb[12];
+  __shared__ WeldTile s_tile;
+  const uint32_t l = blockIdx.x;
+  const uint32_t vb = vbase[l];
+  const uint32_t nv = vbase[l + 1] - vb;
+  if (nv <= lo_cap || nv > CAP) return;
+  const uint32_t t_end = tri_off[l + 1];
+  const uint64_t i_end = lab_item[l + 1];
+  uint64_t first = lab_item[l];
+  WeldItem li = load_weld_item(item_recs, order, itscan, first, i_end);
+  stage_decode_tables(s_pack, s_comb, g.usx, g.usxy);
+  stage_item_first(s_ifirst);
+  for (uint32_t k = threadIdx.x; k < TAB; k += WELD_BLK) s_key[k] = WELD_EMPTY;
+  for (uint32_t t0 = tri_off[l]; t0 < t_end; t0 += WELD_BLK) {
+    const uint32_t t1 = std::min(t0 + WELD_BLK, t_end);
+    stage_weld_tile<true>(s_tile, li, t0, t1);
+    if (t1 < t_end) {
+      first += s_tile.next;
+      li = load_weld_item(item_recs, order, itscan, first, i_end);
+    }
+    const uint32_t t = t0 + threadIdx.x;
+    TriCorners c;
+    if (t < t1) {
+      c = decode_tri(s_tile, s_pack, s_ifirst, s_comb,
+                     s_tile.item[threadIdx.x], t);
+      #pragma unroll
+      for (int v = 0; v < 3; ++v) {
+        if (!((c.first >> v) & 1u)) continue;
+        uint32_t pos = (c.slot[v] * 2654435761u) >> SHIFT;
+        uint32_t n = 0;
+        for (; n < TAB; ++n) {
+          if (atomicCAS(&s_key[pos], WELD_EMPTY, c.slot[v]) == WELD_EMPTY)
+            break;
+          pos = (pos + 1) & (TAB - 1);
+        }
+        if (n == TAB) atomicOr(err, 1u);
+        else s_val[pos] = (uint16_t)(c.id[v] - vb);
+        write_slot_vertex(verts, c.id[v], c.slot[v], g);
+      }
+    }
+    __syncthreads();
+    if (t < t1) {
+      #pragma unroll
+      for (int v = 0; v < 3; ++v) {
+        uint32_t id = c.id[v] - vb;
+        if (!((c.first >> v) & 1u)) {
+          uint32_t pos = (c.slot[v] * 2654435761u) >> SHIFT;
+          uint32_t n = 0, key;
+          while ((key = s_key[pos]) != c.slot[v] && key != WELD_EMPTY &&
+                 ++n < TAB)
+            pos = (pos + 1) & (TAB - 1);
+          id = s_val[pos];
+          if (key != c.slot[v]) atomicOr(err, 2u);
+        }
+        faces[3ull * t + v] = id;
+      }
+      if (lab_sorted) lab_sorted[t] = l;
+    }
+  }
+}
+
+__global__ void k_weld_plan(const uint32_t *__restrict__ tri_off,
+                            const uint32_t *__restrict__ vbase,
+                            uint32_t nlabels, uint32_t *__restrict__ blk_list,
+                            uint32_t *__restrict__ nlist,
+                            uint32_t *__restrict__ ntable) {
+  const uint64_t gid = (uint64_t)blockIdx.x * blockDim.x + threadIdx.x;
+  const uint32_t lane = threadIdx.x & (WAVE - 1);
+  const uint64_t l = gid / WAVE;
+  if (l >= nlabels) return;
+  if (vbase[l + 1] - vbase[l] <= WELD_LDS_CAP) return;
+  uint32_t b0 = tri_off[l] / WELD_BLK;
+  const uint32_t b1 = (tri_off[l + 1] - 1) / WELD_BLK;
+  for (uint64_t m = l; m > 0 && tri_off[m] > b0 * WELD_BLK; --m)
+    if (vbase[m] - vbase[m - 1] > WELD_LDS_CAP) {
+      ++b0;
+      break;
+    }
+  const uint32_t n = b1 + 1 - b0;
+  uint32_t base = 0;
+  if (lane == 0) {
+    base = atomicAdd(nlist, n);
+    atomicAdd(ntable, 1u);
+  }
+  base = __shfl(base, 0);
+  for (uint32_t k = lane; k < n; k += WAVE) blk_list[base + k] = b0 + k;
+}
+
+__global__ __launch_bounds__(WELD_BLK) void k_weld_first(
+    const uint2 *__restrict__ item_recs, const uint32_t *__restrict__ order,
     const uint32_t *__restrict__ item_lab,
-    const uint32_t *__restrict__ itoff,
+    const uint64_t *__restrict__ itscan,
     const uint32_t *__restrict__ blk_item,
+    const uint32_t *__restrict__ blk_list,
+    const uint32_t *__restrict__ vbase,
+    uint4 *__restrict__ quads,
+    uint32_t *__restrict__ wminp,
     uint32_t *__restrict__ lab_sorted,
-    uint32_t *__restrict__ slots_sorted,
-    uint32_t *__restrict__ wminp,
-    unsigned long long *__restrict__ bits,
-    int64_t sx, int64_t sxy,
-    uint64_t nitems, uint64_t ntris, uint64_t nwords) {
+    float *__restrict__ verts, WeldGeom g, uint64_t nitems, uint32_t ntris) {
   __shared__ uint16_t s_pack[256 * MC_MAX_TRIS];
-  __shared__ uint8_t s_first[256 * MC_MAX_TRIS];
+  __shared__ uint16_t s_ifirst[256 * 8];
   __shared__ uint32_t s_comb[12];
-  __shared__ uint32_t s_need[12];
-  __shared__ uint32_t s_off[WELD_FIRST_BLK + 1];
-  __shared__ uint2 s_rec[WELD_FIRST_BLK];
-  __shared__ uint32_t s_lab[WELD_FIRST_BLK];
-  __shared__ uint8_t s_item[WELD_FIRST_BLK];
-  stage_decode_tables(s_pack, s_comb, sx, sxy);
-  for (int k = threadIdx.x; k < 256 * MC_MAX_TRIS; k += blockDim.x)
-    s_first[k] = MC_TRI_FIRST[k / MC_MAX_TRIS][k % MC_MAX_TRIS];
-  if (threadIdx.x < 12) s_need[threadIdx.x] = MC_EDGE_NEED[threadIdx.x];
-  const uint64_t t = (uint64_t)blockIdx.x * WELD_FIRST_BLK + threadIdx.x;
-  const uint32_t t0 = blockIdx.x * WELD_FIRST_BLK;
-  const uint64_t first = blk_item[blockIdx.x];
-  const uint64_t it = first + threadIdx.x;
-  s_off[threadIdx.x] = itoff[std::min<uint64_t>(it, nitems)];
-  if (threadIdx.x == 0)
-    s_off[WELD_FIRST_BLK] =
-        itoff[std::min<uint64_t>(first + WELD_FIRST_BLK, nitems)];
-  __syncthreads();
-  {
-    const uint32_t lo = std::max(s_off[threadIdx.x], t0);
-    const uint32_t hi = std::min<uint32_t>(s_off[threadIdx.x + 1],
-                                           t0 + WELD_FIRST_BLK);
-    if (lo < hi) {
-      s_rec[threadIdx.x] = order ? item_recs[order[it]] : item_recs[it];
-      s_lab[threadIdx.x] = item_lab[it];
-      for (uint32_t q = lo; q < hi; ++q)
-        s_item[q - t0] = (uint8_t)threadIdx.x;
+  __shared__ WeldTile s_tile;
+  stage_decode_tables(s_pack, s_comb, g.usx, g.usxy);
+  stage_item_first(s_ifirst);
+  const uint32_t b = blk_list[blockIdx.x];
+  const uint32_t t0 = b * WELD_BLK;
+  const uint32_t t1 = std::min(t0 + WELD_BLK, ntris);
+  const uint64_t first = blk_item[b];
+  stage_weld_tile<false>(
+      s_tile, load_weld_item(item_recs, order, itscan, first, nitems), t0,
+                  t1);
+  const uint32_t t = t0 + threadIdx.x;
+  uint4 quad = make_uint4(0, 0, 0, WELD_EMPTY);
+  if (t < t1) {
+    const uint32_t j = s_tile.item[threadIdx.x];
+    const uint32_t l = item_lab[first + j];
+    if (vbase[l + 1] - vbase[l] > WELD_LDS_CAP) {
+      const TriCorners c = decode_tri(s_tile, s_pack, s_ifirst, s_comb, j, t);
+      #pragma unroll
+      for (int v = 0; v < 3; ++v)
+        if ((c.first >> v) & 1u) {
+          wminp[c.slot[v]] = c.id[v];
+          write_slot_vertex(verts, c.id[v], c.slot[v], g);
+        }
+      quad = make_uint4(c.slot[0], c.slot[1], c.slot[2], l);
+      if (lab_sorted) lab_sorted[t] = l;
     }
   }
-  __syncthreads();
-  const uint32_t lane = threadIdx.x & (WAVE - 1);
-  bool f[3] = {false, false, false};
-  if (t < ntris) {
-    const uint32_t j = s_item[threadIdx.x];
-    uint2 rec = s_rec[j];
-    rec.y |= ((uint32_t)t - s_off[j]) << 8;
-    lab_sorted[t] = s_lab[j];
-    const uint32_t ti = (rec.y & 255u) * MC_MAX_TRIS + ((rec.y >> 8) & 7u);
-    const uint32_t pk = s_pack[ti];
-    const uint32_t fb = s_first[ti];
-    const uint32_t interior = ~(rec.y >> 11) & 7u;
-    const uint32_t cl3 = rec.x * 3u;
-    #pragma unroll
-    for (int v = 0; v < 3; ++v) {
-      const uint32_t nib = (pk >> (5 * v)) & 31u;
-      const uint32_t e = nib & 15u;
-      const uint32_t slot = ((cl3 + s_comb[e]) << 1) | (nib >> 4);
-      slots_sorted[3 * t + v] = slot;
-      f[v] = ((fb >> v) & 1u) && (s_need[e] & interior) == 0;
-      if (f[v]) wminp[slot] = (uint32_t)(3 * t + v);
-    }
-  }
-  const unsigned long long bal[3] = {__ballot(f[0]), __ballot(f[1]),
-                                     __ballot(f[2])};
-  const uint64_t w0 = (t / WAVE) * 3;
-  #pragma unroll
-  for (uint32_t j = 0; j < 3; ++j) {
-    const uint32_t c = 64 * j + lane;
-    const uint32_t q = c / 3, r = c - 3 * q;
-    const unsigned long long src = r == 0 ? bal[0] : (r == 1 ? bal[1] : bal[2]);
-    const unsigned long long word = __ballot((src >> q) & 1ull);
-    if (lane == j && w0 + j < nwords) bits[w0 + j] = word;
-  }
-}
-
-struct PopcWord {
-  __device__ uint32_t operator()(unsigned long long w) const {
-    return (uint32_t)__popcll(w);
-  }
-};
-
-__device__ __forceinline__ uint32_t vtx_id_of(
-    const uint32_t *__restrict__ wscan,
-    const unsigned long long *__restrict__ bits, uint64_t i) {
-  uint64_t w = i >> 6;
-  unsigned long long mask = (1ull << (i & 63)) - 1;
-  return wscan[w] + (uint32_t)__popcll(bits[w] & mask);
-}
-
-__global__ void k_total_verts(const uint32_t *__restrict__ wscan,
-                              const unsigned long long *__restrict__ bits,
-                              uint64_t nwords, uint32_t *out) {
-  *out = wscan[nwords - 1] + (uint32_t)__popcll(bits[nwords - 1]);
-}
-
-__global__ void k_vbase(const uint32_t *__restrict__ tri_off,
-                        const uint32_t *__restrict__ wscan,
-                        const unsigned long long *__restrict__ bits,
-                        uint32_t *__restrict__ vbase,
-                        uint32_t nlabels, uint64_t total_verts) {
-  uint32_t l = blockIdx.x * blockDim.x + threadIdx.x;
-  if (l > nlabels) return;
-  if (l == nlabels) vbase[l] = (uint32_t)total_verts;
-  else vbase[l] = vtx_id_of(wscan, bits, 3ull * tri_off[l]);
-}
-
-__global__ void k_weld_verts_faces(const uint32_t *__restrict__ slots,
-                                   const uint32_t *__restrict__ wminp,
-                                   const uint32_t *__restrict__ lab_sorted,
-                                   const uint32_t *__restrict__ wscan,
-                                   const unsigned long long *__restrict__ bits,
-                                   const uint32_t *__restrict__ vbase,
-                                   float *__restrict__ verts,
-                                   uint32_t *__restrict__ faces,
-                                   uint32_t usx, uint32_t usxy,
-                                   float rx, float ry, float rz, float shift,
-                                   uint64_t ntris) {
-  uint64_t t = (uint64_t)blockIdx.x * blockDim.x + threadIdx.x;
-  if (t >= ntris) return;
-  const uint32_t e[3] = {slots[3 * t], slots[3 * t + 1], slots[3 * t + 2]};
-  const uint32_t base = vbase[lab_sorted[t]];
-  const uint64_t w0 = (3 * t) >> 6;
-  const uint32_t b0 = (uint32_t)((3 * t) & 63);
-  const bool straddle = b0 > 61;
-  const unsigned long long word0 = bits[w0];
-  const uint32_t scan0 = wscan[w0];
-  const unsigned long long word1 = straddle ? bits[w0 + 1] : 0ull;
-  const uint32_t scan1 = straddle ? wscan[w0 + 1] : 0u;
-  #pragma unroll
-  for (int v = 0; v < 3; ++v) {
-    uint32_t b = b0 + v;
-    const bool second = b > 63;
-    const unsigned long long word = second ? word1 : word0;
-    b &= 63;
-    uint32_t vid;
-    if ((word >> b) & 1ull) {
-      vid = (second ? scan1 : scan0) +
-            (uint32_t)__popcll(word & ((1ull << b) - 1));
-      uint32_t eslot = e[v] >> 1;
-      uint32_t axis = eslot % 3u;
-      uint32_t lin = eslot / 3u;
-      uint32_t vz = lin / usxy;
-      uint32_t rem = lin - vz * usxy;
-      uint32_t vy = rem / usx;
-      uint32_t vx = rem - vy * usx;
-      float dx = (float)(2 * vx + (axis == 0));
-      float dy = (float)(2 * vy + (axis == 1));
-      float dz = (float)(2 * vz + (axis == 2));
-      verts[3ull * vid + 0] = (0.5f * dx + shift) * rx;
-      verts[3ull * vid + 1] = (0.5f * dy + shift) * ry;
-      verts[3ull * vid + 2] = (0.5f * dz + shift) * rz;
-    } else {
-      vid = vtx_id_of(wscan, bits, wminp[e[v]]);
-    }
-    faces[3 * t + v] = vid - base;
-  }
+  quads[(uint64_t)blockIdx.x * WELD_BLK + threadIdx.x] = quad;
+}
+
+__global__ void k_weld_faces(const uint4 *__restrict__ quads,
+                             const uint32_t *__restrict__ blk_list,
+                             const uint32_t *__restrict__ wminp,
+                             const uint32_t *__restrict__ vbase,
+                             uint32_t *__restrict__ faces) {
+  const uint4 q = quads[(uint64_t)blockIdx.x * WELD_BLK + threadIdx.x];
+  if (q.w == WELD_EMPTY) return;
+  const uint64_t t = (uint64_t)blk_list[blockIdx.x] * WELD_BLK + threadIdx.x;
+  const uint32_t base = vbase[q.w];
+  faces[3 * t + 0] = wminp[q.x] - base;
+  faces[3 * t + 1] = wminp[q.y] - base;
+  faces[3 * t + 2] = wminp[q.z] - base;
 }
 
 __global__ void k_iota(uint32_t *p, uint64_t n) {
@@ -687,6 +804,7 @@
   if (hipSetDevice(device_id) != hipSuccess) return nullptr;
   mg_ctx *c = new mg_ctx();
   c->device = device_id;
+  c->stats.weld_lds_cap = WELD_LDS_CAP;
   bool ok =
       hipStreamCreateWithFlags(&c->stream, hipStreamNonBlocking) ==
           hipSuccess &&
@@ -753,7 +871,7 @@
   const uint32_t *item_lab;
   const uint2 *rec_src;
   const uint32_t *order_sorted;
-  uint32_t *slots;
+  bool simplify;
   uint32_t *lab_sorted;
 };
 
@@ -942,33 +1060,22 @@
   return 0;
 }
 
-struct TriSortView {
-  uint64_t *recs, *recs_alt;
-  uint32_t *slots;
-};
-
-static TriSortView tri_sort_view(mg_ctx *c, uint64_t NI) {
-  return {reinterpret_cast<uint64_t *>(c->tri_keys.get()),
-          reinterpret_cast<uint64_t *>(c->keys_sorted.get()),
-          c->keys_sorted.get() + 2 * NI};
-}
-
 static int run_partition(mg_ctx *c, ChunkCall &k) {
   hipStream_t s = c->stream;
   const uint64_t T = k.T, NI = k.NI;
   const char *sre = getenv("MG_SORT_RECS");
   const bool sort_recs = !(sre && sre[0] == '0');
-  if (ensure(c, c->keys_sorted, 2 * NI + 3 * T)) return 19;
   if (ensure(c, c->tri_label_alt, NI)) return 19;
-  const TriSortView tv = tri_sort_view(c, NI);
-  k.slots = tv.slots;
   const dim3 nb((uint32_t)((NI + 255) / 256)), blk(256);
   unsigned end_bit = 1;
   while ((1u << end_bit) < k.nlabels) ++end_bit;
   rocprim::double_buffer<uint32_t> d_keys(c->tri_label.get(),
                                           c->tri_label_alt.get());
   if (sort_recs) {
-    rocprim::double_buffer<uint64_t> d_vals(tv.recs, tv.recs_alt);
+    if (ensure(c, c->keys_sorted, 2 * NI)) return 19;
+    rocprim::double_buffer<uint64_t> d_vals(
+        reinterpret_cast<uint64_t *>(c->tri_keys.get()),
+        reinterpret_cast<uint64_t *>(c->keys_sorted.get()));
     if (int e = sort_pairs(c, d_keys, d_vals, NI, 0u, end_bit, s,
                            "radix_sort size query failed",
                            "radix_sort failed", 19))
@@ -989,36 +1096,36 @@
     k.order_sorted = d_vals.current();
   }
   k.item_lab = d_keys.current();
-  if (ensure(c, c->itoff, NI + 1)) return 19;
-  uint32_t *itoff = c->itoff.get();
+  if (ensure(c, c->itscan, NI + 1)) return 19;
+  uint64_t *itscan = c->itscan.get();
   if (int e = k.order_sorted
-          ? scan_incl_u32(c, rocprim::make_transform_iterator(
-                                 k.order_sorted, ItemTrisVia{k.rec_src}),
-                          itoff + 1, NI, s, "item scan size query failed",
+          ? scan_incl_u64(c, rocprim::make_transform_iterator(
+                                 k.order_sorted, ItemCountsVia{k.rec_src}),
+                          itscan + 1, NI, s, "item scan size query failed",
                           "item scan failed", 19)
-          : scan_incl_u32(c, rocprim::make_transform_iterator(
-                                 k.rec_src, ItemTris{}),
-                          itoff + 1, NI, s, "item scan size query failed",
+          : scan_incl_u64(c, rocprim::make_transform_iterator(
+                                 k.rec_src, ItemCounts{}),
+                          itscan + 1, NI, s, "item scan size query failed",
                           "item scan failed", 19))
     return e;
-  if (ensure(c, c->tri_off, (uint64_t)k.nlabels + 1)) return 19;
-  if (ensure(c, c->blk_item, (T + WELD_FIRST_BLK - 1) / WELD_FIRST_BLK))
-    return 19;
-  hipLaunchKernelGGL(k_label_ranges, nb, blk, 0, s, k.item_lab, itoff,
-                     c->tri_off.get(), c->blk_item.get(), NI, T, k.nlabels);
+  const uint64_t nl1 = (uint64_t)k.nlabels + 1;
+  if (ensure(c, c->tri_off, nl1)) return 19;
+  if (ensure(c, c->lab_item, nl1)) return 19;
+  if (ensure(c, c->vbase, nl1)) return 19;
+  if (ensure(c, c->blk_item, (T + WELD_BLK - 1) / WELD_BLK)) return 19;
+  hipLaunchKernelGGL(k_label_ranges, nb, blk, 0, s, k.item_lab, itscan,
+                     c->tri_off.get(), c->lab_item.get(), c->vbase.get(),
+                     c->blk_item.get(), NI, k.nlabels);
   HIP_TRY(c, hipGetLastError(), 19);
   HIP_TRY(c, hipEventRecord(c->ev[EV_PARTITION_END], s), 19);
   return 0;
 }
 
-struct WeldScanView {
-  unsigned long long *bits;
-  uint32_t *wscan;
-};
-
-static WeldScanView weld_scan_view(mg_ctx *c, uint64_t nwords) {
-  return {reinterpret_cast<unsigned long long *>(c->vtx_scan.get()),
-          c->vtx_scan.get() + 2 * nwords};
+static int check_weld_err(mg_ctx *c) {
+  const uint32_t werr = *c->h_weld_err.get();
+  if (!werr) return 0;
+  SET_ERR(c, "weld: a label table probe reached its bound (flag %u)", werr);
+  return 29;
 }
 
 static int run_weld(mg_ctx *c, ChunkCall &k) {
@@ -1026,51 +1133,78 @@
   const uint64_t T = k.T, NC = 3 * T;
   const uint64_t wslots = 6 * k.nvox;
   if (wslots >= (1ull << 32)) {
-    SET_ERR(c, "chunk too large for the 32-bit weld table (%d x %d x %d); "
+    SET_ERR(c, "chunk too large for the 32-bit weld slots (%d x %d x %d); "
             "split the task shape (the reference's own mesher bound is "
             "1023x1023x511, igneous_cli/cli.py:1049-1052)", k.sx, k.sy, k.sz);
     return 20;
   }
-  if (ensure(c, c->wh_keys, wslots)) return 20;
-  if (ensure(c, c->vtx_scan, NC)) return 20;
-  if (ensure(c, c->lab_sorted, T)) return 20;
-  k.lab_sorted = c->lab_sorted.get();
-  uint32_t *wminp = c->wh_keys.get();
-  const dim3 nbt((uint32_t)((T + 255) / 256)), blk(256);
-  const uint64_t nwords = (NC + 63) / 64;
-  auto [bits, wscan] = weld_scan_view(c, nwords);
-  hipLaunchKernelGGL(k_weld_first,
-                     dim3((uint32_t)((T + WELD_FIRST_BLK - 1) / WELD_FIRST_BLK)),
-                     dim3(WELD_FIRST_BLK), 0, s, k.rec_src, k.order_sorted,
-                     k.item_lab, c->itoff.get(), c->blk_item.get(),
-                     k.lab_sorted, k.slots, wminp, bits, k.g.sx,
-                     k.g.sx * k.g.sy, k.NI, T, nwords);
-  if (int e = scan_u32(c, rocprim::make_transform_iterator(bits, PopcWord{}),
-                       wscan, nwords, s, "weld scan size query failed",
-                       "weld scan failed", 20))
-    return e;
-  uint32_t *d_tv = &c->scalars->weld_verts;
-  hipLaunchKernelGGL(k_total_verts, dim3(1), dim3(1), 0, s, wscan, bits,
-                     nwords, d_tv);
-  uint32_t tv = 0;
-  HIP_TRY(c, hipMemcpyAsync(&tv, d_tv, 4, hipMemcpyDeviceToHost, s), 21);
+  const uint32_t nblocks = (uint32_t)((T + WELD_BLK - 1) / WELD_BLK);
+  if (ensure(c, c->blk_list, nblocks)) return 20;
+  if (ensure(c, c->h_weld_err, 1)) return 20;
+  *c->h_weld_err.get() = 0;
+  hipLaunchKernelGGL(k_weld_plan,
+                     dim3((uint32_t)(((uint64_t)k.nlabels * WAVE + 255) / 256)),
+                     dim3(256), 0, s, c->tri_off.get(), c->vbase.get(),
+                     k.nlabels, c->blk_list.get(), &c->scalars->weld_nlist,
+                     &c->scalars->weld_table_labels);
+  uint64_t tot = 0;
+  uint32_t plan[2] = {0, 0};
+  HIP_TRY(c, hipMemcpyAsync(&tot, c->itscan.get() + k.NI, 8,
+                            hipMemcpyDeviceToHost, s), 21);
+  HIP_TRY(c, hipMemcpyAsync(plan, &c->scalars->weld_nlist, 8,
+                            hipMemcpyDeviceToHost, s), 21);
   HIP_TRY(c, hipStreamSynchronize(s), 21);
-  k.V = tv;
-  c->stats.total_verts = tv;
+  k.V = tot >> 32;
+  const uint64_t nlist = plan[0];
+  c->stats.total_verts = k.V;
+  c->stats.weld_table_labels = plan[1];
+  c->stats.weld_lds_labels = k.nlabels - plan[1];
 
   if (ensure(c, c->verts, 3 * k.V)) return 22;
   if (ensure(c, c->faces, NC)) return 22;
-  if (ensure(c, c->vbase, (uint64_t)k.nlabels + 1)) return 22;
-  hipLaunchKernelGGL(k_vbase, dim3((k.nlabels + 1 + 255) / 256), dim3(256),
-                     0, s, c->tri_off.get(), wscan, bits, c->vbase.get(),
-                     k.nlabels, k.V);
-  hipLaunchKernelGGL(k_weld_verts_faces, nbt, blk, 0, s, k.slots, wminp,
-                     k.lab_sorted, wscan, bits, c->vbase.get(),
-                     c->verts.get(), c->faces.get(), (uint32_t)k.g.sx,
-                     (uint32_t)(k.g.sx * k.g.sy), k.rx, k.ry, k.rz,
-                     k.voxel_centered ? 0.0f : 0.5f, T);
+  k.lab_sorted = nullptr;
+  if (k.simplify) {
+    if (ensure(c, c->lab_sorted, T)) return 22;
+    if (ensure(c, c->vtx_scan, k.V + 1)) return 22;
+    k.lab_sorted = c->lab_sorted.get();
+  }
+  const WeldGeom wg = {(uint32_t)k.g.sx, (uint32_t)(k.g.sx * k.g.sy),
+                       k.rx, k.ry, k.rz, k.voxel_centered ? 0.0f : 0.5f};
+  uint32_t *d_err = &c->scalars->weld_err;
+  if (plan[1] < k.nlabels) {
+    auto launch_band = [&](auto capc, uint32_t lo_cap) {
+      hipLaunchKernelGGL(k_weld_label<decltype(capc)::value>, dim3(k.nlabels),
+                         dim3(WELD_BLK), 0, s, k.rec_src, k.order_sorted,
+                         c->itscan.get(), c->lab_item.get(), c->tri_off.get(),
+                         c->vbase.get(), k.lab_sorted, c->verts.get(),
+                         c->faces.get(), wg, lo_cap, d_err);
+    };
+    launch_band(std::integral_constant<uint32_t, WELD_LDS_CAP>{},
+                WELD_LDS_CAP / 2);
+    launch_band(std::integral_constant<uint32_t, WELD_LDS_CAP / 2>{},
+                WELD_LDS_CAP / 4);
+    launch_band(std::integral_constant<uint32_t, WELD_LDS_CAP / 4>{}, 0u);
+  }
+  if (nlist > 0) {
+    if (ensure(c, c->wh_keys, wslots)) return 22;
+    if (ensure(c, c->weld_quads, nlist * WELD_BLK)) return 22;
+    hipLaunchKernelGGL(k_weld_first, dim3((uint32_t)nlist), dim3(WELD_BLK), 0,
+                       s, k.rec_src, k.order_sorted, k.item_lab,
+                       c->itscan.get(), c->blk_item.get(), c->blk_list.get(),
+                       c->vbase.get(), c->weld_quads.get(), c->wh_keys.get(),
+                       k.lab_sorted, c->verts.get(), wg, k.NI, (uint32_t)T);
+    hipLaunchKernelGGL(k_weld_faces, dim3((uint32_t)nlist), dim3(WELD_BLK), 0,
+                       s, c->weld_quads.get(), c->blk_list.get(),
+                       c->wh_keys.get(), c->vbase.get(), c->faces.get());
+  }
   HIP_TRY(c, hipGetLastError(), 22);
+  HIP_TRY(c, hipMemcpyAsync(c->h_weld_err.get(), d_err, 4,
+                            hipMemcpyDeviceToHost, s), 22);
   HIP_TRY(c, hipEventRecord(c->ev[EV_WELD_END], s), 22);
+  if (k.simplify) {
+    HIP_TRY(c, hipStreamSynchronize(s), 22);
+    if (int e = check_weld_err(c)) return e;
+  }
   return 0;
 }
 
@@ -1178,6 +1312,7 @@
   g.nseg = g.nsegx * g.ncy * g.ncz;
 
   memset(&c->stats, 0, sizeof(c->stats));
+  c->stats.weld_lds_cap = WELD_LDS_CAP;
   c->stats.bytes_read_algorithmic = k.nvox * k.esize;
   hipStream_t s = c->stream;
 
@@ -1210,9 +1345,10 @@
     write_stage_times(c, r, false);
     return 0;
   }
+  k.simplify = r.reduction_factor > 1;
   if (int e = run_partition(c, k)) return e;
   if (int e = run_weld(c, k)) return e;
-  if (r.reduction_factor > 1 && k.T > 0)
+  if (k.simplify)
     if (int e = run_simplify(c, k.nlabels, k.lab_sorted, r.reduction_factor,
                              r.max_error, &k.T, &k.V))
       return e;
@@ -1222,6 +1358,11 @@
     return e;
   HIP_TRY(c, hipEventRecord(c->ev[EV_END], s), 25);
   HIP_TRY(c, hipStreamSynchronize(s), 25);
+  if (int e = check_weld_err(c)) {
+    if (r.bout) { mg_blobset_free(*r.bout); *r.bout = nullptr; }
+    else { mg_meshset_free(*r.out); *r.out = nullptr; }
+    return e;
+  }
   write_stage_times(c, r, true);
   return 0;
 }
diff --git a/igneous_amd/csrc/mg_ctx.h b/igneous_amd/csrc/mg_ctx.h
--- a/igneous_amd/csrc/mg_ctx.h
+++ b/igneous_amd/csrc/mg_ctx.h
@@ -58,7 +58,9 @@
   uint32_t lh_counter;
   uint32_t lh_overflow;
   uint32_t map_err;
-  uint32_t weld_verts;
+  uint32_t weld_nlist;
+  uint32_t weld_table_labels;
+  uint32_t weld_err;
   uint32_t simp_kept;
   uint32_t simp_new_verts;
   uint32_t simp_final_tris;
@@ -67,6 +69,8 @@
 };
 static_assert(offsetof(CtxScalars, lh_overflow) ==
                   offsetof(CtxScalars, lh_counter) + 4, "");
+static_assert(offsetof(CtxScalars, weld_table_labels) ==
+                  offsetof(CtxScalars, weld_nlist) + 4, "");
 
 struct SimpPlane;
 struct CmMisc;
@@ -77,15 +81,19 @@
   LabelVolume labels, holes;
   DevBuf scan_tmp, sort_tmp;
   DevArr<uint64_t> lh_keys, label_values,
-      segcnt, segoff;
+      segcnt, segoff,
+      itscan;
   DevArr<uint32_t> lh_vals,
       tri_label, tri_label_alt, order, order_alt, tri_off,
-      itoff,
+      lab_item,
       blk_item,
+      blk_list,
       lab_sorted,
       keys_sorted,
       vtx_scan,
-      wh_keys, faces, vbase;
+      wh_keys,
+      faces, vbase;
+  DevArr<uint4> weld_quads;
   DevArr<uint2> tri_keys;
   DevArr<float> verts;
   DevArr<SimpPlane> simp_fq;
@@ -159,6 +167,7 @@
   HostArr<float> h_verts;
   HostArr<uint32_t> h_faces;
   HostArr<uint8_t> h_blob;
+  HostArr<uint32_t> h_weld_err;
   hipEvent_t ev[EV_COUNT_] = {};
 
   ~mg_ctx() {
@@ -167,6 +176,7 @@
     h_verts.release();
     h_faces.release();
     h_blob.release();
+    h_weld_err.release();
     for (auto &e : ev) if (e) (void)hipEventDestroy(e);
     if (stream2) (void)hipStreamDestroy(stream2);
     if (stream) (void)hipStreamDestroy(stream);
@@ -267,13 +277,13 @@
 }
 
 template <typename In>
-static int scan_incl_u32(mg_ctx *c, In in, uint32_t *out, size_t n,
+static int scan_incl_u64(mg_ctx *c, In in, uint64_t *out, size_t n,
                          hipStream_t s, const char *err_size,
                          const char *err_run, int rc) {
   return rocprim_two_call(
       c, c->scan_tmp, err_size, err_run, rc, [&](void *tmp, size_t &bytes) {
         return rocprim::inclusive_scan(tmp, bytes, in, out, n,
-                                       rocprim::plus<uint32_t>(), s);
+                                       rocprim::plus<uint64_t>(), s);
       });
 }
 
diff --git a/igneous_amd/engine.py b/igneous_amd/engine.py
--- a/igneous_amd/engine.py
+++ b/igneous_amd/engine.py
@@ -102,6 +102,14 @@
 class MgStatsEncode(MgStatsFill):
     _fields_ = [
         ("ms_encode", ctypes.c_double),
+    ]
+
+
+class MgStatsWeld(MgStatsEncode):
+    _fields_ = [
+        ("weld_lds_labels", ctypes.c_uint64),
+        ("weld_table_labels", ctypes.c_uint64),
+        ("weld_lds_cap", ctypes.c_uint64),
     ]
 
 
@@ -334,7 +342,7 @@
         lib.mg_label_counts_free.argtypes = [ctypes.POINTER(_MgLabelCounts)]
         lib.mg_get_stats.restype = ctypes.c_int
         lib.mg_get_stats.argtypes = [ctypes.c_void_p,
-                                     ctypes.POINTER(MgStatsEncode)]
+                                     ctypes.POINTER(MgStatsWeld)]
         lib.mg_last_error.restype = ctypes.c_char_p
         lib.mg_last_error.argtypes = [ctypes.c_void_p]
         lib.mg_device_count.restype = ctypes.c_int
@@ -831,7 +839,7 @@
         return EncodedLevel(tuple(tuple(p) for p in nodes), sizes, blob)
 
     def stats(self) -> dict:
-        s = MgStatsEncode()
+        s = MgStatsWeld()
         rc = self.lib.mg_get_stats(self.ctx, ctypes.byref(s))
         if rc != 0:
             raise RuntimeError("mg_get_stats failed")
diff --git a/include/meshgine.h b/include/meshgine.h
--- a/include/meshgine.h
+++ b/include/meshgine.h
@@ -56,6 +56,9 @@
   double ms_labelmap;
   double ms_fill;
   double ms_encode;
+  uint64_t weld_lds_labels;
+  uint64_t weld_table_labels;
+  uint64_t weld_lds_cap;
 } mg_stats;
 
 #define MG_ENC_PRECOMPUTED 0u
```

Measured after the change: 14610 Mvox/s (median of 6 runs). 19.2% higher.
